# IGNF/MAESTRO

Measured on AMD Instinct MI355X. Metric: MAE-pretrain tiles/sec, higher is better.
Workload: dtype bf16

## Files before the change

### __graft_entry__.py

```python

from __future__ import annotations

import os
import subprocess
import sys
from pathlib import Path

ROOT = Path(__file__).resolve().parent
if str(ROOT) not in sys.path:
    sys.path.insert(0, str(ROOT))


def build() -> None:
    from maestro_amd.csrc.build import build as build_lib
    from maestro_amd.csrc.build import build_example

    lib = build_lib(verbose=bool(os.environ.get("MAESTRO_BUILD_VERBOSE")))
    build_example()
    import ctypes

    import maestro_amd
    from maestro_amd import hip

    handle = ctypes.CDLL(str(lib))
    import re

    for name in ("maestro_hip.h", "maestro_hip_metrics.h", "maestro_hip_det.h"):
        header = (ROOT / "include" / name).read_text()
        missing = [n for n in re.findall(r"\b(mh_[a-z0-9_]+)\s*\(", header) if not hasattr(handle, n)]
        if missing:
            raise RuntimeError(f"libmaestro_hip.so lacks symbols declared in include/{name}: {sorted(set(missing))}")
    assert hip.lib().mh_version() >= 1


def smoke() -> None:
    import torch

    import maestro_amd.conf as conf
    from maestro_amd.ssl import mae as pmae
    from maestro_amd.train.optim import FusedAdamW
    from oracle import mae as om
    from oracle.gen_golden import build_datasets, case_table, init_weights, make_batch

    if not torch.cuda.is_available():
        raise RuntimeError("smoke() needs cuda:0")
    dev = torch.device("cuda:0")
    case = case_table()["c3_aerial_s2"]
    ds = build_datasets(case, conf)
    kw = dict(interpolate="nearest", model="mae", num_levels=1, fusion_mode=case["fusion"], inter_depth=case["inter_depth"],
              **case["model_kw"])
    oracle = om.build_oracle(ds, conf.MaskConfig(), model_size=case["size"], **kw)
    init_weights(oracle, case["seed"])
    model = getattr(pmae, f"mae_{case['size']}")(datasets=ds, mask=conf.MaskConfig(), **kw)
    model.load_state_dict(oracle.state_dict(), strict=True)
    batch = make_batch(ds.dataset, case["B"], case["seed"], stress=case.get("stress", False))
    eng = model.engine(case["B"], dev, loss="l2_norm")
    torch.manual_seed(7)
    noise, struct = eng.draw_masks()
    loss = eng.forward({k: v.to(dev) for k, v in batch.items()}, noise=noise, struct=struct)
    eng.zero_grad()
    eng.backward()
    pixels, masks = eng.reconstructions()
    ob, orec, omsk, _ = oracle({k: v.clone() for k, v in batch.items()}, "pretrain", noise=noise,
                               struct_masks={g: s[:, :, None] for g, s in struct.items()})
    want = om.compute_loss_rec(ob, orec, omsk, oracle.out_grid_size, om.norm_bands_of(ds.dataset), "l2_norm")
    got = float(loss.item())
    assert abs(got - want.item()) < 3e-3 * abs(want.item()), (got, want.item())
    for m in orec:
        assert torch.equal(masks[m].cpu(), omsk[m]), f"{m}: mask indices differ from the oracle"
        rel = ((pixels[m].cpu() - orec[m]).norm() / orec[m].norm()).item()
        assert rel < 1.3e-2, (m, rel)
    FusedAdamW(eng, 1e-3).step()
    loss2 = float(eng.forward({k: v.to(dev) for k, v in batch.items()}, noise=noise, struct=struct).item())
    assert loss2 < got, (loss2, got)
    print(f"smoke ok: loss hip={got:.6f} oracle={want.item():.6f}; after one AdamW step {loss2:.6f}")


if __name__ == "__main__":
    build()
    if "--smoke" in sys.argv:
# ... 2 lines not shown
```

### maestro_amd/csrc/build.py

```python

from __future__ import annotations

import hashlib
import os
import shutil
import subprocess
import sys
from concurrent.futures import ThreadPoolExecutor
from pathlib import Path

CSRC = Path(__file__).resolve().parent
ROOT = CSRC.parent.parent
LIB_DIR = CSRC.parent / "lib"
LIB = LIB_DIR / "libmaestro_hip.so"
OBJ_DIR = CSRC / "build"
ARCH = "gfx950"
FLAGS = ["-O3", "-std=c++17", "-fPIC", f"--offload-arch={ARCH}", "-Wno-unused-result"] + os.environ.get("MH_BUILD_FLAGS", "").split()
FILE_FLAGS = {"attn.hip": ["-mllvm", "-amdgpu-mfma-vgpr-form", "-fno-slp-vectorize"] + os.environ.get("MH_ATTN_FLAGS", "").split(),
              "gemm_sk.hip": ["-mllvm", "-amdgpu-mfma-vgpr-form"]}
NO_PK_F32 = ["-Xclang", "-target-feature", "-Xclang", "-packed-fp32-ops"]
for _f in ("gemm.hip", "gemm_pp.hip", "gemm_dma.hip"):
    FILE_FLAGS[_f] = FILE_FLAGS.get(_f, []) + NO_PK_F32


def _hipcc() -> str:
    for cand in (shutil.which("hipcc"), "/opt/rocm/bin/hipcc"):
        if cand and Path(cand).exists():
            return cand
    raise RuntimeError("hipcc not found; the MI355X kernels cannot be built")


def _digest(src: Path) -> str:
    h = hashlib.sha256()
    for f in [src, *sorted(CSRC.glob("*.hpp")), ROOT / "include" / "maestro_hip.h",
              ROOT / "include" / "maestro_hip_metrics.h", ROOT / "include" / "maestro_hip_det.h"]:
        h.update(f.read_bytes())
    h.update(" ".join(FLAGS + FILE_FLAGS.get(src.name, [])).encode())
    return h.hexdigest()[:16]


def build(force: bool = False, verbose: bool = False) -> Path:
    hipcc = _hipcc()
    OBJ_DIR.mkdir(exist_ok=True)
    LIB_DIR.mkdir(exist_ok=True)
    sources = sorted(CSRC.glob("*.hip"))
    jobs, objs = [], []
    for src in sources:
        obj = OBJ_DIR / f"{src.stem}.{_digest(src)}.o"
        objs.append(obj)
        if force or not obj.exists():
            for old in OBJ_DIR.glob(f"{src.stem}.*.o"):
                old.unlink()
            jobs.append((src, obj))

    def compile_one(job):
        src, obj = job
        cmd = [hipcc, *FLAGS, *FILE_FLAGS.get(src.name, []), "-c", str(src), "-o", str(obj)]
        if verbose:
            print(" ".join(cmd), flush=True)
        r = subprocess.run(cmd, capture_output=True, text=True)
        if r.returncode != 0:
            raise RuntimeError(f"hipcc failed for {src.name}:\n{r.stdout}\n{r.stderr}")
        return "\n".join(ln for ln in r.stderr.splitlines() if "'-packed-fp32-ops' is not a recognized feature" not in ln)

    if jobs:
        with ThreadPoolExecutor(max_workers=min(4, os.cpu_count() or 1)) as ex:
            for warn in ex.map(compile_one, jobs):
                if verbose and warn:
                    print(warn, file=sys.stderr)
    if jobs or not LIB.exists():
        cmd = [hipcc, "-shared", "-fPIC", f"--offload-arch={ARCH}", *map(str, objs), "-o", str(LIB)]
        r = subprocess.run(cmd, capture_output=True, text=True)
        if r.returncode != 0:
            raise RuntimeError(f"link failed:\n{r.stdout}\n{r.stderr}")
    return LIB


EXAMPLE_SRC = ROOT / "examples" / "abi_smoke.cpp"
EXAMPLE_BIN = ROOT / "examples" / "abi_smoke"


def build_example(force: bool = False) -> Path:
    if not force and EXAMPLE_BIN.exists() and EXAMPLE_BIN.stat().st_mtime >= max(EXAMPLE_SRC.stat().st_mtime, LIB.stat().st_mtime):
        return EXAMPLE_BIN
    cmd = [_hipcc(), "-O2", "-std=c++17", f"--offload-arch={ARCH}", str(EXAMPLE_SRC), f"-I{ROOT / 'include'}", f"-L{LIB_DIR}",
           "-lmaestro_hip", "-Wl,-rpath,$ORIGIN/../maestro_amd/lib", "-o", str(EXAMPLE_BIN)]
    r = subprocess.run(cmd, capture_output=True, text=True)
    if r.returncode != 0:
# ... 8 lines not shown
```

### maestro_amd/csrc/embed.hip

```cpp
#include "common.hpp"
#include "reduce_det.hpp"
#include "../../include/maestro_hip.h"

namespace {

__device__ __forceinline__ float block_sum_any(float v, float* red) {
    v = wave_sum(v);
    const int nw = blockDim.x >> 6;
    if (nw == 1) return v;
    const int w = threadIdx.x >> 6, l = threadIdx.x & 63;
    __syncthreads();
    if (l == 0) red[w] = v;
    __syncthreads();
    float t = 0.f;
    for (int i = 0; i < nw; ++i) t += red[i];
    return t;
}

__global__ void patchify_kernel(const float* __restrict__ img, bf16_t* __restrict__ cols, float* __restrict__ target,
                                int Csrc, int c0, int Ctot, int S, int P, int Kpad, const int* __restrict__ norm_bands,
                                int n_groups, int normalise, int rescale_elev) {
    extern __shared__ __attribute__((aligned(16))) float patch[];
    const int g = S / P;
    const int tok = blockIdx.x;
    const int bd = tok / (g * g), pp = tok - bd * g * g, ph = pp / g, pw = pp - ph * g;
    const int PP = P * P, K = Ctot * PP;
    float* red = patch + K;
    const float* base0 = img + ((size_t)bd * Csrc) * S * S + (size_t)(ph * P) * S + pw * P;
    const float* base = base0 + (size_t)c0 * S * S;
    if ((P & 3) == 0 && (Kpad & 3) == 0) {
        for (int k = threadIdx.x * 4; k < Kpad; k += blockDim.x * 4) {
            f32x4 v = {0.f, 0.f, 0.f, 0.f};
            if (k < K) {
                const int c = k / PP, r = k - c * PP, p1 = r / P, p2 = r - p1 * P;
                v = *reinterpret_cast<const f32x4*>(base + (size_t)c * S * S + p1 * S + p2);
                if (rescale_elev && c0 + c >= 1) v = 30.f * (*reinterpret_cast<const f32x4*>(base0 + p1 * S + p2) - v);
#pragma unroll
                for (int e = 0; e < 4; ++e) patch[(r + e) * Ctot + c] = v[e];
            }
            if (cols) {
                u32x2 pk = {pack_bf2(v[0], v[1]), pack_bf2(v[2], v[3])};
                *reinterpret_cast<u32x2*>(cols + (size_t)tok * Kpad + k) = pk;
            }
        }
    } else {
        for (int k = threadIdx.x; k < Kpad; k += blockDim.x) {
            float v = 0.f;
            if (k < K) {
                const int c = k / PP, r = k - c * PP, p1 = r / P, p2 = r - p1 * P;
                v = base[(size_t)c * S * S + p1 * S + p2];
                if (rescale_elev && c0 + c >= 1) v = 30.f * (base0[p1 * S + p2] - v);
                patch[r * Ctot + c] = v;
            }
            if (cols) cols[(size_t)tok * Kpad + k] = f2bf(v);
        }
// ... 130 lines not shown
    }
}

__global__ __launch_bounds__(64) void gn_finalize_kernel(const float* __restrict__ partial, float* __restrict__ stats,
                                                         long per_image, int nchunk, float eps) {
    const int bd = blockIdx.x;
    double s = 0.0;
    for (int i = threadIdx.x; i < nchunk; i += 64) s += partial[((size_t)bd * nchunk + i) * 2];
    for (int o = 32; o > 0; o >>= 1) s += __shfl_xor(s, o, 64);
    const double mu = s / per_image;
    double q = 0.0;
    for (int i = threadIdx.x; i < nchunk; i += 64) {
        const float sc = partial[((size_t)bd * nchunk + i) * 2];
        const float nc = (float)min((long)GN_CHUNK, per_image - (long)i * GN_CHUNK);
        const float mc = sc / nc;
        const double dm = (double)mc - mu;
        q += partial[((size_t)bd * nchunk + i) * 2 + 1] + dm * (2.0 * ((double)sc - (double)nc * mc) + (double)nc * dm);
    }
    for (int o = 32; o > 0; o >>= 1) q += __shfl_xor(q, o, 64);
    if (threadIdx.x == 0) {
        const double var = fmax(q / per_image, 0.0);
        stats[bd * 2] = (float)mu;
        stats[bd * 2 + 1] = (float)(1.0 / sqrt(var + (double)eps));
    }
}

__global__ __launch_bounds__(256) void embed_finish_kernel(const float* __restrict__ y, const float* __restrict__ stats,
                                                           const float* __restrict__ gamma, const float* __restrict__ beta,
                                                           const float* __restrict__ pos, const float* __restrict__ date,
                                                           float* __restrict__ xg, int B, int D, int L, int E, int tok_off,
                                                           int Lgroup, int date_rows, int date_off) {
    const int row = blockIdx.x * 4 + (threadIdx.x >> 6), lane = threadIdx.x & 63;
    if (row >= B * D * L) return;
    const int bd = row / L, l = row - bd * L, b = bd / D, d = bd - b * D;
    const float mu = stats[bd * 2], rs = stats[bd * 2 + 1];
    const float* yr = y + (size_t)row * E;
    float* o = xg + ((size_t)b * Lgroup + tok_off + d * L + l) * E;
    const float* pr = pos + (size_t)l * E;
    const float* dr = date ? date + ((size_t)b * date_rows + date_off + d) * 8 : nullptr;
    for (int c = lane * 4; c < E; c += 256) {
        const f32x4 v = *reinterpret_cast<const f32x4*>(yr + c);
        const f32x4 g = *reinterpret_cast<const f32x4*>(gamma + c);
        const f32x4 bt = *reinterpret_cast<const f32x4*>(beta + c);
        const f32x4 ps = *reinterpret_cast<const f32x4*>(pr + c);
        f32x4 r;
#pragma unroll
        for (int e = 0; e < 4; ++e) r[e] = (v[e] - mu) * rs * g[e] + bt[e] + ps[e];
        if (dr && c >= E - 8) r += *reinterpret_cast<const f32x4*>(dr + (c - (E - 8)));
        *reinterpret_cast<f32x4*>(o + c) = r;
    }
}

constexpr int EB_ROWS = 8;
template <int NV, bool DET>
__global__ __launch_bounds__(256) void embed_bwd_stats_kernel(const float* __restrict__ dxg, const float* __restrict__ y,
                                                              const float* __restrict__ stats, const float* __restrict__ gamma,
                                                              float* __restrict__ sums, float* __restrict__ dgamma,
                                                              float* __restrict__ dbeta, int B, int D, int L, int E,
                                                              int tok_off, int Lgroup) {
    extern __shared__ __attribute__((aligned(16))) float red[];
    const int w = threadIdx.x >> 6, lane = threadIdx.x & 63;
    const int bd = blockIdx.y, b = bd / D, d = bd - b * D;
    const float mu = stats[bd * 2], rs = stats[bd * 2 + 1];
    float* rg = red + (size_t)w * 2 * E;
    float s1 = 0.f, s2 = 0.f;
    const int l0 = (blockIdx.x * 4 + w) * EB_ROWS;
    if constexpr (NV > 0) {
        f32x4 gz[NV], gd[NV], gm[NV];
#pragma unroll
        for (int j = 0; j < NV; ++j) {
            const int c = lane * 4 + 256 * j;
            gz[j] = (f32x4){0, 0, 0, 0}; gd[j] = (f32x4){0, 0, 0, 0};
            gm[j] = c < E ? *reinterpret_cast<const f32x4*>(gamma + c) : (f32x4){0, 0, 0, 0};
        }
#pragma unroll 2
        for (int rr = 0; rr < EB_ROWS; ++rr) {
            const int l = l0 + rr;
            if (l >= L) break;
            const float* yr = y + ((size_t)bd * L + l) * E;
            const float* gr = dxg + ((size_t)b * Lgroup + tok_off + d * L + l) * E;
#pragma unroll
            for (int j = 0; j < NV; ++j) {
                const int c = lane * 4 + 256 * j;
                if (c < E) {
                    const f32x4 v = *reinterpret_cast<const f32x4*>(yr + c);
                    const f32x4 dd = *reinterpret_cast<const f32x4*>(gr + c);
#pragma unroll
                    for (int e = 0; e < 4; ++e) {
                        const float z = (v[e] - mu) * rs, dz = dd[e] * gm[j][e];
                        s1 += dz; s2 += dz * z;
                        gz[j][e] += dd[e] * z;
                        gd[j][e] += dd[e];
                    }
                }
            }
        }
#pragma unroll
        for (int j = 0; j < NV; ++j) {
            const int c = lane * 4 + 256 * j;
            if (c < E) {
                *reinterpret_cast<f32x4*>(rg + c) = gz[j];
                *reinterpret_cast<f32x4*>(rg + E + c) = gd[j];
            }
        }
    } else {
        for (int c = lane; c < 2 * E; c += 64) rg[c] = 0.f;
        for (int rr = 0; rr < EB_ROWS; ++rr) {
            const int l = l0 + rr;
            if (l >= L) break;
            const float* yr = y + ((size_t)bd * L + l) * E;
            const float* gr = dxg + ((size_t)b * Lgroup + tok_off + d * L + l) * E;
            for (int c = lane * 4; c < E; c += 256) {
                const f32x4 v = *reinterpret_cast<const f32x4*>(yr + c);
                const f32x4 dd = *reinterpret_cast<const f32x4*>(gr + c);
                const f32x4 gm = *reinterpret_cast<const f32x4*>(gamma + c);
#pragma unroll
                for (int e = 0; e < 4; ++e) {
                    const float z = (v[e] - mu) * rs, dz = dd[e] * gm[e];
                    s1 += dz; s2 += dz * z;
                    rg[c + e] += dd[e] * z;
                    rg[E + c + e] += dd[e];
                }
            }
        }
    }
    s1 = wave_sum(s1); s2 = wave_sum(s2);
    if constexpr (DET) {
        if (lane == 0) { red[8 * E + 2 * w] = s1; red[8 * E + 2 * w + 1] = s2; }
    } else {
    if (lane == 0) { atomicAdd(sums + bd * 2, s1); atomicAdd(sums + bd * 2 + 1, s2); }
    }
    __syncthreads();
    for (int c = threadIdx.x; c < 2 * E; c += 256) {
        const float t = red[c] + red[2 * E + c] + red[4 * E + c] + red[6 * E + c];
        if constexpr (DET) {
            dgamma[((size_t)bd * gridDim.x + blockIdx.x) * 2 * E + c] = t;
        } else {
        if (c < E) atomicAdd(dgamma + c, t); else atomicAdd(dbeta + (c - E), t);
        }
    }
    if constexpr (DET) {
        if (threadIdx.x < 2) {
            const float* ws = red + 8 * E + threadIdx.x;
            sums[((size_t)bd * gridDim.x + blockIdx.x) * 2 + threadIdx.x] = ((ws[0] + ws[2]) + ws[4]) + ws[6];
        }
    }
}

__global__ __launch_bounds__(64) void embed_bwd_sums_det_kernel(const float* __restrict__ blk_sums, float* __restrict__ sums, int nblk) {
    if (threadIdx.x < 2)
        sums[blockIdx.x * 2 + threadIdx.x] = 0.f + ordered_job_total(blk_sums + (size_t)blockIdx.x * nblk * 2 + threadIdx.x, nblk, 2);
}

__global__ __launch_bounds__(256) void zero_f32_kernel(float* __restrict__ p, int n) {
    const int i = blockIdx.x * 256 + threadIdx.x;
    if (i < n) p[i] = 0.f;
}

__global__ __launch_bounds__(256) void embed_bwd_apply_kernel(const float* __restrict__ dxg, const float* __restrict__ y,
                                                              const float* __restrict__ stats, const float* __restrict__ gamma,
                                                              const float* __restrict__ sums, bf16_t* __restrict__ dyc,
                                                              int B, int D, int L, int E, int tok_off, int Lgroup) {
    const int row = blockIdx.x * 4 + (threadIdx.x >> 6), lane = threadIdx.x & 63;
    if (row >= B * D * L) return;
    const int bd = row / L, l = row - bd * L, b = bd / D, d = bd - b * D;
    const float mu = stats[bd * 2], rs = stats[bd * 2 + 1];
    const float n = (float)L * (float)E;
    const float c1 = sums[bd * 2] / n, c2 = sums[bd * 2 + 1] / n;
    const float* yr = y + (size_t)row * E;
    const float* gr = dxg + ((size_t)b * Lgroup + tok_off + d * L + l) * E;
    bf16_t* o = dyc + (size_t)row * E;
    for (int c = lane * 4; c < E; c += 256) {
        const f32x4 v = *reinterpret_cast<const f32x4*>(yr + c);
        const f32x4 dd = *reinterpret_cast<const f32x4*>(gr + c);
        const f32x4 gm = *reinterpret_cast<const f32x4*>(gamma + c);
        float r[4];
#pragma unroll
        for (int e = 0; e < 4; ++e) {
            const float z = (v[e] - mu) * rs;
            r[e] = rs * (dd[e] * gm[e] - c1 - z * c2);
        }
        u32x2 pk = {pack_bf2(r[0], r[1]), pack_bf2(r[2], r[3])};
        *reinterpret_cast<u32x2*>(o + c) = pk;
    }
}

__global__ __launch_bounds__(256) void depatchify_kernel(const float* __restrict__ patches, float* __restrict__ img,
                                                         int C, int S, int P, long total) {
    const long i = (long)blockIdx.x * 256 + threadIdx.x;
    if (i >= total) return;
    const int x = i % S; long r = i / S;
    const int yy = r % S; r /= S;
    const int c = r % C; const long bd = r / C;
    const int g = S / P, ph = yy / P, p1 = yy - ph * P, pw = x / P, p2 = x - pw * P;
    img[i] = patches[((bd * g + ph) * g + pw) * (long)(P * P * C) + (p1 * P + p2) * C + c];
}

__global__ __launch_bounds__(256) void date_features_kernel(const int16_t* __restrict__ dates, const int16_t* __restrict__ ref,
                                                            float* __restrict__ out, int B, int D, int rows, int row_off, float fac) {
    const int i = blockIdx.x * 256 + threadIdx.x;
    if (i >= B * D) return;
    const int b = i / D, d = i - b * D;
    const int16_t* dt = dates + (size_t)i * 3;
    const float year = (float)dt[0], doy = (float)dt[1] / 365.25f, hour = (float)dt[2] / 24.0f;
    const float year_ref = (float)ref[b * 3], doy_ref = (float)ref[b * 3 + 1] / 365.25f;
    const float diff = (year + doy) - (year_ref + doy_ref);
    const float a = 6.283185307179586f * doy, h = 6.283185307179586f * hour;
    float* o = out + ((size_t)b * rows + row_off + d) * 8;
    o[0] = o[1] = o[2] = o[3] = diff * fac;
    o[4] = sinf(a) * fac; o[5] = cosf(a) * fac; o[6] = sinf(h) * fac; o[7] = cosf(h) * fac;
}

__global__ __launch_bounds__(256) void rescale_elev_kernel(const float* __restrict__ img, float* __restrict__ out, int C, long plane, long total) {
    const long i = (long)blockIdx.x * 256 + threadIdx.x;
    if (i >= total) return;
    const long px = i % plane; const long r = i / plane; const int c = r % C; const long bd = r / C;
    const float v = img[i];
    out[i] = c == 0 ? v : 30.f * (img[(bd * C) * plane + px] - v);
}

__device__ __forceinline__ void cubic_weights(float t, float (&w)[4]) {
    const float A = -0.75f;
    const float x0 = t + 1.f, x3 = 2.f - t, x2 = 1.f - t;
    w[0] = ((A * x0 - 5.f * A) * x0 + 8.f * A) * x0 - 4.f * A;
    w[1] = ((A + 2.f) * t - (A + 3.f)) * t * t + 1.f;
    w[2] = ((A + 2.f) * x2 - (A + 3.f)) * x2 * x2 + 1.f;
    w[3] = ((A * x3 - 5.f * A) * x3 + 8.f * A) * x3 - 4.f * A;
}
__global__ __launch_bounds__(256) void resize_kernel(const float* __restrict__ in, float* __restrict__ out, int Hin, int Win,
                                                     int Hout, int Wout, int mode, long total) {
    const long i = (long)blockIdx.x * 256 + threadIdx.x;
    if (i >= total) return;
    const int x = i % Wout; const long r = i / Wout; const int y = r % Hout; const long plane = r / Hout;
    const float* src = in + plane * (long)Hin * Win;
    const float sy = (float)Hin / (float)Hout, sx = (float)Win / (float)Wout;
    if (mode == 0) {
        const int yy = min((int)floorf(y * sy), Hin - 1), xx = min((int)floorf(x * sx), Win - 1);
// ... 135 lines not shown
    MH_LAUNCH_CHECK();
    return 0;
}

extern "C" int mh_groupnorm_stats(const float* y, float* partial, float* stats, int BD, int L, int E, float eps,
                                  void* stream) {
    MH_CHECK_ARG(y && partial && stats && E % 4 == 0, "mh_groupnorm_stats: bad arguments");
    const long per_image = (long)L * E;
    const int nchunk = ceil_div(per_image, GN_CHUNK);
    hipLaunchKernelGGL(gn_partial_kernel, dim3(nchunk, BD), dim3(256), 0, (hipStream_t)stream, y, partial, per_image, nchunk);
    hipLaunchKernelGGL(gn_finalize_kernel, dim3(BD), dim3(64), 0, (hipStream_t)stream, partial, stats, per_image, nchunk, eps);
    MH_LAUNCH_CHECK();
    return 0;
}

extern "C" int mh_groupnorm_partial_size(int BD, int L, int E) { return BD * ceil_div((long)L * E, GN_CHUNK) * 2; }

extern "C" int mh_embed_finish(const float* y, const float* stats, const float* gamma, const float* beta,
                               const float* pos, const float* date, int date_rows, int date_off, float* xg, int B, int D,
                               int L, int E, int tok_off, int Lgroup, void* stream) {
    MH_CHECK_ARG(y && stats && gamma && beta && pos && xg && E % 4 == 0 && E >= 8, "mh_embed_finish: bad arguments");
    MH_CHECK_ARG(tok_off + D * L <= Lgroup, "mh_embed_finish: modality does not fit its group sequence");
    hipLaunchKernelGGL(embed_finish_kernel, dim3(ceil_div((long)B * D * L, 4)), dim3(256), 0, (hipStream_t)stream, y, stats,
                       gamma, beta, pos, date, xg, B, D, L, E, tok_off, Lgroup, date_rows, date_off);
    MH_LAUNCH_CHECK();
    return 0;
}

extern "C" int mh_embed_finish_bwd(const float* dxg, const float* y, const float* stats, const float* gamma, void* dyc,
                                   float* dgamma, float* dbeta, float* sums, int B, int D, int L, int E, int tok_off,
                                   int Lgroup, void* stream) {
    MH_CHECK_ARG(dxg && y && stats && gamma && dyc && dgamma && dbeta && sums && E % 4 == 0, "mh_embed_finish_bwd: bad arguments");
    hipStream_t s = (hipStream_t)stream;
    hipLaunchKernelGGL(zero_f32_kernel, dim3(ceil_div((long)B * D * 2, 256)), dim3(256), 0, s, sums, B * D * 2);
    {
        const dim3 grid(ceil_div(L, 4 * EB_ROWS), B * D), block(256);
        const size_t lds = (size_t)8 * E * sizeof(float);
#define MH_EB_LAUNCH(NV) hipLaunchKernelGGL((embed_bwd_stats_kernel<NV, false>), grid, block, lds, s, dxg, y, stats, gamma, sums, dgamma, dbeta, B, D, L, E, tok_off, Lgroup)
        switch ((E + 255) / 256) {
            case 1: MH_EB_LAUNCH(1); break;
            case 2: MH_EB_LAUNCH(2); break;
            case 3: MH_EB_LAUNCH(3); break;
            case 4: MH_EB_LAUNCH(4); break;
            default: MH_EB_LAUNCH(0); break;
        }
#undef MH_EB_LAUNCH
    }
    hipLaunchKernelGGL(embed_bwd_apply_kernel, dim3(ceil_div((long)B * D * L, 4)), dim3(256), 0, s, dxg, y, stats, gamma, sums,
                       (bf16_t*)dyc, B, D, L, E, tok_off, Lgroup);
    MH_LAUNCH_CHECK();
    return 0;
}

extern "C" int mh_embed_bwd_partial_rows(int BD, int L) { return BD > 0 && L > 0 ? BD * ceil_div(L, 4 * EB_ROWS) : 0; }

extern "C" int mh_embed_finish_bwd_det(const float* dxg, const float* y, const float* stats, const float* gamma, void* dyc,
                                       float* param_partial, float* blk_sums, float* sums, int B, int D, int L, int E, int tok_off,
                                       int Lgroup, void* stream) {
    MH_CHECK_ARG(dxg && y && stats && gamma && dyc && param_partial && blk_sums && sums, "mh_embed_finish_bwd_det: null pointer");
    MH_CHECK_ARG(B > 0 && D > 0 && L > 0 && E > 0 && E % 4 == 0 && tok_off >= 0 && tok_off + D * L <= Lgroup,
                 "mh_embed_finish_bwd_det: bad sizes B=%d D=%d L=%d E=%d tok_off=%d Lgroup=%d", B, D, L, E, tok_off, Lgroup);
    hipStream_t s = (hipStream_t)stream;
    const int nblk = ceil_div(L, 4 * EB_ROWS);
    {
        const dim3 grid(nblk, B * D), block(256);
        const size_t lds = (size_t)(8 * E + 8) * sizeof(float);
#define MH_EB_LAUNCH(NV) hipLaunchKernelGGL((embed_bwd_stats_kernel<NV, true>), grid, block, lds, s, dxg, y, stats, gamma, blk_sums, param_partial, (float*)nullptr, B, D, L, E, tok_off, Lgroup)
        switch ((E + 255) / 256) {
            case 1: MH_EB_LAUNCH(1); break;
            case 2: MH_EB_LAUNCH(2); break;
            case 3: MH_EB_LAUNCH(3); break;
            case 4: MH_EB_LAUNCH(4); break;
            default: MH_EB_LAUNCH(0); break;
        }
#undef MH_EB_LAUNCH
    }
    hipLaunchKernelGGL(embed_bwd_sums_det_kernel, dim3(B * D), dim3(64), 0, s, blk_sums, sums, nblk);
    hipLaunchKernelGGL(embed_bwd_apply_kernel, dim3(ceil_div((long)B * D * L, 4)), dim3(256), 0, s, dxg, y, stats, gamma, sums,
                       (bf16_t*)dyc, B, D, L, E, tok_off, Lgroup);
    MH_LAUNCH_CHECK();
    return 0;
}

extern "C" int mh_depatchify(const float* patches, float* img, int BD, int C, int S, int P, void* stream) {
    MH_CHECK_ARG(patches && img && S % P == 0, "mh_depatchify: bad arguments");
    const long total = (long)BD * C * S * S;
    hipLaunchKernelGGL(depatchify_kernel, dim3(ceil_div(total, 256)), dim3(256), 0, (hipStream_t)stream, patches, img, C, S, P, total);
    MH_LAUNCH_CHECK();
    return 0;
}
```

### maestro_amd/csrc/loss.hip

```cpp
#include "gemm_common.hpp"
#include "../../include/maestro_hip_det.h"

namespace {

template <bool DET>
__global__ __launch_bounds__(256) void masked_loss_kernel(const float* __restrict__ rec, const float* __restrict__ target,
                                                          const uint8_t* __restrict__ mask_group, const int* __restrict__ n_masked,
                                                          float weight, float* __restrict__ acc, bf16_t* __restrict__ drec,
                                                          int B, int Lm, int Lgroup, int tok_off, int PPC, int p, int tgt_C,
                                                          int tgt_c0, int n_g, int denom_is_elems, int rows_per_wave) {
    __shared__ float red[4];
    const int w = threadIdx.x >> 6, lane = threadIdx.x & 63;
    const float coef = weight / (denom_is_elems ? (float)(*n_masked) : (float)(*n_masked) * (float)PPC);
    const bool window = n_g != tgt_C;
    const int tgt_ld = window ? PPC / n_g * tgt_C : PPC;
    float s = 0.f;
    for (int rr = 0; rr < rows_per_wave; ++rr) {
        const int row = (blockIdx.x * 4 + w) * rows_per_wave + rr;
        if (row >= B * Lm) break;
        const int b = row / Lm, t = row - b * Lm;
        const bool masked = mask_group[(size_t)b * Lgroup + tok_off + t] != 0;
        const float* r = rec + (size_t)row * PPC;
        const float* g = target + (size_t)row * tgt_ld;
        bf16_t* d = drec ? drec + (size_t)row * PPC : nullptr;
        for (int c = lane * 4; c < PPC; c += 256) {
            float dd[4] = {0.f, 0.f, 0.f, 0.f};
            if (masked) {
                const f32x4 rv = *reinterpret_cast<const f32x4*>(r + c);
                f32x4 tv;
                if (!window) {
                    tv = *reinterpret_cast<const f32x4*>(g + c);
                } else {
#pragma unroll
                    for (int e = 0; e < 4; ++e) { const int pix = (c + e) / n_g; tv[e] = g[pix * tgt_C + tgt_c0 + (c + e) - pix * n_g]; }
                }
#pragma unroll
                for (int e = 0; e < 4; ++e) {
                    const float diff = rv[e] - tv[e];
                    if (p == 2) { s += diff * diff; dd[e] = 2.f * diff * coef; }
                    else { s += fabsf(diff); dd[e] = (diff > 0.f ? coef : (diff < 0.f ? -coef : 0.f)); }
                }
            }
            if (d) {
                u32x2 pk = {pack_bf2(dd[0], dd[1]), pack_bf2(dd[2], dd[3])};
                *reinterpret_cast<u32x2*>(d + c) = pk;
            }
        }
    }
    s = wave_sum(s);
    if (lane == 0) red[w] = s;
    __syncthreads();
    if (threadIdx.x == 0) {
        const float t = (red[0] + red[1]) + (red[2] + red[3]);
        if constexpr (DET) {
            acc[blockIdx.x] = (blockIdx.x == 0 && *n_masked == 0) ? __builtin_nanf("") : t * coef;
        } else {
        if (t != 0.f) atomicAdd(acc, t * coef);
        if (blockIdx.x == 0 && *n_masked == 0) atomicAdd(acc, __builtin_nanf(""));
        }
    }
}

template <bool DET>
__global__ __launch_bounds__(1024) void colsum_kernel(const void* __restrict__ x, int is_f32, float* __restrict__ out, int M,
                                                      int N, int ld, int rows_per_block) {
    __shared__ f32x4 red[16][64];
    const int w = threadIdx.x >> 6, lane = threadIdx.x & 63, nw = blockDim.x >> 6;
    const int c = (blockIdx.x * 64 + lane) * 4;
    const int r0 = blockIdx.y * rows_per_block, r1 = min(M, r0 + rows_per_block);
    f32x4 acc = {0, 0, 0, 0};
    if (c < N) {
        if (is_f32) {
#pragma unroll 8
            for (int r = r0 + w; r < r1; r += nw)
                acc += *reinterpret_cast<const f32x4*>(reinterpret_cast<const float*>(x) + (size_t)r * ld + c);
        } else {
#pragma unroll 8
            for (int r = r0 + w; r < r1; r += nw) {
                const u32x2 pk = *reinterpret_cast<const u32x2*>(reinterpret_cast<const bf16_t*>(x) + (size_t)r * ld + c);
                acc += (f32x4){__uint_as_float(pk[0] << 16), __uint_as_float(pk[0] & 0xffff0000u),
                               __uint_as_float(pk[1] << 16), __uint_as_float(pk[1] & 0xffff0000u)};
            }
        }
    }
    red[w][lane] = acc;
    __syncthreads();
    if (w == 0 && c < N) {
        f32x4 t = red[0][lane];
        for (int i = 1; i < nw; ++i) t += red[i][lane];
        if constexpr (DET) {
            *reinterpret_cast<f32x4*>(out + (size_t)blockIdx.y * N + c) = t;
        } else {
#pragma unroll
        for (int e = 0; e < 4; ++e) atomicAdd(out + c + e, t[e]);
        }
    }
}

__global__ __launch_bounds__(256) void zero_spans_kernel(float* __restrict__ base, const long* __restrict__ spans) {
    const long off = spans[2 * blockIdx.y], len = spans[2 * blockIdx.y + 1];
// ... 140 lines not shown
    MH_CHECK_ARG((p == 1 || p == 2) && PPC % 4 == 0 && tok_off + Lm <= Lgroup, "mh_masked_loss: bad arguments");
    const int rpw = loss_rows_per_wave((long)B * Lm);
    hipLaunchKernelGGL(masked_loss_kernel<false>, dim3(ceil_div((long)B * Lm, 4 * rpw)), dim3(256), 0, (hipStream_t)stream, rec, target, mask_group, n_masked,
                       weight, acc, (bf16_t*)drec, B, Lm, Lgroup, tok_off, PPC, p, 1, 0, 1, 0, rpw);
    MH_LAUNCH_CHECK();
    return 0;
}

extern "C" int mh_masked_loss_bands(const float* rec, const float* target, const uint8_t* mask_group, const int* n_elems,
                                    float weight, float* acc, void* drec, int B, int Lm, int Lgroup, int tok_off, int PPC, int p,
                                    int tgt_C, int tgt_c0, int n_g, void* stream) {
    MH_CHECK_ARG(rec && target && mask_group && n_elems && acc, "mh_masked_loss_bands: null pointer");
    MH_CHECK_ARG((p == 1 || p == 2) && PPC % 4 == 0 && tok_off + Lm <= Lgroup, "mh_masked_loss_bands: bad arguments");
    MH_CHECK_ARG(n_g > 0 && PPC % n_g == 0 && tgt_c0 >= 0 && tgt_c0 + n_g <= tgt_C, "mh_masked_loss_bands: band window [%d, %d) of %d",
                 tgt_c0, tgt_c0 + n_g, tgt_C);
    const int rpw = loss_rows_per_wave((long)B * Lm);
    hipLaunchKernelGGL(masked_loss_kernel<false>, dim3(ceil_div((long)B * Lm, 4 * rpw)), dim3(256), 0, (hipStream_t)stream, rec, target, mask_group, n_elems,
                       weight, acc, (bf16_t*)drec, B, Lm, Lgroup, tok_off, PPC, p, tgt_C, tgt_c0, n_g, 1, rpw);
    MH_LAUNCH_CHECK();
    return 0;
}

extern "C" int mh_masked_loss_partial_size(int B, int Lm) {
    const long rows = (long)B * Lm;
    return rows > 0 ? ceil_div(rows, 4 * loss_rows_per_wave(rows)) : 0;
}

extern "C" int mh_masked_loss_det(const float* rec, const float* target, const uint8_t* mask_group, const int* n_masked,
                                  float weight, float* loss_partial, void* drec, int B, int Lm, int Lgroup, int tok_off, int PPC,
                                  int p, void* stream) {
    MH_CHECK_ARG(rec && target && mask_group && n_masked && loss_partial, "mh_masked_loss_det: null pointer");
    MH_CHECK_ARG(B > 0 && Lm > 0 && (p == 1 || p == 2) && PPC % 4 == 0 && tok_off + Lm <= Lgroup, "mh_masked_loss_det: bad arguments");
    const int rpw = loss_rows_per_wave((long)B * Lm);
    hipLaunchKernelGGL(masked_loss_kernel<true>, dim3(ceil_div((long)B * Lm, 4 * rpw)), dim3(256), 0, (hipStream_t)stream, rec, target,
                       mask_group, n_masked, weight, loss_partial, (bf16_t*)drec, B, Lm, Lgroup, tok_off, PPC, p, 1, 0, 1, 0, rpw);
    MH_LAUNCH_CHECK();
    return 0;
}

extern "C" int mh_masked_loss_bands_det(const float* rec, const float* target, const uint8_t* mask_group, const int* n_elems,
                                        float weight, float* loss_partial, void* drec, int B, int Lm, int Lgroup, int tok_off,
                                        int PPC, int p, int tgt_C, int tgt_c0, int n_g, void* stream) {
    MH_CHECK_ARG(rec && target && mask_group && n_elems && loss_partial, "mh_masked_loss_bands_det: null pointer");
    MH_CHECK_ARG(B > 0 && Lm > 0 && (p == 1 || p == 2) && PPC % 4 == 0 && tok_off + Lm <= Lgroup, "mh_masked_loss_bands_det: bad arguments");
    MH_CHECK_ARG(n_g > 0 && PPC % n_g == 0 && tgt_c0 >= 0 && tgt_c0 + n_g <= tgt_C, "mh_masked_loss_bands_det: band window [%d, %d) of %d",
                 tgt_c0, tgt_c0 + n_g, tgt_C);
    const int rpw = loss_rows_per_wave((long)B * Lm);
    hipLaunchKernelGGL(masked_loss_kernel<true>, dim3(ceil_div((long)B * Lm, 4 * rpw)), dim3(256), 0, (hipStream_t)stream, rec, target,
                       mask_group, n_elems, weight, loss_partial, (bf16_t*)drec, B, Lm, Lgroup, tok_off, PPC, p, tgt_C, tgt_c0, n_g, 1, rpw);
    MH_LAUNCH_CHECK();
    return 0;
}

extern "C" int mh_colsum_partial_rows(int M) { return M > 0 ? ceil_div(M, MH_COLSUM_PARTIAL_ROWS) : 0; }

extern "C" int mh_colsum_partial(const void* x, int x_is_f32, float* partial, int M, int N, int ld, void* stream) {
    MH_CHECK_ARG(x && partial && ((uintptr_t)partial % 16) == 0, "mh_colsum_partial: null pointer / partial not 16-byte aligned");
    MH_CHECK_ARG(M > 0 && N > 0 && N % 4 == 0 && ld % 4 == 0 && N <= ld, "mh_colsum_partial: bad sizes M=%d N=%d ld=%d", M, N, ld);
    hipLaunchKernelGGL(colsum_kernel<true>, dim3(ceil_div(N, 256), ceil_div(M, MH_COLSUM_PARTIAL_ROWS)), dim3(1024), 0,
                       (hipStream_t)stream, x, x_is_f32, partial, M, N, ld, MH_COLSUM_PARTIAL_ROWS);
    MH_LAUNCH_CHECK();
    return 0;
}

extern "C" int mh_colsum(const void* x, int x_is_f32, float* out, int M, int N, int ld, void* stream) {
    MH_CHECK_ARG(x && out && N % 4 == 0 && ld % 4 == 0, "mh_colsum: bad arguments");
    const int col_blocks = ceil_div(N, 256);
    int rows_per_block = 1024;
    while (rows_per_block > 128 && (long)col_blocks * ceil_div(M, rows_per_block) < 128) rows_per_block >>= 1;
    hipLaunchKernelGGL(colsum_kernel<false>, dim3(col_blocks, ceil_div(M, rows_per_block)), dim3(1024), 0, (hipStream_t)stream, x,
                       x_is_f32, out, M, N, ld, rows_per_block);
    MH_LAUNCH_CHECK();
    return 0;
}

extern "C" int mh_zero_spans(float* base, const long* spans_device, int n_spans, long max_len, void* stream) {
    MH_CHECK_ARG(base && spans_device && n_spans > 0 && max_len > 0, "mh_zero_spans: bad arguments");
    dim3 grid((unsigned)min(64L, (max_len + 1023) / 1024), n_spans);
    hipLaunchKernelGGL(zero_spans_kernel, grid, dim3(256), 0, (hipStream_t)stream, base, spans_device);
    MH_LAUNCH_CHECK();
    return 0;
}

extern "C" int mh_cast_bf16(const float* src, void* dst, long n, void* stream) {
    MH_CHECK_ARG(src && dst && n > 0, "mh_cast_bf16: bad arguments");
    hipLaunchKernelGGL(cast_bf16_kernel, dim3(ceil_div(n, 1024)), dim3(256), 0, (hipStream_t)stream, src, (bf16_t*)dst, n);
    MH_LAUNCH_CHECK();
    return 0;
}

extern "C" int mh_pack_rows_bf16(const float* w, void* dst, int E, int K, int Kpad, void* stream) {
    MH_CHECK_ARG(w && dst && Kpad >= K, "mh_pack_rows_bf16: bad arguments");
    hipLaunchKernelGGL(pack_rows_kernel, dim3(ceil_div((long)E * Kpad, 256)), dim3(256), 0, (hipStream_t)stream, w, (bf16_t*)dst, E, K, Kpad);
    MH_LAUNCH_CHECK();
    return 0;
}

extern "C" int mh_unpack_rows_add(const float* src, float* dst, int E, int K, int Kpad, void* stream) {
    MH_CHECK_ARG(src && dst && Kpad >= K, "mh_unpack_rows_add: bad arguments");
    hipLaunchKernelGGL(unpack_rows_add_kernel, dim3(ceil_div((long)E * K, 256)), dim3(256), 0, (hipStream_t)stream, src, dst, E, K, Kpad);
    MH_LAUNCH_CHECK();
    return 0;
}

extern "C" int mh_adamw(float* p, const float* g, float* m, float* v, void* p_bf16, long n, float lr, float b1, float b2,
                        float eps, float wd, int step, float grad_scale, void* stream) {
// ... 31 lines not shown
```

### maestro_amd/csrc/mask.hip

```cpp
#include "common.hpp"
#include "../../include/maestro_hip.h"

namespace {

__global__ __launch_bounds__(1024) void mask_select_kernel(const float* __restrict__ noise, const uint8_t* __restrict__ smask,
                                                          int* __restrict__ visible_idx, int* __restrict__ masked_idx,
                                                          int* __restrict__ inv, uint8_t* __restrict__ mask, int L, int k) {
    extern __shared__ __attribute__((aligned(16))) float sm[];
    const int L4 = (L + 3) & ~3;
    int* wtot = reinterpret_cast<int*>(sm + L4);
    const int b = blockIdx.x, lane = threadIdx.x & 63, w = threadIdx.x >> 6;
    for (int i = threadIdx.x; i < L4; i += 1024) {
        float v = INFINITY;
        if (i < L) {
            v = noise[(size_t)b * L + i];
            if (smask && smask[(size_t)b * L + i]) v = 0.f;
        }
        sm[i] = v;
    }
    __syncthreads();
    int base = 0;
    for (int i0 = 0; i0 < L; i0 += 1024) {
        const int i = i0 + threadIdx.x;
        int f = 0;
        if (i < L) {
            const float v = sm[i];
            int r = 0;
            for (int j = 0; j < L4; j += 4) {
                const f32x4 u = *reinterpret_cast<const f32x4*>(sm + j);
                r += (int)((u[0] < v) | ((u[0] == v) & (j < i)));
                r += (int)((u[1] < v) | ((u[1] == v) & (j + 1 < i)));
                r += (int)((u[2] < v) | ((u[2] == v) & (j + 2 < i)));
                r += (int)((u[3] < v) | ((u[3] == v) & (j + 3 < i)));
            }
            f = r < k;
        }
        const unsigned long long bal = __ballot(f);
        const int before = __popcll(bal & ((1ull << lane) - 1ull));
        __syncthreads();
        if (lane == 0) wtot[w] = __popcll(bal);
        __syncthreads();
        int nm = base + before, tot = 0;
#pragma unroll
        for (int x = 0; x < 16; ++x) {
            const int c = wtot[x];
            nm += x < w ? c : 0;
            tot += c;
        }
        base += tot;
        if (i < L) {
            mask[(size_t)b * L + i] = (uint8_t)f;
            if (f) {
                masked_idx[(size_t)b * k + nm] = i;
                inv[(size_t)b * L + i] = -1;
            } else {
                visible_idx[(size_t)b * (L - k) + (i - nm)] = i;
                inv[(size_t)b * L + i] = i - nm;
            }
        }
    }
}

__global__ __launch_bounds__(256) void gather_rows_kernel(const float* __restrict__ src, const int* __restrict__ idx,
                                                          float* __restrict__ dst, int B, int src_L, int n_idx, int dim,
                                                          int dst_L, int dst_off) {
    const int row = blockIdx.x * 4 + (threadIdx.x >> 6), lane = threadIdx.x & 63;
    if (row >= B * n_idx) return;
    const int b = row / n_idx, j = row - b * n_idx;
    const float* s = src + ((size_t)b * src_L + idx[row]) * dim;
    float* d = dst + ((size_t)b * dst_L + dst_off + j) * dim;
    for (int c = lane * 4; c < dim; c += 256) *reinterpret_cast<f32x4*>(d + c) = *reinterpret_cast<const f32x4*>(s + c);
}

__global__ __launch_bounds__(256) void scatter_rows_kernel(const float* __restrict__ ddst, const int* __restrict__ idx,
                                                           float* __restrict__ dsrc, int B, int src_L, int n_idx, int dim,
                                                           int dst_L, int dst_off) {
    const int row = blockIdx.x * 4 + (threadIdx.x >> 6), lane = threadIdx.x & 63;
    if (row >= B * n_idx) return;
    const int b = row / n_idx, j = row - b * n_idx;
    float* s = dsrc + ((size_t)b * src_L + idx[row]) * dim;
    const float* d = ddst + ((size_t)b * dst_L + dst_off + j) * dim;
    for (int c = lane * 4; c < dim; c += 256) *reinterpret_cast<f32x4*>(s + c) = *reinterpret_cast<const f32x4*>(d + c);
}

__global__ __launch_bounds__(256) void expand_rows_kernel(const float* __restrict__ src, const int* __restrict__ inv,
                                                          float* __restrict__ dst, int B, int L, int n, int dim) {
    const int row = blockIdx.x * 4 + (threadIdx.x >> 6), lane = threadIdx.x & 63;
    if (row >= B * L) return;
    const int b = row / L, iv = inv[row];
    float* o = dst + (size_t)row * dim;
    const float* s = src + ((size_t)b * n + (iv < 0 ? 0 : iv)) * dim;
    for (int c = lane * 4; c < dim; c += 256) {
        f32x4 v = {0.f, 0.f, 0.f, 0.f};
        if (iv >= 0) v = *reinterpret_cast<const f32x4*>(s + c);
        *reinterpret_cast<f32x4*>(o + c) = v;
    }
}

__global__ __launch_bounds__(256) void unmask_kernel(const float* __restrict__ y, const int* __restrict__ inv,
                                                     const float* __restrict__ mask_token, const int* __restrict__ tok_slot,
                                                     const float* __restrict__ pos, const float* __restrict__ date,
                                                     const int* __restrict__ date_row, int n_date_rows,
                                                     float* __restrict__ xdec, int B, int L, int n_vis, int Dd, int slot_stride) {
    const int row = blockIdx.x * 4 + (threadIdx.x >> 6), lane = threadIdx.x & 63;
    if (row >= B * L) return;
    const int b = row / L, t = row - b * L;
    const int iv = inv[row];
    const float* s = iv < 0 ? mask_token + (size_t)tok_slot[(size_t)b * slot_stride + t] * Dd : y + ((size_t)b * n_vis + iv) * Dd;
    const float* pr = pos + (size_t)t * Dd;
    const float* dr = date ? date + ((size_t)b * n_date_rows + date_row[t]) * 8 : nullptr;
    float* o = xdec + (size_t)row * Dd;
    for (int c = lane * 4; c < Dd; c += 256) {
        f32x4 v = *reinterpret_cast<const f32x4*>(s + c) + *reinterpret_cast<const f32x4*>(pr + c);
        if (dr && c >= Dd - 8) v += *reinterpret_cast<const f32x4*>(dr + (c - (Dd - 8)));
        *reinterpret_cast<f32x4*>(o + c) = v;
    }
}

constexpr int UM_ROWS = 512, UM_NT = 1024;
template <bool DET>
__global__ __launch_bounds__(UM_NT) void unmask_bwd_token_kernel(const float* __restrict__ dxdec, const uint8_t* __restrict__ mask,
                                                                 const int* __restrict__ tok_slot, float* __restrict__ dmask_token,
                                                                 int B, int L, int Dd, int slot, int t_lo, int t_hi, int slot_stride) {
    __shared__ __attribute__((aligned(16))) float red[UM_NT * 4];
// ... 24 lines not shown
                const int off = ri < UM_ROWS ? row_off[ri] : -1;
                if (off >= 0) v[u] = *reinterpret_cast<const f32x4*>(dxdec + (size_t)off * Dd + 4 * col);
            }
            acc += (v[0] + v[1]) + (v[2] + v[3]);
        }
    }
    *reinterpret_cast<f32x4*>(red + 4 * threadIdx.x) = acc;
    __syncthreads();
    if (sub == 0) {
        for (int s = 1; s < lanes; ++s) acc += *reinterpret_cast<const f32x4*>(red + 4 * (s * cols + col));
        if constexpr (DET) {
            *reinterpret_cast<f32x4*>(dmask_token + (size_t)blockIdx.x * Dd + 4 * col) = acc;
        } else {
#pragma unroll
        for (int e = 0; e < 4; ++e) if (acc[e] != 0.f) atomicAdd(dmask_token + 4 * col + e, acc[e]);
        }
    }
}

__global__ __launch_bounds__(1024) void count_masked_kernel(const uint8_t* __restrict__ mask, int B, int L, int t_lo, int t_hi,
                                                            int* __restrict__ out, int mult, int accumulate) {
    __shared__ float red[16];
    const int span = t_hi - t_lo, w = threadIdx.x >> 6, lane = threadIdx.x & 63;
    float c = 0.f;
    for (int b = w; b < B; b += 16) {
        const uint8_t* row = mask + (size_t)b * L + t_lo;
        for (int t = lane; t < span; t += 64) c += row[t] ? 1.f : 0.f;
    }
    c = block_sum<16>(c, red);
    if (threadIdx.x == 0) *out = (accumulate ? *out : 0) + (int)(c + 0.5f) * mult;
}

}

extern "C" int mh_mask_select(const float* noise, const uint8_t* struct_mask, int* visible_idx, int* masked_idx, int* inv,
                              uint8_t* mask, int B, int L, int k, void* stream) {
    MH_CHECK_ARG(noise && visible_idx && masked_idx && inv && mask, "mh_mask_select: null pointer");
    MH_CHECK_ARG(B > 0 && L > 0 && k >= 0 && k <= L && L <= 8192, "mh_mask_select: bad sizes B=%d L=%d k=%d", B, L, k);
    hipLaunchKernelGGL(mask_select_kernel, dim3(B), dim3(1024), (size_t)((L + 3) & ~3) * 4 + 64, (hipStream_t)stream, noise, struct_mask,
                       visible_idx, masked_idx, inv, mask, L, k);
    MH_LAUNCH_CHECK();
    return 0;
}

extern "C" int mh_gather_rows(const float* src, const int* idx, float* dst, int B, int src_L, int n_idx, int dim, int dst_L,
                              int dst_off, void* stream) {
    MH_CHECK_ARG(src && idx && dst && dim % 4 == 0 && dst_off + n_idx <= dst_L, "mh_gather_rows: bad arguments");
    hipLaunchKernelGGL(gather_rows_kernel, dim3(ceil_div((long)B * n_idx, 4)), dim3(256), 0, (hipStream_t)stream, src, idx, dst, B,
                       src_L, n_idx, dim, dst_L, dst_off);
    MH_LAUNCH_CHECK();
    return 0;
}

extern "C" int mh_scatter_rows(const float* ddst, const int* idx, float* dsrc, int B, int src_L, int n_idx, int dim,
                               int dst_L, int dst_off, void* stream) {
    MH_CHECK_ARG(ddst && idx && dsrc && dim % 4 == 0 && dst_off + n_idx <= dst_L, "mh_scatter_rows: bad arguments");
    hipLaunchKernelGGL(scatter_rows_kernel, dim3(ceil_div((long)B * n_idx, 4)), dim3(256), 0, (hipStream_t)stream, ddst, idx, dsrc,
                       B, src_L, n_idx, dim, dst_L, dst_off);
    MH_LAUNCH_CHECK();
    return 0;
}

extern "C" int mh_expand_rows(const float* src, const int* inv, float* dst, int B, int L, int n, int dim, void* stream) {
    MH_CHECK_ARG(src && inv && dst && B > 0 && L > 0 && n > 0 && dim % 4 == 0, "mh_expand_rows: bad arguments");
    hipLaunchKernelGGL(expand_rows_kernel, dim3(ceil_div((long)B * L, 4)), dim3(256), 0, (hipStream_t)stream, src, inv, dst, B, L,
                       n, dim);
    MH_LAUNCH_CHECK();
    return 0;
}

extern "C" int mh_unmask_assemble(const float* y, const int* inv, const float* mask_token, const int* tok_slot,
                                  const float* pos, const float* date, const int* date_row, int n_date_rows, float* xdec,
                                  int B, int L, int n_vis, int Dd, void* stream) {
    MH_CHECK_ARG(y && inv && mask_token && tok_slot && pos && xdec && Dd % 4 == 0 && Dd >= 8, "mh_unmask_assemble: bad arguments");
    MH_CHECK_ARG(!date || date_row, "mh_unmask_assemble: date without date_row");
    hipLaunchKernelGGL(unmask_kernel, dim3(ceil_div((long)B * L, 4)), dim3(256), 0, (hipStream_t)stream, y, inv, mask_token,
                       tok_slot, pos, date, date_row, n_date_rows, xdec, B, L, n_vis, Dd, 0);
    MH_LAUNCH_CHECK();
    return 0;
}

extern "C" int mh_unmask_assemble_per_sample(const float* y, const int* inv, const float* mask_token, const int* tok_slot_bl,
                                             const float* pos, const float* date, const int* date_row, int n_date_rows,
                                             float* xdec, int B, int L, int n_vis, int Dd, void* stream) {
    MH_CHECK_ARG(y && inv && mask_token && tok_slot_bl && pos && xdec && Dd % 4 == 0 && Dd >= 8, "mh_unmask_assemble_per_sample: bad arguments");
    MH_CHECK_ARG(!date || date_row, "mh_unmask_assemble_per_sample: date without date_row");
    hipLaunchKernelGGL(unmask_kernel, dim3(ceil_div((long)B * L, 4)), dim3(256), 0, (hipStream_t)stream, y, inv, mask_token,
                       tok_slot_bl, pos, date, date_row, n_date_rows, xdec, B, L, n_vis, Dd, L);
    MH_LAUNCH_CHECK();
    return 0;
}

extern "C" int mh_unmask_token_grad(const float* dxdec, const uint8_t* mask, const int* tok_slot, float* dmask_token, int B,
                                    int L, int Dd, int slot, int t_lo, int t_hi, void* stream) {
    MH_CHECK_ARG(dxdec && mask && tok_slot && dmask_token && Dd % 4 == 0 && Dd <= 1024, "mh_unmask_token_grad: bad arguments");
    MH_CHECK_ARG(0 <= t_lo && t_lo < t_hi && t_hi <= L, "mh_unmask_token_grad: bad token range");
    hipLaunchKernelGGL(unmask_bwd_token_kernel<false>, dim3(ceil_div((long)B * (t_hi - t_lo), UM_ROWS)), dim3(UM_NT), 0,
                       (hipStream_t)stream, dxdec, mask, tok_slot, dmask_token, B, L, Dd, slot, t_lo, t_hi, 0);
    MH_LAUNCH_CHECK();
    return 0;
}

extern "C" int mh_unmask_token_grad_per_sample(const float* dxdec, const uint8_t* mask, const int* tok_slot_bl, float* dmask_token,
                                               int B, int L, int Dd, int slot, void* stream) {
    MH_CHECK_ARG(dxdec && mask && tok_slot_bl && dmask_token && Dd % 4 == 0 && Dd <= 1024 && B > 0 && L > 0,
                 "mh_unmask_token_grad_per_sample: bad arguments");
// ... 45 lines not shown
```

### maestro_amd/csrc/norm.hip

```cpp
#include "gemm_common.hpp"

namespace {

struct RowMap { int L, off; };
__device__ __forceinline__ size_t map_row(RowMap m, int b, int j) { return (size_t)b * m.L + m.off + j; }

template <int NV>
__global__ __launch_bounds__(256) void ln_fwd_kernel(const float* __restrict__ x, RowMap xm, const float* __restrict__ gamma,
                                                     const float* __restrict__ beta, void* __restrict__ y, RowMap ym,
                                                     int y_is_f32, float* __restrict__ mean, float* __restrict__ rstd,
                                                     int B, int n, int dim, float eps, uint8_t* __restrict__ y8,
                                                     const float* __restrict__ y8_scale, float* __restrict__ y8_amax,
                                                     uint8_t* __restrict__ y8s, int ld_y8s) {
    const int row = blockIdx.x * 4 + (threadIdx.x >> 6);
    const int lane = threadIdx.x & 63;
    if (row >= B * n) return;
    const int b = row / n, j = row - b * n;
    const float* xr = x + map_row(xm, b, j) * dim;
    const int nv = dim >> 2;
    f32x4 v[NV];
    float s = 0.f;
#pragma unroll
    for (int i = 0; i < NV; ++i) {
        const int c = lane + 64 * i;
        v[i] = (f32x4){0, 0, 0, 0};
        if (c < nv) v[i] = *reinterpret_cast<const f32x4*>(xr + 4 * c);
        s += (v[i][0] + v[i][1]) + (v[i][2] + v[i][3]);
    }
    const float mu = wave_sum(s) / dim;
    float q = 0.f;
#pragma unroll
    for (int i = 0; i < NV; ++i) {
        if (lane + 64 * i < nv) {
#pragma unroll
            for (int e = 0; e < 4; ++e) { const float d = v[i][e] - mu; q += d * d; }
        }
    }
    const float rs = rsqrtf(wave_sum(q) / dim + eps);
    if (lane == 0) { mean[row] = mu; rstd[row] = rs; }
    const size_t yrow = map_row(ym, b, j) * dim;
    const bool t8 = y8 && !y8s;
    const float s8 = t8 ? *y8_scale : 0.f;
    float amax8 = 0.f;
#pragma unroll
    for (int i = 0; i < NV; ++i) {
        const int c = lane + 64 * i;
        u32x2 pk16 = {0u, 0u};
        if (c < nv) {
            const f32x4 g = *reinterpret_cast<const f32x4*>(gamma + 4 * c);
            const f32x4 bt = *reinterpret_cast<const f32x4*>(beta + 4 * c);
            f32x4 o;
#pragma unroll
            for (int e = 0; e < 4; ++e) o[e] = (v[i][e] - mu) * rs * g[e] + bt[e];
// ... 269 lines not shown
        gm[i] = *reinterpret_cast<const f32x4*>(gamma + 4 * (lane + 64 * i));
    }
    const int row0 = (blockIdx.x * 4 + w) * ROWS_PER_WAVE;
    if (row0 < B * n) {
        f32x4 xq[ROWS_PER_WAVE][NV], rq[ROWS_PER_WAVE][NV];
        u32x2 dq[ROWS_PER_WAVE][NV];
        float muq[ROWS_PER_WAVE], rsq[ROWS_PER_WAVE];
        size_t xrowq[ROWS_PER_WAVE];
        auto fetch = [&](int p) {
            const int row = row0 + p, b = row / n, j = row - b * n;
            xrowq[p] = map_row(xm, b, j) * dim;
            const size_t dyrow = map_row(dym, b, j) * dim;
            muq[p] = mean[row]; rsq[p] = rstd[row];
#pragma unroll
            for (int i = 0; i < NV; ++i) {
                const int c4 = 4 * (lane + 64 * i);
                xq[p][i] = *reinterpret_cast<const f32x4*>(x + xrowq[p] + c4);
                dq[p][i] = *reinterpret_cast<const u32x2*>(dy + dyrow + c4);
                rq[p][i] = *reinterpret_cast<const f32x4*>(dres + xrowq[p] + c4);
            }
        };
#pragma unroll
        for (int p = 0; p < DEPTH; ++p) fetch(p);
#pragma unroll
        for (int rr = 0; rr < ROWS_PER_WAVE; ++rr) {
            if (rr + DEPTH < ROWS_PER_WAVE) fetch(rr + DEPTH);
            __builtin_amdgcn_sched_barrier(0);
            const float mu = muq[rr], rs = rsq[rr];
            f32x4 xh[NV], dz[NV];
            float s1 = 0.f, s2 = 0.f;
#pragma unroll
            for (int i = 0; i < NV; ++i) {
                const u32x2 pk = dq[rr][i];
                const f32x4 d = {__uint_as_float(pk[0] << 16), __uint_as_float(pk[0] & 0xffff0000u),
                                 __uint_as_float(pk[1] << 16), __uint_as_float(pk[1] & 0xffff0000u)};
#pragma unroll
                for (int e = 0; e < 4; ++e) {
                    xh[i][e] = (xq[rr][i][e] - mu) * rs;
                    dz[i][e] = d[e] * gm[i][e];
                    s1 += dz[i][e];
                    s2 += dz[i][e] * xh[i][e];
                    gsum[i][e] += d[e] * xh[i][e];
                    bsum[i][e] += d[e];
                }
            }
            const float c1 = ln_wave_sum(s1) / dim, c2 = ln_wave_sum(s2) / dim;
#pragma unroll
            for (int i = 0; i < NV; ++i) {
                const int c4 = 4 * (lane + 64 * i);
                f32x4 o;
#pragma unroll
                for (int e = 0; e < 4; ++e) o[e] = rs * (dz[i][e] - c1 - xh[i][e] * c2);
                o += rq[rr][i];
                csum[i] += o;
                *reinterpret_cast<f32x4*>(dx + xrowq[rr] + c4) = o;
                const u32x2 pk = {pack_bf2(o[0], o[1]), pack_bf2(o[2], o[3])};
                *reinterpret_cast<u32x2*>(dx_bf16 + xrowq[rr] + c4) = pk;
            }
            __builtin_amdgcn_sched_barrier(0);
        }
    }
    if (!partial) return;
    float* rg = red + (size_t)w * 3 * dim;
#pragma unroll
    for (int i = 0; i < NV; ++i) {
        const int c4 = 4 * (lane + 64 * i);
        *reinterpret_cast<f32x4*>(rg + c4) = gsum[i];
        *reinterpret_cast<f32x4*>(rg + dim + c4) = bsum[i];
        *reinterpret_cast<f32x4*>(rg + 2 * dim + c4) = csum[i];
    }
    __syncthreads();
    float* prow = partial + (size_t)blockIdx.x * 3 * dim;
    for (int c = threadIdx.x; c < 3 * dim; c += 256)
        prow[c] = red[c] + red[3 * dim + c] + red[6 * dim + c] + red[9 * dim + c];
}

#ifndef LN_BWD_DEPTH
#define LN_BWD_DEPTH 4
#endif
constexpr int RED_ROWS = 8;
__global__ __launch_bounds__(256) void ln_bwd_reduce_kernel(const float* __restrict__ partial, int nblk, int dim,
                                                            float* __restrict__ dgamma, float* __restrict__ dbeta,
                                                            float* __restrict__ dcol) {
    const int c = blockIdx.x * 256 + threadIdx.x;
    if (c >= 3 * dim) return;
    const int r0 = blockIdx.y * RED_ROWS, r1 = min(nblk, r0 + RED_ROWS);
    float s = 0.f;
    for (int r = r0; r < r1; ++r) s += partial[(size_t)r * 3 * dim + c];
    if (c < dim) atomicAdd(dgamma + c, s);
    else if (c < 2 * dim) atomicAdd(dbeta + (c - dim), s);
    else if (dcol) atomicAdd(dcol + (c - 2 * dim), s);
}

__global__ __launch_bounds__(256) void colsum_batched_kernel(const MhColsumJob* __restrict__ jobs, int n_jobs,
                                                             const uint64_t* __restrict__ blocks) {
    const uint64_t e = blocks[blockIdx.x];
    const int ji = (int)(e >> 48);
    if (ji >= n_jobs) return;
    const MhColsumJob j = jobs[ji];
    const int c = (int)((e >> 32) & 0xFFFF) * 256 + threadIdx.x;
    const int r0 = (int)(e & 0xFFFFFFFFu) * MH_COLSUM_ROWS;
    if (c >= j.cols || r0 >= j.rows) return;
    const int r1 = min(j.rows, r0 + MH_COLSUM_ROWS);
    const float* src = j.src + (size_t)r0 * j.ld + c;
    float v[MH_COLSUM_ROWS];
#pragma unroll
// ... 39 lines not shown

static int layernorm_fwd_impl(const float* x, int x_L, int x_off, const float* gamma, const float* beta, void* y, int y_L,
                              int y_off, int y_is_f32, float* mean, float* rstd, int B, int n, int dim, float eps, void* y8,
                              const float* y8_scale, float* y8_amax, void* stream, void* y8s, int ld_y8s) {
    MH_CHECK_ARG(x && gamma && beta && y && mean && rstd, "mh_layernorm_fwd: null pointer");
    MH_CHECK_ARG(dim % 4 == 0 && dim >= 4 && dim <= 2048, "mh_layernorm_fwd: dim %d unsupported", dim);
    MH_CHECK_ARG(B > 0 && n > 0 && x_off + n <= x_L && y_off + n <= y_L, "mh_layernorm_fwd: bad row map");
    const int rows = B * n;
    dim3 grid(ceil_div(rows, 4)), block(256);
    hipStream_t s = (hipStream_t)stream;
#define LN_FWD(NV) hipLaunchKernelGGL(ln_fwd_kernel<NV>, grid, block, 0, s, x, RowMap{x_L, x_off}, gamma, beta, y, \
                                      RowMap{y_L, y_off}, y_is_f32, mean, rstd, B, n, dim, eps, (uint8_t*)y8, y8_scale, y8_amax, \
                                      (uint8_t*)y8s, ld_y8s)
#define LN_FWD_FAST_(NV, FP8) hipLaunchKernelGGL((ln_fwd_fast_kernel<NV, FP8>), grid, block, 0, s, x, RowMap{x_L, x_off}, gamma, beta, \
                                                 (bf16_t*)y, RowMap{y_L, y_off}, mean, rstd, B, n, eps, (uint8_t*)y8, y8_scale, y8_amax)
#define LN_FWD_FAST_MX(NV) hipLaunchKernelGGL((ln_fwd_fast_mx_kernel<NV>), grid, block, 0, s, x, RowMap{x_L, x_off}, gamma, beta, \
                                              (bf16_t*)y, RowMap{y_L, y_off}, mean, rstd, B, n, eps, (uint8_t*)y8, (uint8_t*)y8s, ld_y8s)
#define LN_FWD_FAST(NV) do { if (y8s) LN_FWD_FAST_MX(NV); else if (y8) LN_FWD_FAST_(NV, true); else LN_FWD_FAST_(NV, false); } while (0)
    const int nvs = ln_nv(dim);
    MH_CHECK_ARG(!y8s || (dim % 32 == 0 && !y_is_f32), "mh_layernorm_fwd_mx: dim %% 32 == 0 required, got %d", dim);
    if (MH_LN_FAST && nvs <= 4 && dim == 256 * nvs && !y_is_f32) {
        switch (nvs) { case 1: LN_FWD_FAST(1); break; case 2: LN_FWD_FAST(2); break; case 3: LN_FWD_FAST(3); break;
                       default: LN_FWD_FAST(4); }
    } else {
        switch (nvs) { case 1: LN_FWD(1); break; case 2: LN_FWD(2); break; case 3: LN_FWD(3); break;
                       case 4: LN_FWD(4); break; default: LN_FWD(8); }
    }
#undef LN_FWD_FAST
#undef LN_FWD_FAST_MX
#undef LN_FWD_FAST_
#undef LN_FWD
    MH_LAUNCH_CHECK();
    return 0;
}

extern "C" long mh_layernorm_bwd_workspace(int rows, int dim) {
    return (long)ceil_div(rows, 4 * ROWS_PER_WAVE) * 3 * dim;
}

static int layernorm_bwd_impl(const void* dy, int dy_L, int dy_off, int dy_is_f32, const float* x, int x_L, int x_off,
                              const float* gamma, const float* mean, const float* rstd, const float* dres, float* dx,
                              void* dx_bf16, float* dgamma, float* dbeta, float* dcol, float* workspace, bool partial_only,
                              int B, int n, int dim, void* stream) {
    const int rows = B * n, nblk = ceil_div(rows, 4 * ROWS_PER_WAVE);
    const size_t lds = (size_t)4 * 3 * dim * sizeof(float);
    dim3 grid(nblk), block(256);
    hipStream_t s = (hipStream_t)stream;
    float* part = (dgamma || partial_only) ? workspace : nullptr;
#define LN_BWD(NV) hipLaunchKernelGGL(ln_bwd_kernel<NV>, grid, block, lds, s, dy, RowMap{dy_L, dy_off}, dy_is_f32, x, \
                                      RowMap{x_L, x_off}, gamma, mean, rstd, dres, dx, (bf16_t*)dx_bf16, part, B, n, dim)
#define LN_BWD_FAST(NV, DEPTH) hipLaunchKernelGGL((ln_bwd_fast_kernel<NV, DEPTH>), grid, block, lds, s, (const bf16_t*)dy, \
                                                  RowMap{dy_L, dy_off}, x, RowMap{x_L, x_off}, gamma, mean, rstd, dres, dx, \
                                                  (bf16_t*)dx_bf16, part, B, n)
    const int nvs = ln_nv(dim);
    if (MH_LN_FAST && nvs <= 4 && dim == 256 * nvs && !dy_is_f32 && dres && dx_bf16 && rows % ROWS_PER_WAVE == 0) {
        constexpr int DEPTH = LN_BWD_DEPTH < ROWS_PER_WAVE ? LN_BWD_DEPTH : ROWS_PER_WAVE, DEPTH4 = 2 < ROWS_PER_WAVE ? 2 : ROWS_PER_WAVE;
        switch (nvs) { case 1: LN_BWD_FAST(1, DEPTH); break; case 2: LN_BWD_FAST(2, DEPTH); break;
                       case 3: LN_BWD_FAST(3, DEPTH); break; default: LN_BWD_FAST(4, DEPTH4); }
    } else {
        switch (nvs) { case 1: LN_BWD(1); break; case 2: LN_BWD(2); break; case 3: LN_BWD(3); break;
                       case 4: LN_BWD(4); break; default: LN_BWD(8); }
    }
#undef LN_BWD_FAST
#undef LN_BWD
    if (dgamma && !partial_only)
        hipLaunchKernelGGL(ln_bwd_reduce_kernel, dim3(ceil_div(3 * dim, 256), ceil_div(nblk, RED_ROWS)), dim3(256), 0, s,
                           workspace, nblk, dim, dgamma, dbeta, dcol);
    MH_LAUNCH_CHECK();
    return 0;
}

extern "C" int mh_layernorm_bwd(const void* dy, int dy_L, int dy_off, int dy_is_f32, const float* x, int x_L, int x_off,
                                const float* gamma, const float* mean, const float* rstd, const float* dres, float* dx,
                                void* dx_bf16, float* dgamma, float* dbeta, float* dcol, float* workspace, int B, int n,
                                int dim, void* stream) {
    MH_CHECK_ARG(dy && x && gamma && mean && rstd && dx, "mh_layernorm_bwd: null pointer");
    MH_CHECK_ARG((dgamma == nullptr) == (dbeta == nullptr), "mh_layernorm_bwd: dgamma/dbeta must come together");
    MH_CHECK_ARG(!dgamma || workspace, "mh_layernorm_bwd: parameter gradients need the workspace");
    MH_CHECK_ARG(!dcol || dgamma, "mh_layernorm_bwd: dcol needs dgamma/dbeta");
    MH_CHECK_ARG(dim % 4 == 0 && dim >= 4 && dim <= 2048, "mh_layernorm_bwd: dim %d unsupported", dim);
    MH_CHECK_ARG(B > 0 && n > 0 && x_off + n <= x_L && dy_off + n <= dy_L, "mh_layernorm_bwd: bad row map");
    return layernorm_bwd_impl(dy, dy_L, dy_off, dy_is_f32, x, x_L, x_off, gamma, mean, rstd, dres, dx, dx_bf16, dgamma, dbeta, dcol,
                              workspace, false, B, n, dim, stream);
}

extern "C" int mh_layernorm_bwd_partial(const void* dy, int dy_L, int dy_off, int dy_is_f32, const float* x, int x_L, int x_off,
                                        const float* gamma, const float* mean, const float* rstd, const float* dres, float* dx,
                                        void* dx_bf16, float* workspace, int B, int n, int dim, void* stream) {
    MH_CHECK_ARG(dy && x && gamma && mean && rstd && dx && workspace, "mh_layernorm_bwd_partial: null pointer");
    MH_CHECK_ARG(dim % 4 == 0 && dim >= 4 && dim <= 2048, "mh_layernorm_bwd_partial: dim %d unsupported", dim);
    MH_CHECK_ARG(B > 0 && n > 0 && x_off + n <= x_L && dy_off + n <= dy_L, "mh_layernorm_bwd_partial: bad row map");
    return layernorm_bwd_impl(dy, dy_L, dy_off, dy_is_f32, x, x_L, x_off, gamma, mean, rstd, dres, dx, dx_bf16, nullptr, nullptr,
                              nullptr, workspace, true, B, n, dim, stream);
}

extern "C" int mh_colsum_batched(const MhColsumJob* jobs_device, int n_jobs, const uint64_t* blocks_device, int n_blocks,
                                 void* stream) {
    MH_CHECK_ARG(jobs_device && blocks_device && n_jobs > 0 && n_jobs < 65536 && n_blocks > 0, "mh_colsum_batched: bad arguments");
    hipLaunchKernelGGL(colsum_batched_kernel, dim3(n_blocks), dim3(256), 0, (hipStream_t)stream, jobs_device, n_jobs, blocks_device);
    MH_LAUNCH_CHECK();
    return 0;
}
```

### maestro_amd/engine.py

```python

from __future__ import annotations

import contextlib
import gc
import os
import weakref
import time

import torch
from torch import nn

from maestro_amd import hip
from maestro_amd.fp8 import mx_scale_cols, resolve_scaling
from maestro_amd.layers.utils import draw_struct_masks

F32, BF16, I32, U8 = torch.float32, torch.bfloat16, torch.int32, torch.uint8
_NEVER = object()
_ROCTX = os.environ.get("MAESTRO_ROCTX", "0") == "1"
RING = 4
ALIGN = 64


class ParamStore:

# ... 309 lines not shown
            else:
                hip.layernorm_bwd(self.dh2, M, 0, x_in, M, 0, attn.norm.weight, s["mean1"], s["rstd1"], mid, nxt, nxt16,
                                  ps.g(attn.norm.weight), ps.g(attn.norm.bias), prev_fc2_bias, self.ln_ws, 1, M, dim)
            cur, cur16 = nxt, nxt16
            if ready:
                eng._grads_ready(self.t.layers[l])
        return cur, cur16


class PatchEmbedEnd:

    def __init__(self, eng: "EngineBase", s) -> None:
        self.eng, self.s = eng, s
        m, dev, E = eng.model, eng.device, eng.E
        e = lambda *sh, dt=F32: torch.empty(*sh, dtype=dt, device=dev)
        z = lambda *sh, dt=F32: torch.zeros(*sh, dtype=dt, device=dev)
        T, BD = s.Beff * s.n_tok, s.Beff * s.D
        self.buf = dict(
            cols=e(T, s.Kpad, dt=BF16), yconv=e(T, E), gn_partial=e(hip.groupnorm_partial_size(BD, s.L, E)), gn_stats=e(BD, 2),
            gn_sums=e(BD, 2), pos_enc=m.pos_enc_rows[s.name].to(dev), norm_bands=torch.tensor(s.norm_bands, dtype=I32, device=dev),
            w_conv16=z(E, s.Kpad, dt=BF16), dw_conv=z(E, s.Kpad), dyc=e(T, E, dt=BF16),
            pe=m.patch_embed[s.embed].patchify_bands[s.gi])

    def pack(self) -> None:
        b, s = self.buf, self.s
        hip.pack_rows_bf16(b["pe"].conv.weight, b["w_conv16"], self.eng.E, s.K, s.Kpad)

    def forward(self, batch: dict, gbuf: dict, xg: torch.Tensor, Lgroup: int, target=None, normalise: bool = False) -> None:
        eng, s, b = self.eng, self.s, self.buf
        m, B, E = eng.model, eng.B, eng.E
        BD, T = s.Beff * s.D, s.Beff * s.n_tok
        if s.G == 1 and target is not None:
            hip.patchify(batch[s.src], b["cols"], target, BD, s.C, s.S, s.P, s.Kpad, b["norm_bands"], len(s.norm_bands),
                         normalise, s.rescale_elev)
        else:
            hip.patchify_bands(batch[s.src], b["cols"], None, BD, s.C_src, s.c0, s.C, s.S, s.P, s.Kpad, None, 0, False,
                               s.rescale_elev)
            if target is not None and s.gi == 0:
                k_src = s.C_src * s.P * s.P
                hip.patchify_bands(batch[s.src], None, target, BD, s.C_src, 0, s.C_src, s.S, s.P, (k_src + 7) // 8 * 8,
                                   b["norm_bands"], len(s.norm_bands), normalise, s.rescale_elev)
        dates, ref_date = batch[f"{s.src}_dates"], batch["ref_date"]
        if s.D != s.Dates:
            hip.date_features(dates, ref_date, gbuf["dates"].view(B, s.Dates, 8), B, s.Dates, s.Dates, 0, m.fac_date_enc)
        else:
            hip.date_features(dates, ref_date, gbuf["dates"], B, s.D, gbuf["n_dates"], s.date_off, m.fac_date_enc)
        pe = b["pe"]
        hip.gemm(hip.GEMM_NT, T, E, s.Kpad, b["cols"], s.Kpad, b["w_conv16"], s.Kpad, b["yconv"], E, hip.OUT_F32 | hip.BIAS,
                 bias=pe.conv.bias)
        hip.groupnorm_stats(b["yconv"], b["gn_partial"], b["gn_stats"], BD, s.L, E)
        hip.embed_finish(b["yconv"], b["gn_stats"], pe.norm.weight, pe.norm.bias, b["pos_enc"], gbuf["dates"], gbuf["n_dates"],
                         s.date_off, xg, s.Beff, s.D, s.L, E, s.tok_off, Lgroup)

    def backward(self, dxg: torch.Tensor, Lgroup: int, clear_dw: bool) -> None:
        eng, s, b = self.eng, self.s, self.buf
        ps, E, pe, T = eng.store, eng.E, b["pe"], s.Beff * s.n_tok
        if getattr(eng, "deterministic", False):
            return self._backward_det(dxg, Lgroup)
        hip.embed_finish_bwd(dxg, b["yconv"], b["gn_stats"], pe.norm.weight, b["dyc"], ps.g(pe.norm.weight), ps.g(pe.norm.bias),
                             b["gn_sums"], s.Beff, s.D, s.L, E, s.tok_off, Lgroup)
        if clear_dw:
            b["dw_conv"].zero_()
        hip.gemm(hip.GEMM_TN, E, s.Kpad, T, b["dyc"], E, b["cols"], s.Kpad, b["dw_conv"], s.Kpad, hip.OUT_F32 | hip.ATOMIC)
        hip.unpack_rows_add(b["dw_conv"], ps.g(pe.conv.weight), E, s.K, s.Kpad)
        hip.colsum(b["dyc"], ps.g(pe.conv.bias), T, E, E)

    def _backward_det(self, dxg: torch.Tensor, Lgroup: int) -> None:
        eng, s, b = self.eng, self.s, self.buf
        ps, E, pe, T = eng.store, eng.E, b["pe"], s.Beff * s.n_tok

        def make():
            e = lambda *sh: torch.empty(*sh, dtype=F32, device=eng.device)
            rows, S, cr = hip.embed_bwd_partial_rows(s.Beff * s.D, s.L), hip.det_slices(T), hip.colsum_partial_rows(T)
            w = dict(gn=e(rows, 2 * E), blk=e(rows, 2), slabs=e(S, E, s.Kpad), cs=e(cr, E))
            flat = w["gn"].view(-1)
            return w, [(flat, ps.g(pe.norm.weight), rows, E, 2 * E), (flat[E:], ps.g(pe.norm.bias), rows, E, 2 * E),
                       (w["slabs"].view(-1), b["dw_conv"].view(-1), S, E * s.Kpad, E * s.Kpad),
                       (w["cs"].view(-1), ps.g(pe.conv.bias), cr, E, E)]
        w = eng._det_site("bwd", ("embed", s.name), make)
        hip.embed_finish_bwd_det(dxg, b["yconv"], b["gn_stats"], pe.norm.weight, b["dyc"], w["gn"], w["blk"], b["gn_sums"], s.Beff,
                                 s.D, s.L, E, s.tok_off, Lgroup)
        hip.gemm_tn_slabs(E, s.Kpad, T, b["dyc"], E, b["cols"], s.Kpad, w["slabs"])
        hip.colsum_partial(b["dyc"], w["cs"], T, E, E)


_RETIRED_GRAPHS: list = []


def resolve_deterministic(flag: bool | None = None) -> bool:
    if flag is None:
        return os.environ.get("MAESTRO_DETERMINISTIC", "0") == "1"
    return bool(flag)


def training_warm_passes() -> int:
    return 0 if _PROCESS_WARMED else max(0, int(os.environ.get("MAESTRO_WARM_PASSES", "6")))


def _retire_graphs(graphs: dict) -> None:
    if graphs:
        _RETIRED_GRAPHS.append(dict(graphs))
        graphs.clear()


def drain_retired_graphs() -> None:
    if _RETIRED_GRAPHS:
        torch.cuda.synchronize()
        _RETIRED_GRAPHS.clear()


_PROCESS_WARMED = False


class EngineBase:

    def _init_runtime(self, device, n_side_streams: int) -> None:
        self.device = device
        self.grad_hook = None
# ... 103 lines not shown
            side.wait_stream(main)
        fns[0]()
        for side, fn in zip(sides, fns[1:]):
            with torch.cuda.stream(side):
                fn()
        for side in sides:
            main.wait_stream(side)

    def _instep_tune(self, one_pass) -> None:
        self.instep_tune = False
        if (getattr(self, "fp8", None) is not None or getattr(self, "_opt", None) is not None or hip.kernel_timer_active()
                or torch.cuda.is_current_stream_capturing()):
            return
        saved = (self.use_graphs, self.multi_stream, self.grad_hook)
        self.use_graphs, self.multi_stream, self.grad_hook = False, False, None
        tuner = hip.InStepTuner()
        hip.set_instep_tuner(tuner)
        try:
            one_pass()
            for cand in tuner.CANDIDATES:
                tuner.begin(cand)
                one_pass()
            tuner.begin(None)
            self.tile_report = tuner.finish()
        finally:
            hip.set_instep_tuner(None)
            self.use_graphs, self.multi_stream, self.grad_hook = saved

    def _warm_up(self, one_pass) -> None:
        global _PROCESS_WARMED
        n, self.warm_passes = self.warm_passes, 0
        self.warm_passes_run = 0
        if (n <= 0 or _PROCESS_WARMED or getattr(self, "fp8", None) is not None or getattr(self, "_opt", None) is not None
                or hip.kernel_timer_active() or torch.cuda.is_current_stream_capturing() or not torch.is_grad_enabled()):
            return
        _PROCESS_WARMED = True
        hook, graphs = self.grad_hook, self.use_graphs
        self.use_graphs = False
        if hook is not None:
            self.grad_hook = lambda lo, hi: None
        try:
            for _ in range(n):
                one_pass()
                self.warm_passes_run += 1
        finally:
            self.grad_hook, self.use_graphs = hook, graphs

    def _first_step_passes(self, one_pass) -> None:
        if self.instep_tune:
            self._instep_tune(one_pass)
        if self.warm_passes > 0:
            self._warm_up(one_pass)

    def _launch_wgrads(self, items) -> None:
        items = [(st, lo, hi) for st, lo, hi in items if hi > lo]
        if not items:
            return
        key = tuple((st.tag, lo, hi) for st, lo, hi in items)
        table = self._wgrad_tables.get(key)
        if table is None:
            probs = [p for st, lo, hi in items for p in st.wgrad_problems(lo, hi)]
            jobs = [j for st, lo, hi in items for j in st.reduce_jobs(lo, hi)]
            table = self._wgrad_tables[key] = (hip.GroupedTN(probs, self.device), hip.ColsumBatch(jobs, self.device))
        table[1].launch()
        table[0].launch()

    @contextlib.contextmanager
    def _tuning_pass(self, what: str):
        if not self.tune_gemm or what in self._tuned or hip.kernel_timer_active():
            yield
            return
        saved = self.multi_stream
        self.multi_stream = False
        hip.set_gemm_tuning(True)
        try:
            yield
        finally:
            hip.set_gemm_tuning(False)
            self.multi_stream = saved
            self._tuned.add(what)

    def _segment(self, name: str, key, fn) -> None:
        if _ROCTX:
            torch.cuda.nvtx.range_push(f"maestro:{name.split(':')[0]}")
            try:
                return self._segment_run(name, key, fn)
            finally:
                torch.cuda.nvtx.range_pop()
        return self._segment_run(name, key, fn)

    def _segment_run(self, name: str, key, fn) -> None:
        if not self.use_graphs or hip.kernel_timer_active():
            self._ready_spans = []
            fn()
            self._flush_ready(self._ready_spans)
            return
        entry = self._graphs.get(name)
        if entry is not None and entry["key"] == key:
            entry["graph"].replay()
            self._flush_ready(entry["spans"])
            return
        seen = self._seen.get(name, _NEVER)
        self._ready_spans = []
        if seen == key:
            graph = torch.cuda.CUDAGraph()
            gc_was_on, failure = gc.isenabled(), None
            gc.disable()
            try:
                with torch.cuda.graph(graph, capture_error_mode="thread_local"):
                    fn()
            except Exception as exc:
                failure = exc
            finally:
                if gc_was_on:
                    gc.enable()
            if failure is not None:
                import warnings
                warnings.warn(f"hipGraph capture of segment {name!r} failed ({failure}); continuing with eager launches")
                self.use_graphs = False
                torch.cuda.synchronize()
                self._ready_spans = []
                fn()
                self._flush_ready(self._ready_spans)
                return
            self._graphs[name] = {"key": key, "graph": graph, "spans": list(self._ready_spans)}
            graph.replay()
        else:
            self._seen[name] = key
            fn()
        self._flush_ready(self._ready_spans)

    def _flush_ready(self, spans) -> None:
        if self.grad_hook is not None:
            for lo, hi in spans:
                self.grad_hook(lo, hi)



class MAEEngine(EngineBase):
    def __init__(self, model, batch_size: int, device, loss: str = "l2_norm", dtype: str = "bf16",
                 fp8_scaling: str | None = None, deterministic: bool = False) -> None:
        self.deterministic = bool(deterministic)
        if self.deterministic and dtype == "fp8":
            raise ValueError("deterministic=True is not available with dtype='fp8' (the amax / scale bookkeeping is not covered)")
        if loss not in ("l1", "l2", "l1_norm", "l2_norm"):
            raise ValueError(f"Invalid loss {loss}.")
        if dtype not in ("bf16", "fp8"):
            raise ValueError(f"Invalid compute dtype {dtype!r} (bf16, fp8)")
        scaling = resolve_scaling(fp8_scaling)
        self.fp8_scaling = scaling if dtype == "fp8" else None
        device = torch.device(device)
        if device.type != "cuda":
            raise hip.HipExtensionError("MAEEngine needs a GPU device; the MAE hot path has no CPU fallback")
        hip.lib()
        self.model, self.B, self.device, self.loss, self.dtype = model, batch_size, device, loss, dtype
        self.fp8, self._fp8_weights = None, {}
        self.p_loss = 1 if loss.startswith("l1") else 2
        self.normalise = loss.endswith("_norm")
        m = model
        self.e2d_identity = m.embed_dim == m.decoder_dim
        self.E, self.Dd = m.embed_dim, m.decoder_dim
        self._init_runtime(device, len(model.group_specs) - 1)
        self.wgrad_mode = os.environ.get("MAESTRO_WGRAD", "auto")
        if self.wgrad_mode not in ("auto", "fused", "deferred"):
            raise ValueError(f"MAESTRO_WGRAD={self.wgrad_mode!r}: expected auto, fused or deferred")
        self._wgrad_plans, self._zero_lists = {}, {}
        self._det_sites, self._det_tables = {"fwd": {}, "bwd": {}}, {}
        self._h2d_done = [None] * RING
        self._opt = None
        self.host_wait_s = 0.0
        self._step = 0
        self._enc_state = {}
        B = batch_size
        fold = m.fusion_mode in ("shared", "monotemp")
        self.mods, self.groups = m.mod_specs, list(m.group_specs.values())
        for s in self.mods.values():
            s.Beff = B * s.Dates if fold else B
        for g in self.groups:
            g.Beff = g.mods[0].Beff
        ordered = []
        for name in m.patch_embed:
            ordered += [(f"patch_embed.{name}.{k}", p) for k, p in m.patch_embed[name].named_parameters()]
        for name in m.encoder:
            ordered += [(f"encoder.{name}.{k}", p) for k, p in m.encoder[name].named_parameters()]
        if m.encoder_inter is not None:
            ordered += [(f"encoder_inter.{k}", p) for k, p in m.encoder_inter.named_parameters()]
        for name in m.enc_to_dec:
            ordered += [(f"enc_to_dec.{name}.{k}", p) for k, p in m.enc_to_dec[name].named_parameters()]
        ordered += [(f"mask_token.{k}", p) for k, p in m.mask_token.items()]
        for name in m.decoder:
            ordered += [(f"decoder.{name}.{k}", p) for k, p in m.decoder[name].named_parameters()]
        for name in m.embed_to_rec:
            ordered += [(f"embed_to_rec.{name}.{k}", p) for k, p in m.embed_to_rec[name].named_parameters()]
        self.store = ParamStore(ordered, device)
        for bname in ("enc_pos_encoding", "dec_pos_encoding"):
            setattr(m, bname, getattr(m, bname).to(device))
        if dtype == "fp8":
            from maestro_amd.fp8 import Fp8Plan
            self.fp8 = Fp8Plan(device, self.store.total, scaling=self.fp8_scaling)
        self._alloc()
        self._alloc_mask_upload()
        if self.fp8 is not None:
            self.fp8.finalize()
        self.store.refresh_half(force=True)
        self._pack_conv_weights()

    @property
    def grad_hook(self):
        return self._grad_hook

    @grad_hook.setter
    def grad_hook(self, fn) -> None:
        if fn is not None and getattr(self, "deterministic", False):
            raise ValueError("deterministic=True excludes a gradient hook / exchange: the order of the cross-rank sum is the "
                             "collective library's, and the ready spans would have to move behind the ordered reduce")
        self._grad_hook = fn

    def _det_site(self, phase: str, key, make, variant=None):
        site = self._det_sites[phase].get(key)
# ... 29 lines not shown
            w = dict(slabs=e(S, M, N), cs=e(cr, M))
            return w, [(w["slabs"].view(-1), weight_grad.view(-1), S, M * N, M * N), (w["cs"].view(-1), bias_grad, cr, M, M)]
        w = self._det_site("bwd", key, make)
        hip.gemm_tn_slabs(M, N, K, dy16, M, x16, N, w["slabs"])
        hip.colsum_partial(dy16, w["cs"], K, M, M)

    def _det_finish_backward(self) -> None:
        wg = self._det_tables.get("wgrad")
        if wg is None:
            probs = [p for st in self._all_stacks() for p in st.wgrad_problems()]
            n_writers: dict = {}
            for p in probs:
                n_writers[p[2].data_ptr()] = n_writers.get(p[2].data_ptr(), 0) + 1
            slabs_of, seen, slab_jobs, out = {}, {}, [], []
            for p in probs:
                dst = p[2]
                n = n_writers[dst.data_ptr()]
                if n > 1:
                    if dst.data_ptr() not in slabs_of:
                        slabs = slabs_of[dst.data_ptr()] = torch.empty(n, dst.numel(), dtype=F32, device=self.device)
                        slab_jobs.append((slabs.view(-1), dst.view(-1), n, dst.numel(), dst.numel()))
                    i = seen[dst.data_ptr()] = seen.get(dst.data_ptr(), -1) + 1
                    p = p[:2] + (slabs_of[dst.data_ptr()][i].view(dst.shape),) + p[3:]
                out.append(p)
            grouped, single = [], []
            for i, p in enumerate(out):
                try:
                    hip.GroupedTN.check(i, p)
                    grouped.append(p)
                except hip.HipExtensionError:
                    single.append(p)
            stack_jobs = [j for st in self._all_stacks() for j in st.reduce_jobs()]
            wg = self._det_tables["wgrad"] = (hip.GroupedTN(grouped, self.device) if grouped else None, single, stack_jobs + slab_jobs)
        if wg[0] is not None:
            wg[0].launch()
        for (A, B, C, M, N, K, lda, ldb, ldc) in wg[1]:
            hip.gemm(hip.GEMM_TN, M, N, K, A, lda, B, ldb, C, ldc, hip.OUT_F32)
        self._det_reduce("bwd", wg[2])
        for end in self.embed.values():
            b, s = end.buf, end.s
            hip.unpack_rows_add(b["dw_conv"], self.store.g(b["pe"].conv.weight), self.E, s.K, s.Kpad)

    def _alloc(self) -> None:
        m, dev, E, Dd = self.model, self.device, self.E, self.Dd
        e = lambda *s, dt=F32: torch.empty(*s, dtype=dt, device=dev)
        z = lambda *s, dt=F32: torch.zeros(*s, dtype=dt, device=dev)
        self._alloc_embed()
        for name, s in self.mods.items():
            T = s.Beff * s.n_tok
            first = self.mb[m.src_specs[s.src][0].name] if s.gi else None
            self.mb[name].update(
                target=first["target"] if first else e(T, s.C_src * s.P * s.P), hdec=e(T, Dd, dt=BF16), mean_f=e(T), rstd_f=e(T),
                rec=e(T, s.K), drec=e(T, s.K, dt=BF16), dh=e(T, Dd, dt=BF16), cnt=first["cnt"] if first else z(1, dt=I32))
        self.gb = {}
        self.enc, self.dec = {}, {}
        for g in self.groups:
            Bn, L, N = g.Beff, g.L, g.N
            n_dates = sum(s.D for s in g.mods)
            tok_slot = torch.cat([torch.full((s.n_tok,), s.slot, dtype=I32) for s in g.mods])
            date_row = torch.cat([(s.date_off + torch.arange(s.n_tok) // s.L).to(I32) for s in g.mods])
            pos_dec = torch.cat([m.pos_dec_rows[s.name].repeat(s.D, 1) for s in g.mods], dim=0)
            self.gb[g.name] = dict(
                xg=e(Bn, L, E), dxg=z(Bn, L, E),
                vis=e(Bn, N, dt=I32), msk=e(Bn, g.k, dt=I32), inv=e(Bn, L, dt=I32), mask=e(Bn, L, dt=U8),
                dates=z(Bn, n_dates, 8), n_dates=n_dates, tok_slot=tok_slot.to(dev), date_row=date_row.to(dev),
                pos_dec=pos_dec.to(dev).contiguous(), tok_table=e(len(g.mods), Dd),
                henc=e(Bn * N, E, dt=BF16), mean_e=e(Bn * N), rstd_e=e(Bn * N), y_e2d=e(Bn * N, Dd),
                dy_e2d=e(Bn * N, Dd), dy_e2d16=e(Bn * N, Dd, dt=BF16), dhenc=e(Bn * N, E, dt=BF16),
                mean_j=e(Bn * N), rstd_j=e(Bn * N))
            holder = m.encoder[g.model]
            self.enc[g.name] = Stack(self, holder, Bn, N, f"enc.{g.name}")
            self.dec[g.name] = Stack(self, m.decoder[g.model], Bn, L, f"dec.{g.name}")
        if m.encoder_inter is not None:
            self.joint = Stack(self, m.encoder_inter, self.B, m.joint_N, "joint")
        else:
            self.joint = None
        for g in self.groups:
            self.gb[g.name]["ln_ws"] = e(max(hip.layernorm_bwd_workspace(g.Beff * g.L, Dd),
                                             hip.layernorm_bwd_workspace(g.Beff * g.N, E)))
        self.loss_acc = z(1)
        srcs = {s.src: s for s in self.mods.values()}
        tot_w = sum(s.Dates * s.L for s in srcs.values())
        self.loss_w = {n: (s.Dates * s.L) / tot_w for n, s in srcs.items()}

    def _alloc_mask_upload(self) -> None:
        segs, off = [], 0
        for g in self.groups:
            for key, dt, esz in (("noise", F32, 4), ("struct", U8, 1)):
                n = g.Beff * g.L * esz
                segs.append((g.name, key, dt, off, n, (g.Beff, g.L)))
                off += (n + 255) // 256 * 256
        self._mask_dev = torch.zeros(off, dtype=U8, device=self.device)
        self._mask_stage = [torch.zeros(off, dtype=U8, device=self.device) for _ in range(RING)]
        self._mask_host = [torch.zeros(off, dtype=U8).pin_memory() for _ in range(RING)]
        self._upload_stream = torch.cuda.Stream(device=self.device)
        for name, key, dt, o, n, shape in segs:
            self.gb[name][key] = self._mask_dev[o: o + n].view(dt).view(shape)
            self.gb[name][key + "_h"] = [h[o: o + n].view(dt).view(shape) for h in self._mask_host]

    def _pack_conv_weights(self, fp8_done: bool = False) -> None:
        super()._pack_conv_weights()
        if self.fp8 is not None:
            if fp8_done:
                self.fp8.refresh_transposed()
            else:
                self.fp8.refresh_weights()

    def draw_masks(self, generator=None):
        struct = draw_struct_masks(self.groups, self.mods, generator)
        noise = {}
        for g in self.groups:
            if g.draw not in noise:
                noise[g.draw] = torch.rand((g.Beff * g.draw_G, g.L), generator=generator)
        return noise, struct

    @staticmethod
    def _rows_of(draws: dict, g) -> torch.Tensor:
        if g.name in draws:
            return draws[g.name]
        t = draws[g.draw]
        if g.draw_G == 1:
# ... 28 lines not shown
    def forward(self, batch: dict, noise: dict | None = None, struct: dict | None = None) -> torch.Tensor:
        if self.deterministic:
            self.tune_gemm = self.instep_tune = False
            with hip.shape_only_tiles():
                return self._forward(batch, noise, struct)
        return self._forward(batch, noise, struct)

    def _forward(self, batch: dict, noise: dict | None, struct: dict | None) -> torch.Tensor:
        if self.store.refresh_half():
            if self.fp8 is not None:
                self.fp8._w_ready = False
            self._pack_conv_weights()
        if noise is None or struct is None:
            n2, s2 = self.draw_masks()
            noise = noise if noise is not None else n2
            struct = struct if struct is not None else s2

        def one_pass():
            self.forward(batch, noise=noise, struct=struct)
            self.zero_grad()
            self.backward()
        self._first_step_passes(one_pass)
        slot = self._step % RING
        self._step += 1
        if self._h2d_done[slot] is not None:
            t0 = time.perf_counter()
            self._h2d_done[slot].synchronize()
            self.host_wait_s += time.perf_counter() - t0
        for g in self.groups:
            gbuf = self.gb[g.name]
            nh, sh = gbuf["noise_h"][slot], gbuf["struct_h"][slot]
            n_g, s_g = self._rows_of(noise, g), self._rows_of(struct, g).reshape(g.Beff, g.L)
            if self.tie_order == "torch":
                n_g, s_g = self._reference_tie_order(g, gbuf, n_g, s_g, slot)
            nh.copy_(n_g)
            sh.copy_(s_g)
        main = torch.cuda.current_stream()
        with torch.cuda.stream(self._upload_stream):
            self._mask_stage[slot].copy_(self._mask_host[slot], non_blocking=True)
            up = torch.cuda.Event()
            up.record(self._upload_stream)
        main.wait_event(up)
        self._mask_dev.copy_(self._mask_stage[slot], non_blocking=True)
        if self._opt is not None:
            hh = self._opt_hyper_h[slot]
            hh.copy_(torch.tensor(self._opt_pending if self._opt_pending is not None else [0.0] * 5, dtype=F32))
            self._opt_hyper.copy_(hh, non_blocking=True)
            self._opt_pending = None
        ev = torch.cuda.Event()
        ev.record()
        self._h2d_done[slot] = ev
        batch = self._stage_inputs(batch)
        with self._tuning_pass("forward"):
            self._segment("forward" if self._opt is None else "forward:opt", self._cur_key, lambda: self._forward_launches(batch))
        if self._opt is not None:
            self.store.mark_synced()
        return self.loss_acc

    def attach_optimizer(self, opt) -> None:
        if self.deterministic:
            raise ValueError("deterministic=True excludes overlap_optimizer (the update inside the next forward is not covered)")
        self._attach_optimizer(opt)

    def _attach_optimizer(self, opt) -> None:
        m, ps = self.model, self.store
        if (opt.lo, opt.hi) != (0, ps.total):
            raise ValueError("the overlapped optimizer expects an optimizer over the whole flat buffer")
        stages: dict = {}
        seen_spans = set()

        def add(key, params):
            params = list(params)
            if params:
                sp = ps.span(params)
                if sp not in seen_spans:
                    seen_spans.add(sp)
                    stages.setdefault(key, []).append(sp)

        for name in m.patch_embed:
            add(("embed", 0), m.patch_embed[name].parameters())
        for kind, holders in (("enc", [m.encoder[n] for n in m.encoder]),
                              ("joint", [m.encoder_inter] if m.encoder_inter is not None else []),
                              ("dec", [m.decoder[n] for n in m.decoder])):
            for t in holders:
                depth = len(t.layers)
                for l, layer in enumerate(t.layers):
                    add((kind, l), layer.parameters())
                add((kind, max(depth - 1, 0)), t.norm.parameters())
        add(("e2d", 0), [p for n in m.enc_to_dec for p in m.enc_to_dec[n].parameters()] + list(m.mask_token.values()))
        for name in m.embed_to_rec:
            add(("rec", 0), m.embed_to_rec[name].parameters())
        order = {"embed": 0, "enc": 1, "joint": 2, "e2d": 3, "dec": 4, "rec": 5}
        self._opt_stage_keys = sorted(stages, key=lambda k: (order[k[0]], k[1]))
        covered = sorted(sp for k in stages for sp in stages[k])
        assert covered[0][0] == 0 and all(a[1] <= b[0] for a, b in zip(covered, covered[1:])), "optimizer stages overlap"
        n_cov = sum(hi - lo for lo, hi in covered)
        n_par = sum((p.numel() + ALIGN - 1) // ALIGN * ALIGN for p in ps.params)
        assert n_cov >= n_par - ALIGN * len(ps.params) and covered[-1][1] <= ps.total, "optimizer stages miss parameters"
        self._opt_stages = stages
        self._opt = opt
        self._opt_hyper = torch.zeros(5, dtype=F32, device=self.device)
        self._opt_hyper_h = [torch.zeros(5, dtype=F32).pin_memory() for _ in range(RING)]
        self._opt_pending = None
        self._opt_events = {}
        self._opt_stream = torch.cuda.Stream(device=self.device)

    def defer_step(self, lr: float, grad_scale: float = 1.0) -> None:
# ... 69 lines not shown

        def tail(g):
            def run():
                gbuf, st = self.gb[g.name], self.dec[g.name]
                self._opt_wait("e2d")
                if self.joint is not None:
                    nrm = self.joint.t.norm
                    hip.layernorm_fwd(self.joint.x_last, m.joint_N, g.joint_off, nrm.weight, nrm.bias,
                                      gbuf["y_e2d" if self.e2d_identity else "henc"], g.N, 0, gbuf["mean_j"], gbuf["rstd_j"],
                                      g.Beff, g.N, E)
                lin = m.enc_to_dec[g.model]
                M = g.Beff * g.N
                if not self.e2d_identity:
                    hip.gemm(hip.GEMM_NT, M, Dd, E, gbuf["henc"], E, self.store.h(lin.weight), E, gbuf["y_e2d"], Dd,
                             hip.OUT_F32 | hip.BIAS, bias=lin.bias)
                for s in g.mods:
                    gbuf["tok_table"][s.slot].copy_(m.mask_token[s.src].view(s.G, Dd)[s.gi])
                if self.tie_order == "torch":
                    hip.unmask_assemble_per_sample(gbuf["y_e2d"], gbuf["inv"], gbuf["tok_table"], gbuf["tok_slot_ps"], gbuf["pos_dec"],
                                                   gbuf["dates"], gbuf["date_row"], gbuf["n_dates"], st.x0, g.Beff, g.L, g.N, Dd)
                else:
                    hip.unmask_assemble(gbuf["y_e2d"], gbuf["inv"], gbuf["tok_table"], gbuf["tok_slot"], gbuf["pos_dec"],
                                        gbuf["dates"], gbuf["date_row"], gbuf["n_dates"], st.x0, g.Beff, g.L, g.N, Dd)
                st.forward(lambda l: self._opt_wait("dec", l))
                tail_post(g, gbuf, st)
            return run

        def tail_post(g, gbuf, st):
            nrm = st.t.norm
            self._opt_wait("rec")
            for s in g.mods:
                b = self.mb[s.name]
                T = s.Beff * s.n_tok
                conv = m.embed_to_rec[s.embed].pixelify_bands[s.gi].conv
                hip.layernorm_fwd(st.x_last, g.L, s.tok_off, nrm.weight, nrm.bias, b["hdec"], s.n_tok, 0, b["mean_f"],
                                  b["rstd_f"], s.Beff, s.n_tok, Dd)
                hip.gemm(hip.GEMM_NT, T, s.K, Dd, b["hdec"], Dd, self.store.h(conv.weight).view(s.K, Dd), Dd, b["rec"],
                         s.K, hip.OUT_F32 | hip.BIAS, bias=conv.bias)
                if s.G == 1:
                    hip.count_masked(gbuf["mask"], g.Beff, g.L, s.tok_off, s.tok_off + s.n_tok, b["cnt"])
            for s in g.mods:
                b = self.mb[s.name]
                if self.deterministic:
                    def make(s=s):
                        part = torch.empty(hip.masked_loss_partial_size(s.Beff, s.n_tok), dtype=F32, device=self.device)
                        return part, [(part, self.loss_acc, part.numel(), 1, 1)]
                    part = self._det_site("fwd", ("loss", s.name), make)
                    if s.G == 1:
                        hip.masked_loss_det(b["rec"], b["target"], gbuf["mask"], b["cnt"], self.loss_w[s.src], part,
                                            b["drec"], s.Beff, s.n_tok, g.L, s.tok_off, s.K, self.p_loss)
                    else:
                        hip.masked_loss_bands_det(b["rec"], b["target"], gbuf["mask"], b["cnt"], self.loss_w[s.src], part,
                                                  b["drec"], s.Beff, s.n_tok, g.L, s.tok_off, s.K, self.p_loss, s.C_src, s.c0, s.C)
                elif s.G == 1:
                    hip.masked_loss(b["rec"], b["target"], gbuf["mask"], b["cnt"], self.loss_w[s.src], self.loss_acc,
                                    b["drec"], s.Beff, s.n_tok, g.L, s.tok_off, s.K, self.p_loss)
                else:
                    hip.masked_loss_bands(b["rec"], b["target"], gbuf["mask"], b["cnt"], self.loss_w[s.src], self.loss_acc,
                                          b["drec"], s.Beff, s.n_tok, g.L, s.tok_off, s.K, self.p_loss, s.C_src, s.c0, s.C)

        self._run_parallel([head(g) for g in self.groups])
        if self.joint is not None:
            self.joint.forward(lambda l: self._opt_wait("joint", l))
        for parts in m.src_specs.values():
            if len(parts) > 1:
                for s in parts:
                    g = m.group_specs[s.group]
                    hip.count_masked_elems(self.gb[g.name]["mask"], g.Beff, g.L, s.tok_off, s.tok_off + s.n_tok,
                                           self.mb[s.name]["cnt"], s.K, s.gi > 0)
        self._run_parallel([tail(g) for g in self.groups])
        if self.deterministic:
            self._det_reduce("fwd")
        if self._opt is not None and self._opt_events:
            torch.cuda.current_stream().wait_stream(self._opt_stream)
        if self.fp8 is not None:
            self.fp8.end_of_forward()

    def zero_grad(self) -> None:
        plan = self._wgrad_plan()
        if plan == "fused":
            self.store.grad.zero_()
            for b in self.mb.values():
                if b.get("dw_conv") is not None:
                    b["dw_conv"].zero_()
            self._dw_conv_clear = True
            return
        z = self._zero_lists.get(plan)
        if z is None:
            writers = {}
            for st in self._all_stacks():
                for prob in st.wgrad_problems():
                    c = prob[2]
                    writers.setdefault(c.data_ptr(), [0, c.numel()])[0] += 1
            base = self.store.grad.data_ptr()
            stored = sorted(((ptr - base) // 4, n) for ptr, (cnt, n) in writers.items() if cnt == 1)
            spans, cur = [], 0
            for off, n in stored:
                if off > cur:
                    spans.append((cur, off - cur))
                cur = off + n
            if cur < self.store.total:
                spans.append((cur, self.store.total - cur))
            for b in self.mb.values():
                if b.get("dw_conv") is not None:
                    spans.append(((b["dw_conv"].data_ptr() - base) // 4, b["dw_conv"].numel()))
            dev = torch.tensor([v for sp in spans for v in sp], dtype=torch.int64, device=self.device)
            z = self._zero_lists[plan] = (dev, len(spans), max(n for _, n in spans))
        hip.zero_spans(self.store.grad, z[0], z[1], z[2])
        self._dw_conv_clear = True

    WGRAD_MIN_TILES = 256

    def _wgrad_plan(self) -> str:
        if self.deterministic:
            return "all"
        if self.wgrad_mode == "fused":
            return "fused"
        hooked = self.grad_hook is not None
        plan = self._wgrad_plans.get((self.wgrad_mode, hooked))
        if plan is not None:
            return plan
        try:
            every = {st.tag: hip.GroupedTN.count_tiles(st.wgrad_problems()) for st in self._all_stacks()}
            tiles = [every[st.tag] for st in self.enc.values()] if hooked else list(every.values())
            ok = True
        except hip.HipExtensionError:
            tiles, ok = [], False
        if not ok:
            if self.wgrad_mode == "deferred":
                raise hip.HipExtensionError("MAESTRO_WGRAD=deferred: a weight-gradient problem is not eligible for the grouped GEMM")
            plan = "fused"
        elif hooked:
            n_seg = len(self._enc_cuts()) - 1
            plan = "enc" if self.wgrad_mode == "deferred" or sum(tiles) // n_seg >= self.WGRAD_MIN_TILES else "fused"
        else:
            plan = "all" if self.wgrad_mode == "deferred" or sum(tiles) >= self.WGRAD_MIN_TILES else "fused"
            if plan == "all" and os.environ.get("MAESTRO_WGRAD_OVERLAP", "0") == "1":
                plan = "ovl"
        self._wgrad_plans[(self.wgrad_mode, hooked)] = plan
        return plan

    def _all_stacks(self) -> list:
        return list(self.dec.values()) + ([self.joint] if self.joint is not None else []) + list(self.enc.values())

    def _with_overlapped_wgrads(self, fn, previous, own):
        def run():
            if previous and self.multi_stream:
                main = torch.cuda.current_stream()
                side = self._wgrad_stream
                side.wait_stream(main)
                with torch.cuda.stream(side):
                    self._launch_wgrads(previous)
                fn()
                main.wait_stream(side)
            else:
                if previous:
                    self._launch_wgrads(previous)
                fn()
            if own:
                self._launch_wgrads(own)
        return run

    def _enc_cuts(self) -> list:
        depth = max(st.depth for st in self.enc.values())
        n = max(1, min(4, int(os.environ.get("MAESTRO_ENC_CUTS", "3"))))
        cut = self.grad_hook is not None or getattr(self, "_plan", None) == "ovl"
        if not cut or depth < 3 or n == 1:
            return [depth, 0]
        return [depth] + [depth - (i * depth) // n for i in range(1, n)] + [0]

    def backward(self, grad_scale: float = 1.0) -> None:
        if grad_scale != 1.0:
            raise NotImplementedError("loss scaling is not needed for bf16 (SURVEY §8(f) AMP row)")
        if self.deterministic:
            with hip.shape_only_tiles():
                return self._backward()
        return self._backward()

    def _backward(self) -> None:
        key = getattr(self, "_cur_key", None)
        plan = self._plan = self._wgrad_plan()
        sfx = f":{plan}:{'h' if self.grad_hook is not None else 'n'}"
        if not self._dw_conv_clear:
            sfx += ":nz"
        if self.fp8 is not None and self.fp8.dgrad:
            sfx += ":f8" if self.fp8.grad_ready else ":cal"
        cuts = self._enc_cuts()
        segs = [("bwd_dec", self._bwd_decoder_side, [(st, 0, st.depth) for st in self.dec.values()])]
        if self.joint is not None:
            segs.append(("bwd_joint", self._bwd_joint, [(self.joint, 0, self.joint.depth)]))
        for i in range(len(cuts) - 1):
            segs.append((f"bwd_enc{i}", lambda hi=cuts[i], lo=cuts[i + 1], first=(i == 0), last=(i == len(cuts) - 2):
                         self._bwd_encoder_side(hi, lo, first, last),
                         [(st, min(cuts[i + 1], st.depth), min(cuts[i], st.depth)) for st in self.enc.values()]))
        with self._tuning_pass("backward"):
            for i, (name, fn, items) in enumerate(segs):
                if plan == "ovl":
                    fn = self._with_overlapped_wgrads(fn, segs[i - 1][2] if i else None, items if i == len(segs) - 1 else None)
                self._segment(name + sfx, key, fn)
        self._dw_conv_clear = False
        if self.fp8 is not None:
            self.fp8.end_of_backward()

    def _bwd_decoder_side(self) -> None:
        m, E, Dd, ps = self.model, self.E, self.Dd, self.store
        AT = hip.OUT_F32 | hip.ATOMIC

        def side(g):
            def run():
                gbuf, st = self.gb[g.name], self.dec[g.name]
                nrm = st.t.norm
                dx, dx16 = st.dxa, st.top16
                for s in g.mods:
                    b = self.mb[s.name]
                    T = s.Beff * s.n_tok
                    conv = m.embed_to_rec[s.embed].pixelify_bands[s.gi].conv
                    w16 = ps.h(conv.weight).view(s.K, Dd)
                    hip.gemm(hip.GEMM_NN, T, Dd, s.K, b["drec"], s.K, w16, Dd, b["dh"], Dd)
                    if self.deterministic:
                        self._det_linear_grads(("rec", s.name), b["drec"], b["hdec"], s.K, Dd, T, ps.g(conv.weight), ps.g(conv.bias))
                        self._det_layernorm_bwd(("ln_dec", s.name), b["dh"], s.n_tok, 0, st.x_last, g.L, s.tok_off, nrm, b["mean_f"],
                                                b["rstd_f"], dx, dx16, st.top_bias_grad(), s.Beff, s.n_tok, Dd)
                        self._grads_ready(m.embed_to_rec[s.embed])
                        continue
                    hip.gemm(hip.GEMM_TN, s.K, Dd, T, b["drec"], s.K, b["hdec"], Dd, ps.g(conv.weight).view(s.K, Dd), Dd, AT)
                    hip.colsum(b["drec"], ps.g(conv.bias), T, s.K, s.K)
                    hip.layernorm_bwd(b["dh"], s.n_tok, 0, st.x_last, g.L, s.tok_off, nrm.weight, b["mean_f"], b["rstd_f"],
                                      None, dx, dx16, ps.g(nrm.weight), ps.g(nrm.bias), st.top_bias_grad(), gbuf["ln_ws"],
                                      s.Beff, s.n_tok, Dd)
                    self._grads_ready(m.embed_to_rec[s.embed])
                dx0, _ = st.backward(dx, defer=self._plan in ("all", "enc", "ovl"))
                side_post(g, gbuf, st, dx0)
            return run

        def side_post(g, gbuf, st, dx0):
            self._grads_ready(st.t.norm)
            hip.gather_rows(dx0, gbuf["vis"], gbuf["dy_e2d"], g.Beff, g.L, g.N, Dd, g.N, 0)
            for s in g.mods:
                if self.deterministic:
                    per_sample = self.tie_order == "torch"
                    n_rows = g.Beff * (g.L if per_sample else s.n_tok)

                    def make(s=s, n_rows=n_rows):
                        rows = hip.unmask_token_grad_partial_rows(n_rows)
                        part = torch.empty(rows, Dd, dtype=F32, device=self.device)
                        return part, [(part.view(-1), ps.g(m.mask_token[s.src]).view(s.G, Dd)[s.gi], rows, Dd, Dd)]
                    part = self._det_site("bwd", ("tok", s.name), make, variant=per_sample)
                    if per_sample:
                        hip.unmask_token_grad_per_sample_det(dx0, gbuf["mask"], gbuf["tok_slot_ps"], part, g.Beff, g.L, Dd, s.slot)
                    else:
                        hip.unmask_token_grad_det(dx0, gbuf["mask"], gbuf["tok_slot"], part, g.Beff, g.L, Dd, s.slot, s.tok_off,
                                                  s.tok_off + s.n_tok)
                elif self.tie_order == "torch":
                    hip.unmask_token_grad_per_sample(dx0, gbuf["mask"], gbuf["tok_slot_ps"],
                                                     ps.g(m.mask_token[s.src]).view(s.G, Dd)[s.gi], g.Beff, g.L, Dd, s.slot)
                else:
                    hip.unmask_token_grad(dx0, gbuf["mask"], gbuf["tok_slot"], ps.g(m.mask_token[s.src]).view(s.G, Dd)[s.gi], g.Beff,
                                          g.L, Dd, s.slot, s.tok_off, s.tok_off + s.n_tok)
                self._ready_spans.append(ps.span([m.mask_token[s.src]]))
            M = g.Beff * g.N
            lin = m.enc_to_dec[g.model]
            if not self.e2d_identity:
                hip.cast_bf16(gbuf["dy_e2d"], gbuf["dy_e2d16"], M * Dd)
                hip.gemm(hip.GEMM_NN, M, E, Dd, gbuf["dy_e2d16"], Dd, ps.h(lin.weight), E, gbuf["dhenc"], E)
                if self.deterministic:
                    self._det_linear_grads(("e2d", g.name), gbuf["dy_e2d16"], gbuf["henc"], Dd, E, M, ps.g(lin.weight), ps.g(lin.bias))
                else:
                    hip.gemm(hip.GEMM_TN, Dd, E, M, gbuf["dy_e2d16"], Dd, gbuf["henc"], E, ps.g(lin.weight), E, AT)
                    hip.colsum(gbuf["dy_e2d16"], ps.g(lin.bias), M, Dd, Dd)
                self._grads_ready(lin)
            if self.joint is not None:
                jt = self.joint
                jn = jt.t.norm
                dy = gbuf["dy_e2d" if self.e2d_identity else "dhenc"]
                if self.deterministic:
                    self._det_layernorm_bwd(("ln_joint", g.name), dy, g.N, 0, jt.x_last, m.joint_N, g.joint_off, jn, gbuf["mean_j"],
                                            gbuf["rstd_j"], jt.dxa, jt.top16, jt.top_bias_grad(), g.Beff, g.N, E)
                else:
                    hip.layernorm_bwd(dy, g.N, 0, jt.x_last, m.joint_N, g.joint_off, jn.weight, gbuf["mean_j"],
                                      gbuf["rstd_j"], None, jt.dxa, jt.top16, ps.g(jn.weight), ps.g(jn.bias),
                                      jt.top_bias_grad(), gbuf["ln_ws"], g.Beff, g.N, E)

        self._run_parallel([side(g) for g in self.groups])
        if self._plan == "enc":
            self._launch_wgrads([(st, 0, st.depth) for st in self.dec.values()])

    def _bwd_joint(self) -> None:
        jt = self.joint
        self._djoint, _ = jt.backward(jt.dxa, defer=self._plan in ("all", "enc", "ovl"))
        self._grads_ready(jt.t.norm)
        if self._plan == "enc":
            self._launch_wgrads([(jt, 0, jt.depth)])

    def _bwd_encoder_side(self, hi: int, lo: int, first: bool, last: bool) -> None:
        m, E, ps = self.model, self.E, self.store

        def side(g):
            def run():
                gbuf, st = self.gb[g.name], self.enc[g.name]
                nrm = st.t.norm
                s_hi, s_lo = min(hi, st.depth), min(lo, st.depth)
                if first and self.deterministic:
                    dy, dy_L, dy_off = ((self._djoint, m.joint_N, g.joint_off) if self.joint is not None else
                                        (gbuf["dy_e2d" if self.e2d_identity else "dhenc"], g.N, 0))
                    self._det_layernorm_bwd(("ln_enc", g.name), dy, dy_L, dy_off, st.x_last, g.N, 0, nrm, gbuf["mean_e"], gbuf["rstd_e"],
                                            st.dxa, st.top16, st.top_bias_grad(), g.Beff, g.N, E)
                    self._grads_ready(nrm)
                    self._enc_state[g.name] = (st.dxa, st.top16)
                elif first:
                    if self.joint is not None:
                        hip.layernorm_bwd(self._djoint, m.joint_N, g.joint_off, st.x_last, g.N, 0, nrm.weight, gbuf["mean_e"],
                                          gbuf["rstd_e"], None, st.dxa, st.top16, ps.g(nrm.weight), ps.g(nrm.bias),
                                          st.top_bias_grad(), gbuf["ln_ws"], g.Beff, g.N, E)
                    else:
                        hip.layernorm_bwd(gbuf["dy_e2d" if self.e2d_identity else "dhenc"], g.N, 0, st.x_last, g.N, 0, nrm.weight,
                                          gbuf["mean_e"],
                                          gbuf["rstd_e"], None, st.dxa, st.top16, ps.g(nrm.weight), ps.g(nrm.bias),
                                          st.top_bias_grad(), gbuf["ln_ws"], g.Beff, g.N, E)
                    self._grads_ready(nrm)
                    self._enc_state[g.name] = (st.dxa, st.top16)
                cur, _ = self._enc_state[g.name]
                self._enc_state[g.name] = st.backward(cur, s_hi, s_lo, defer=self._plan != "fused")
                if last:
                    side_post(g, gbuf, st)
            return run

        def side_post(g, gbuf, st):
            dx0 = self._enc_state[g.name][0]
            hip.expand_rows(dx0, gbuf["inv"], gbuf["dxg"], g.Beff, g.L, g.N, E)
            for s in g.mods:
                self.embed[s.name].backward(gbuf["dxg"], g.L, not self._dw_conv_clear)

        self._run_parallel([side(g) for g in self.groups])
        if self._plan == "enc":
            self._launch_wgrads([(st, min(lo, st.depth), min(hi, st.depth)) for st in self.enc.values()])
        elif self.deterministic and last:
            self._det_finish_backward()
        elif self._plan == "all" and last:
            self._launch_wgrads([(st, 0, st.depth) for st in self._all_stacks()])
        if last:
            for name in m.patch_embed:
                self._grads_ready(m.patch_embed[name])

    def reconstructions(self):
        pixels, masks = {}, {}
        for g in self.groups:
            mask = self.gb[g.name]["mask"]
            for s in g.mods:
                b = self.mb[s.name]
                BD = s.Beff * s.D
                img = torch.empty(BD, s.C, s.S, s.S, dtype=F32, device=self.device)
                hip.depatchify(b["rec"], img, BD, s.C, s.S, s.P)
                pixels[s.name] = img.view(self.B, s.Dates, s.C, s.S, s.S)
                tok = mask[:, s.tok_off: s.tok_off + s.n_tok].bool().reshape(self.B, s.Dates, 1, s.g, 1, s.g, 1)
                masks[s.name] = tok.expand(self.B, s.Dates, s.C, s.g, s.P, s.g, s.P).reshape(self.B, s.Dates, s.C, s.S, s.S)
        for src, parts in self.model.src_specs.items():
            if len(parts) > 1:
                pixels[src] = torch.cat([pixels.pop(s.name) for s in parts], dim=2)
                masks[src] = torch.cat([masks.pop(s.name) for s in parts], dim=2)
        return pixels, masks

    def logged_sample(self, name_mod: str):
        parts = self.model.src_specs[name_mod]
        s0 = parts[0]
        recs, msks = [], []
        for s in parts:
            g = next(g for g in self.groups if s in g.mods)
            rec = torch.empty(1, s.C, s.S, s.S, dtype=F32, device=self.device)
            hip.depatchify(self.mb[s.name]["rec"][: s.L], rec, 1, s.C, s.S, s.P)
            tok = self.gb[g.name]["mask"][0, s.tok_off: s.tok_off + s.L].bool().reshape(1, s.g, 1, s.g, 1)
            recs.append(rec[0])
            msks.append(tok.expand(s.C, s.g, s.P, s.g, s.P).reshape(s.C, s.S, s.S))
        tgt = self._staged[name_mod][0, 0]
        if s0.rescale_elev:
            res = torch.empty(1, s0.C_src, s0.S, s0.S, dtype=F32, device=self.device)
            hip.rescale_elev(tgt.contiguous(), res, 1, s0.C_src, s0.S)
            tgt = res[0]
        return tgt, (recs[0] if len(parts) == 1 else torch.cat(recs)), (msks[0] if len(parts) == 1 else torch.cat(msks))

    def token_masks(self) -> dict:
        return {g.name: self.gb[g.name]["mask"].bool() for g in self.groups}
```

### maestro_amd/hip.py

```python

from __future__ import annotations

import contextlib
import ctypes
import os
from pathlib import Path

import torch

_LIB_PATH = Path(__file__).resolve().parent / "lib" / "libmaestro_hip.so"
_lib = None

GEMM_NT, GEMM_NN, GEMM_TN = 0, 1, 2
OUT_F32, BIAS, GELU, RESIDUAL, DGELU, ATOMIC, COLSUM, AUX_DGELU, MULAUX, C8_E5M2, AUX_U8 = 1, 2, 4, 8, 16, 32, 64, 128, 256, 512, 1024


class HipExtensionError(RuntimeError):
    pass


def lib() -> ctypes.CDLL:
    global _lib
    if _lib is None:
        if not _LIB_PATH.exists():
            raise HipExtensionError(
                f"{_LIB_PATH} not found: build it with `python -m maestro_amd.csrc.build` "
                "(or __graft_entry__.build()).  The MAE hot path has no fallback implementation.")
        retired = [v for v in ("MAESTRO_GROUPED", "MH_GEMM_SPLITK", "MH_ATTN_BWD", "MAESTRO_CU_MASK") if os.environ.get(v)]
        if retired:
            raise HipExtensionError(f"{', '.join(retired)}: retired experiment switch(es) -- the variant no longer exists, this run "
                                    "would measure the default path (INTEGRATION.md, profiles/r05_experiments.md, r06_experiments.md)")
        _lib = ctypes.CDLL(str(_LIB_PATH))
        _lib.mh_last_error.restype = ctypes.c_char_p
        vp, ci = ctypes.c_void_p, ctypes.c_int
        _lib.mh_confusion_ce.argtypes = [vp, vp, ci, ctypes.c_long, vp, ci, ci, ci, ci, ci, vp]
        _lib.mh_confusion_bce.argtypes = [vp, vp, ctypes.c_float, ctypes.c_float, vp, ci, ci, vp]
        _lib.mh_confusion_ce.restype = _lib.mh_confusion_bce.restype = ci
        _lib.mh_reduce_ordered.argtypes = [vp, vp, ci, vp, ci, vp]
        _lib.mh_colsum_partial_rows.argtypes = [ci]
        _lib.mh_masked_loss_partial_size.argtypes = _lib.mh_embed_bwd_partial_rows.argtypes = [ci, ci]
        _lib.mh_unmask_token_grad_partial_rows.argtypes = [ctypes.c_long]
    return _lib


def _check(rc: int, what: str) -> None:
    if rc != 0:
        msg = lib().mh_last_error().decode(errors="replace")
        raise HipExtensionError(f"{what} failed (rc={rc}): {msg}")


def ptr(t: torch.Tensor | None):
    if t is None:
        return ctypes.c_void_p(0)
    if not t.is_cuda:
        raise HipExtensionError("maestro_amd kernels need GPU tensors (no CPU fallback)")
    return ctypes.c_void_p(t.data_ptr())


def stream():
    return ctypes.c_void_p(torch.cuda.current_stream().cuda_stream)


_I, _F, _L = ctypes.c_int, ctypes.c_float, ctypes.c_long


TILE_AUTO, TILE_REG_128, TILE_DMA_256, TILE_DMA_256x128, TILE_DMA_128x256, TILE_DMA_128, TILE_DMA_128x4 = -1, 0, 1, 2, 3, 4, 5
TILE_DMA_256_LOCKSTEP = 6
TILE_REG_64, TILE_REG_192 = 13, 14
TILE_SK_192, TILE_SK_256, TILE_SK_DMA_256 = 15, 16, 17
SK_TILES = (TILE_SK_192, TILE_SK_256, TILE_SK_DMA_256)
TILE_PP_128 = 7
TILES = (TILE_REG_128, TILE_DMA_256, TILE_DMA_256x128, TILE_DMA_128x256, TILE_DMA_128, TILE_DMA_128x4)
_LAYOUT_NAME = {0: "NT", 1: "NN", 2: "TN"}
_TILE_NAME = {TILE_REG_128: "gemm_kernel<{}>", TILE_DMA_256: "gemm_dma_kernel<256x256,{}>",
              TILE_DMA_256x128: "gemm_dma_kernel<256x128,{}>", TILE_DMA_128x256: "gemm_dma_kernel<128x256,{}>",
              TILE_DMA_128: "gemm_dma_kernel<128x128,{}>", TILE_DMA_128x4: "gemm_dma_kernel<128x128q,{}>",
              TILE_DMA_256_LOCKSTEP: "gemm_dma_kernel<256x256,{}>", TILE_PP_128: "gemm_pp_kernel<{}>",
              TILE_REG_64: "gemm_kernel<{},64x128>", TILE_REG_192: "gemm_kernel<{},192x128>",
              TILE_SK_192: "gemm_sk_kernel<{},192x128>", TILE_SK_256: "gemm_sk_kernel<{},256x128>",
              TILE_SK_DMA_256: "gemm_sk_dma_kernel<256x256,{}>"}
_tile_choice: dict = {}
_tuning = False


def set_gemm_tuning(on: bool) -> None:
    global _tuning
    _tuning = bool(on)


def gemm_tile_choices() -> dict:
    return dict(_tile_choice)


class InStepTuner:
# ... 344 lines not shown

    def launch(self) -> None:
        ev = _timer.record_bytes("reduce_ordered", self.nbytes) if _timer is not None else None
        if ev is not None:
            ev[0].record()
        _check(lib().mh_reduce_ordered(ctypes.byref(self.host), ptr(self.table), _I(self.n), ptr(self.blocks), _I(self.n_blocks),
                                       stream()), "mh_reduce_ordered")
        if ev is not None:
            ev[1].record()


def colsum_partial_rows(M) -> int:
    return int(lib().mh_colsum_partial_rows(_I(M)))


def colsum_partial(x, partial, M, N, ld):
    call("mh_colsum_partial", x, _I(1 if x.dtype == torch.float32 else 0), partial, _I(M), _I(N), _I(ld))


def masked_loss_partial_size(B, Lm) -> int:
    return int(lib().mh_masked_loss_partial_size(_I(B), _I(Lm)))


def masked_loss_det(rec, target, mask_group, n_masked, weight, loss_partial, drec, B, Lm, Lgroup, tok_off, PPC, p):
    _hbm_call("masked_loss", float(B) * Lm * (PPC * (_esz(rec) + 4 + _esz(drec)) + 1), "mh_masked_loss_det", rec, target, mask_group,
              n_masked, _F(weight), loss_partial, drec, _I(B), _I(Lm), _I(Lgroup), _I(tok_off), _I(PPC), _I(p))


def masked_loss_bands_det(rec, target, mask_group, n_elems, weight, loss_partial, drec, B, Lm, Lgroup, tok_off, PPC, p, tgt_C,
                          tgt_c0, n_g):
    call("mh_masked_loss_bands_det", rec, target, mask_group, n_elems, _F(weight), loss_partial, drec, _I(B), _I(Lm), _I(Lgroup),
         _I(tok_off), _I(PPC), _I(p), _I(tgt_C), _I(tgt_c0), _I(n_g))


def unmask_token_grad_partial_rows(n_rows) -> int:
    return int(lib().mh_unmask_token_grad_partial_rows(_L(n_rows)))


def unmask_token_grad_det(dxdec, mask, tok_slot, partial, B, L, Dd, slot, t_lo, t_hi):
    call("mh_unmask_token_grad_det", dxdec, mask, tok_slot, partial, _I(B), _I(L), _I(Dd), _I(slot), _I(t_lo), _I(t_hi))


def unmask_token_grad_per_sample_det(dxdec, mask, tok_slot_bl, partial, B, L, Dd, slot):
    call("mh_unmask_token_grad_per_sample_det", dxdec, mask, tok_slot_bl, partial, _I(B), _I(L), _I(Dd), _I(slot))


def embed_bwd_partial_rows(BD, L) -> int:
    return int(lib().mh_embed_bwd_partial_rows(_I(BD), _I(L)))


def embed_finish_bwd_det(dxg, y, stats, gamma, dyc, param_partial, blk_sums, sums, B, D, L, E, tok_off, Lgroup):
    call("mh_embed_finish_bwd_det", dxg, y, stats, gamma, dyc, param_partial, blk_sums, sums, _I(B), _I(D), _I(L), _I(E),
         _I(tok_off), _I(Lgroup))


def det_slices(K: int) -> int:
    return max(1, min(8, K // 1024))


def gemm_tn_slabs(M, N, K, A, lda, B, ldb, slabs):
    S = slabs.shape[0]
    step = -(-(-(-K // S)) // 64) * 64
    for i in range(S):
        k0 = i * step
        kn = min(K, k0 + step) - k0
        if kn <= 0:
            raise HipExtensionError(f"gemm_tn_slabs: empty K-slice {i} of {S} (K = {K})")
        gemm(GEMM_TN, M, N, kn, A[k0:], lda, B[k0:], ldb, slabs[i], N, OUT_F32)


def attn_fwd(qkv, out, lse, B, N, H, D, scale):
    call("mh_attn_fwd", qkv, out, lse, _I(B), _I(N), _I(H), _I(D), _F(scale))


def attn_bwd(qkv, out, dout, lse, delta, dqkv, B, N, H, D, scale):
    call("mh_attn_bwd", qkv, out, dout, lse, delta, dqkv, _I(B), _I(N), _I(H), _I(D), _F(scale))


def patchify(img, cols, target, BD, Ctot, S, P, Kpad, norm_bands, n_groups, normalise, rescale_elev):
    nb = float(BD) * S * S * Ctot * 4 + float(BD) * (S // P) ** 2 * (Kpad * 2 * (cols is not None) + Ctot * P * P * 4 * (target is not None))
    _hbm_call("patchify", nb, "mh_patchify", img, cols, target, _I(BD), _I(Ctot), _I(S), _I(P), _I(Kpad), norm_bands, _I(n_groups),
              _I(int(normalise)), _I(int(rescale_elev)))


def patchify_bands(img, cols, target, BD, Csrc, c0, Ctot, S, P, Kpad, norm_bands, n_groups, normalise, rescale_elev):
    call("mh_patchify_bands", img, cols, target, _I(BD), _I(Csrc), _I(c0), _I(Ctot), _I(S), _I(P), _I(Kpad), norm_bands,
         _I(n_groups), _I(int(normalise)), _I(int(rescale_elev)))


def groupnorm_partial_size(BD, L, E) -> int:
    return int(lib().mh_groupnorm_partial_size(_I(BD), _I(L), _I(E)))


def groupnorm_stats(y, partial, stats, BD, L, E, eps=1e-5):
    call("mh_groupnorm_stats", y, partial, stats, _I(BD), _I(L), _I(E), _F(eps))


def embed_finish(y, stats, gamma, beta, pos, date, date_rows, date_off, xg, B, D, L, E, tok_off, Lgroup):
    call("mh_embed_finish", y, stats, gamma, beta, pos, date, _I(date_rows), _I(date_off), xg, _I(B), _I(D), _I(L), _I(E),
         _I(tok_off), _I(Lgroup))


def date_features(dates, ref_date, out, B, D, rows, row_off, fac):
    call("mh_date_features", dates, ref_date, out, _I(B), _I(D), _I(rows), _I(row_off), _F(fac))


# ... 534 lines not shown
```

Baseline: 1828.

## Fuse bias column sums into loss, gather and embed backward kernels

```diff
diff --git a/__graft_entry__.py b/__graft_entry__.py
--- a/__graft_entry__.py
+++ b/__graft_entry__.py
@@ -25,7 +25,7 @@
     handle = ctypes.CDLL(str(lib))
     import re
 
-    for name in ("maestro_hip.h", "maestro_hip_metrics.h", "maestro_hip_det.h"):
+    for name in ("maestro_hip.h", "maestro_hip_metrics.h", "maestro_hip_det.h", "maestro_hip_ends.h"):
         header = (ROOT / "include" / name).read_text()
         missing = [n for n in re.findall(r"\b(mh_[a-z0-9_]+)\s*\(", header) if not hasattr(handle, n)]
         if missing:
diff --git a/include/maestro_hip_ends.h b/include/maestro_hip_ends.h
--- /dev/null
+++ b/include/maestro_hip_ends.h
@@ -0,0 +1,28 @@
+#ifndef MAESTRO_HIP_ENDS_H
+#define MAESTRO_HIP_ENDS_H
+#include <stdint.h>
+#ifdef __cplusplus
+extern "C" {
+#endif
+
+int mh_masked_loss_cs_rows(int B, int Lm);
+int mh_masked_loss_cs(const float* rec, const float* target, const uint8_t* mask_group, const int* n_masked, float weight,
+                      float* acc, void* drec, float* cs_partial, int B, int Lm, int Lgroup, int tok_off, int PPC, int p,
+                      void* stream);
+int mh_masked_loss_bands_cs(const float* rec, const float* target, const uint8_t* mask_group, const int* n_elems, float weight,
+                            float* acc, void* drec, float* cs_partial, int B, int Lm, int Lgroup, int tok_off, int PPC, int p,
+                            int tgt_C, int tgt_c0, int n_g, void* stream);
+
+int mh_gather_rows_cs_rows(long rows);
+int mh_gather_rows_bf16_cs(const float* src, const int* idx, void* dst16, float* cs_partial, int B, int src_L, int n_idx, int dim,
+                           void* stream);
+
+int mh_embed_bwd_cs_rows(long rows);
+int mh_embed_finish_bwd_ends(const float* dx, const int* inv, int n_vis, const float* y, const float* stats, const float* gamma,
+                             void* dyc, float* dgamma, float* dbeta, float* sums, float* cs_partial, int B, int D, int L, int E,
+                             int tok_off, int Lgroup, void* stream);
+
+#ifdef __cplusplus
+}
+#endif
+#endif
diff --git a/maestro_amd/csrc/build.py b/maestro_amd/csrc/build.py
--- a/maestro_amd/csrc/build.py
+++ b/maestro_amd/csrc/build.py
@@ -33,7 +33,8 @@
 def _digest(src: Path) -> str:
     h = hashlib.sha256()
     for f in [src, *sorted(CSRC.glob("*.hpp")), ROOT / "include" / "maestro_hip.h",
-              ROOT / "include" / "maestro_hip_metrics.h", ROOT / "include" / "maestro_hip_det.h"]:
+              ROOT / "include" / "maestro_hip_metrics.h", ROOT / "include" / "maestro_hip_det.h",
+              ROOT / "include" / "maestro_hip_ends.h"]:
         h.update(f.read_bytes())
     h.update(" ".join(FLAGS + FILE_FLAGS.get(src.name, [])).encode())
     return h.hexdigest()[:16]
diff --git a/maestro_amd/csrc/embed.hip b/maestro_amd/csrc/embed.hip
--- a/maestro_amd/csrc/embed.hip
+++ b/maestro_amd/csrc/embed.hip
@@ -1,6 +1,7 @@
 #include "common.hpp"
 #include "reduce_det.hpp"
 #include "../../include/maestro_hip.h"
+#include "../../include/maestro_hip_ends.h"
 
 namespace {
 
@@ -237,12 +238,14 @@
 }
 
 constexpr int EB_ROWS = 8;
-template <int NV, bool DET>
+template <int NV, bool DET, bool MAP = false>
 __global__ __launch_bounds__(256) void embed_bwd_stats_kernel(const float* __restrict__ dxg, const float* __restrict__ y,
                                                               const float* __restrict__ stats, const float* __restrict__ gamma,
                                                               float* __restrict__ sums, float* __restrict__ dgamma,
                                                               float* __restrict__ dbeta, int B, int D, int L, int E,
-                                                              int tok_off, int Lgroup) {
+                                                              int tok_off, int Lgroup, const int* __restrict__ inv = nullptr,
+                                                              int n_vis = 0) {
+    static_assert(!MAP || NV > 0, "the position-map form keeps its sums in registers");
     extern __shared__ __attribute__((aligned(16))) float red[];
     const int w = threadIdx.x >> 6, lane = threadIdx.x & 63;
     const int bd = blockIdx.y, b = bd / D, d = bd - b * D;
@@ -264,6 +267,11 @@
             if (l >= L) break;
             const float* yr = y + ((size_t)bd * L + l) * E;
             const float* gr = dxg + ((size_t)b * Lgroup + tok_off + d * L + l) * E;
+            if constexpr (MAP) {
+                const int iv = inv[(size_t)b * Lgroup + tok_off + d * L + l];
+                if (iv < 0) continue;
+                gr = dxg + ((size_t)b * n_vis + iv) * E;
+            }
 #pragma unroll
             for (int j = 0; j < NV; ++j) {
                 const int c = lane * 4 + 256 * j;
@@ -368,6 +376,68 @@
         u32x2 pk = {pack_bf2(r[0], r[1]), pack_bf2(r[2], r[3])};
         *reinterpret_cast<u32x2*>(o + c) = pk;
     }
+}
+
+constexpr int EA_ROWS = 8;
+template <int NV, bool MAP>
+__global__ __launch_bounds__(256) void embed_bwd_apply_cs_kernel(const float* __restrict__ dxg, const int* __restrict__ inv, int n_vis,
+                                                                 const float* __restrict__ y, const float* __restrict__ stats,
+                                                                 const float* __restrict__ gamma, const float* __restrict__ sums,
+                                                                 bf16_t* __restrict__ dyc, float* __restrict__ cs_partial,
+                                                                 int B, int D, int L, int E, int tok_off, int Lgroup) {
+    __shared__ f32x4 red[4][64 * NV];
+    const int w = threadIdx.x >> 6, lane = threadIdx.x & 63;
+    const long rows = (long)B * D * L, row0 = ((long)blockIdx.x * 4 + w) * EA_ROWS;
+    const float n = (float)L * (float)E;
+    f32x4 gm[NV], cs[NV];
+#pragma unroll
+    for (int j = 0; j < NV; ++j) {
+        const int c = lane * 4 + 256 * j;
+        cs[j] = (f32x4){0, 0, 0, 0};
+        gm[j] = c < E ? *reinterpret_cast<const f32x4*>(gamma + c) : (f32x4){0, 0, 0, 0};
+    }
+#pragma unroll 2
+    for (int rr = 0; rr < EA_ROWS; ++rr) {
+        const long row = row0 + rr;
+        if (row >= rows) break;
+        const int bd = (int)(row / L), l = (int)(row - (long)bd * L), b = bd / D, d = bd - b * D;
+        const float mu = stats[bd * 2], rs = stats[bd * 2 + 1];
+        const float c1 = sums[bd * 2] / n, c2 = sums[bd * 2 + 1] / n;
+        const float* yr = y + (size_t)row * E;
+        const float* gr = dxg + ((size_t)b * Lgroup + tok_off + d * L + l) * E;
+        bool vis = true;
+        if constexpr (MAP) {
+            const int iv = inv[(size_t)b * Lgroup + tok_off + d * L + l];
+            vis = iv >= 0;
+            gr = dxg + ((size_t)b * n_vis + (vis ? iv : 0)) * E;
+        }
+        bf16_t* o = dyc + (size_t)row * E;
+#pragma unroll
+        for (int j = 0; j < NV; ++j) {
+            const int c = lane * 4 + 256 * j;
+            if (c < E) {
+                const f32x4 v = *reinterpret_cast<const f32x4*>(yr + c);
+                f32x4 dd = {0.f, 0.f, 0.f, 0.f};
+                if (vis) dd = *reinterpret_cast<const f32x4*>(gr + c);
+                float r[4];
+#pragma unroll
+                for (int e = 0; e < 4; ++e) {
+                    const float z = (v[e] - mu) * rs;
+                    r[e] = rs * (dd[e] * gm[j][e] - c1 - z * c2);
+                }
+                const u32x2 pk = {pack_bf2(r[0], r[1]), pack_bf2(r[2], r[3])};
+                *reinterpret_cast<u32x2*>(o + c) = pk;
+                cs[j] += (f32x4){__uint_as_float(pk[0] << 16), __uint_as_float(pk[0] & 0xffff0000u),
+                                 __uint_as_float(pk[1] << 16), __uint_as_float(pk[1] & 0xffff0000u)};
+            }
+        }
+    }
+#pragma unroll
+    for (int j = 0; j < NV; ++j) red[w][lane + 64 * j] = cs[j];
+    __syncthreads();
+    const float* cr = reinterpret_cast<const float*>(red);
+    for (int c = threadIdx.x; c < E; c += 256)
+        cs_partial[(size_t)blockIdx.x * E + c] = (cr[c] + cr[256 * NV + c]) + (cr[512 * NV + c] + cr[768 * NV + c]);
 }
 
 __global__ __launch_bounds__(256) void depatchify_kernel(const float* __restrict__ patches, float* __restrict__ img,
@@ -609,6 +679,38 @@
     return 0;
 }
 
+extern "C" int mh_embed_bwd_cs_rows(long rows) { return rows > 0 ? (int)ceil_div(rows, (long)(4 * EA_ROWS)) : 0; }
+
+extern "C" int mh_embed_finish_bwd_ends(const float* dx, const int* inv, int n_vis, const float* y, const float* stats,
+                                        const float* gamma, void* dyc, float* dgamma, float* dbeta, float* sums, float* cs_partial,
+                                        int B, int D, int L, int E, int tok_off, int Lgroup, void* stream) {
+    MH_CHECK_ARG(dx && y && stats && gamma && dyc && dgamma && dbeta && sums && cs_partial, "mh_embed_finish_bwd_ends: null pointer");
+    MH_CHECK_ARG(B > 0 && D > 0 && L > 0 && E > 0 && E % 4 == 0 && E <= 1024 && tok_off >= 0 && tok_off + D * L <= Lgroup &&
+                 (!inv || (n_vis > 0 && n_vis <= Lgroup)),
+                 "mh_embed_finish_bwd_ends: bad sizes B=%d D=%d L=%d E=%d (E %% 4 == 0, E <= 1024) tok_off=%d Lgroup=%d n_vis=%d", B, D, L, E,
+                 tok_off, Lgroup, n_vis);
+    hipStream_t s = (hipStream_t)stream;
+    hipLaunchKernelGGL(zero_f32_kernel, dim3(ceil_div((long)B * D * 2, 256)), dim3(256), 0, s, sums, B * D * 2);
+    const dim3 grid(ceil_div(L, 4 * EB_ROWS), B * D), block(256), grid2(mh_embed_bwd_cs_rows((long)B * D * L));
+    const size_t lds = (size_t)8 * E * sizeof(float);
+#define MH_EB_LAUNCH(NV, MAP) do { \
+        hipLaunchKernelGGL((embed_bwd_stats_kernel<NV, false, MAP>), grid, block, lds, s, dx, y, stats, gamma, sums, dgamma, dbeta, B, D, L, \
+                           E, tok_off, Lgroup, inv, n_vis); \
+        hipLaunchKernelGGL((embed_bwd_apply_cs_kernel<NV, MAP>), grid2, block, 0, s, dx, inv, n_vis, y, stats, gamma, sums, (bf16_t*)dyc, \
+                           cs_partial, B, D, L, E, tok_off, Lgroup); } while (0)
+#define MH_EB_FORMS(NV) do { if (inv) MH_EB_LAUNCH(NV, true); else MH_EB_LAUNCH(NV, false); } while (0)
+    switch ((E + 255) / 256) {
+        case 1: MH_EB_FORMS(1); break;
+        case 2: MH_EB_FORMS(2); break;
+        case 3: MH_EB_FORMS(3); break;
+        default: MH_EB_FORMS(4); break;
+    }
+#undef MH_EB_FORMS
+#undef MH_EB_LAUNCH
+    MH_LAUNCH_CHECK();
+    return 0;
+}
+
 extern "C" int mh_embed_bwd_partial_rows(int BD, int L) { return BD > 0 && L > 0 ? BD * ceil_div(L, 4 * EB_ROWS) : 0; }
 
 extern "C" int mh_embed_finish_bwd_det(const float* dxg, const float* y, const float* stats, const float* gamma, void* dyc,
diff --git a/maestro_amd/csrc/loss.hip b/maestro_amd/csrc/loss.hip
--- a/maestro_amd/csrc/loss.hip
+++ b/maestro_amd/csrc/loss.hip
@@ -1,20 +1,26 @@
 #include "gemm_common.hpp"
 #include "../../include/maestro_hip_det.h"
+#include "../../include/maestro_hip_ends.h"
 
 namespace {
 
-template <bool DET>
+constexpr int LOSS_CS_NV = 4;
+template <bool DET, bool CS = false>
 __global__ __launch_bounds__(256) void masked_loss_kernel(const float* __restrict__ rec, const float* __restrict__ target,
                                                           const uint8_t* __restrict__ mask_group, const int* __restrict__ n_masked,
                                                           float weight, float* __restrict__ acc, bf16_t* __restrict__ drec,
                                                           int B, int Lm, int Lgroup, int tok_off, int PPC, int p, int tgt_C,
-                                                          int tgt_c0, int n_g, int denom_is_elems, int rows_per_wave) {
+                                                          int tgt_c0, int n_g, int denom_is_elems, int rows_per_wave,
+                                                          float* __restrict__ cs_partial = nullptr) {
     __shared__ float red[4];
     const int w = threadIdx.x >> 6, lane = threadIdx.x & 63;
     const float coef = weight / (denom_is_elems ? (float)(*n_masked) : (float)(*n_masked) * (float)PPC);
     const bool window = n_g != tgt_C;
     const int tgt_ld = window ? PPC / n_g * tgt_C : PPC;
     float s = 0.f;
+    f32x4 cs[CS ? LOSS_CS_NV : 1];
+#pragma unroll
+    for (int j = 0; j < (CS ? LOSS_CS_NV : 1); ++j) cs[j] = (f32x4){0, 0, 0, 0};
     for (int rr = 0; rr < rows_per_wave; ++rr) {
         const int row = (blockIdx.x * 4 + w) * rows_per_wave + rr;
         if (row >= B * Lm) break;
@@ -23,7 +29,7 @@
         const float* r = rec + (size_t)row * PPC;
         const float* g = target + (size_t)row * tgt_ld;
         bf16_t* d = drec ? drec + (size_t)row * PPC : nullptr;
-        for (int c = lane * 4; c < PPC; c += 256) {
+        auto chunk = [&](int c, f32x4* colsum) {
             float dd[4] = {0.f, 0.f, 0.f, 0.f};
             if (masked) {
                 const f32x4 rv = *reinterpret_cast<const f32x4*>(r + c);
@@ -41,11 +47,28 @@
                     else { s += fabsf(diff); dd[e] = (diff > 0.f ? coef : (diff < 0.f ? -coef : 0.f)); }
                 }
             }
-            if (d) {
-                u32x2 pk = {pack_bf2(dd[0], dd[1]), pack_bf2(dd[2], dd[3])};
-                *reinterpret_cast<u32x2*>(d + c) = pk;
-            }
-        }
+            u32x2 pk = {pack_bf2(dd[0], dd[1]), pack_bf2(dd[2], dd[3])};
+            if (d) *reinterpret_cast<u32x2*>(d + c) = pk;
+            if (CS && masked)
+                *colsum += (f32x4){__uint_as_float(pk[0] << 16), __uint_as_float(pk[0] & 0xffff0000u),
+                                   __uint_as_float(pk[1] << 16), __uint_as_float(pk[1] & 0xffff0000u)};
+        };
+        if constexpr (CS) {
+#pragma unroll
+            for (int j = 0; j < LOSS_CS_NV; ++j)
+                if (lane * 4 + 256 * j < PPC) chunk(lane * 4 + 256 * j, &cs[j]);
+        } else {
+            for (int c = lane * 4; c < PPC; c += 256) chunk(c, nullptr);
+        }
+    }
+    if constexpr (CS) {
+        __shared__ f32x4 csred[4][64 * LOSS_CS_NV];
+#pragma unroll
+        for (int j = 0; j < LOSS_CS_NV; ++j) csred[w][lane + 64 * j] = cs[j];
+        __syncthreads();
+        const float* cr = reinterpret_cast<const float*>(csred);
+        for (int c = threadIdx.x; c < PPC; c += 256)
+            cs_partial[(size_t)blockIdx.x * PPC + c] = (cr[c] + cr[256 * LOSS_CS_NV + c]) + (cr[512 * LOSS_CS_NV + c] + cr[768 * LOSS_CS_NV + c]);
     }
     s = wave_sum(s);
     if (lane == 0) red[w] = s;
@@ -292,6 +315,37 @@
     return 0;
 }
 
+extern "C" int mh_masked_loss_cs_rows(int B, int Lm) { return mh_masked_loss_partial_size(B, Lm); }
+
+extern "C" int mh_masked_loss_cs(const float* rec, const float* target, const uint8_t* mask_group, const int* n_masked, float weight,
+                                 float* acc, void* drec, float* cs_partial, int B, int Lm, int Lgroup, int tok_off, int PPC, int p,
+                                 void* stream) {
+    MH_CHECK_ARG(rec && target && mask_group && n_masked && acc && drec && cs_partial, "mh_masked_loss_cs: null pointer");
+    MH_CHECK_ARG(B > 0 && Lm > 0 && (p == 1 || p == 2) && PPC > 0 && PPC % 4 == 0 && PPC <= 256 * LOSS_CS_NV && tok_off >= 0 &&
+                 tok_off + Lm <= Lgroup, "mh_masked_loss_cs: bad arguments (PPC %% 4 == 0, PPC <= %d)", 256 * LOSS_CS_NV);
+    const int rpw = loss_rows_per_wave((long)B * Lm);
+    hipLaunchKernelGGL((masked_loss_kernel<false, true>), dim3(ceil_div((long)B * Lm, 4 * rpw)), dim3(256), 0, (hipStream_t)stream, rec,
+                       target, mask_group, n_masked, weight, acc, (bf16_t*)drec, B, Lm, Lgroup, tok_off, PPC, p, 1, 0, 1, 0, rpw, cs_partial);
+    MH_LAUNCH_CHECK();
+    return 0;
+}
+
+extern "C" int mh_masked_loss_bands_cs(const float* rec, const float* target, const uint8_t* mask_group, const int* n_elems,
+                                       float weight, float* acc, void* drec, float* cs_partial, int B, int Lm, int Lgroup, int tok_off,
+                                       int PPC, int p, int tgt_C, int tgt_c0, int n_g, void* stream) {
+    MH_CHECK_ARG(rec && target && mask_group && n_elems && acc && drec && cs_partial, "mh_masked_loss_bands_cs: null pointer");
+    MH_CHECK_ARG(B > 0 && Lm > 0 && (p == 1 || p == 2) && PPC > 0 && PPC % 4 == 0 && PPC <= 256 * LOSS_CS_NV && tok_off >= 0 &&
+                 tok_off + Lm <= Lgroup, "mh_masked_loss_bands_cs: bad arguments (PPC %% 4 == 0, PPC <= %d)", 256 * LOSS_CS_NV);
+    MH_CHECK_ARG(n_g > 0 && PPC % n_g == 0 && tgt_c0 >= 0 && tgt_c0 + n_g <= tgt_C, "mh_masked_loss_bands_cs: band window [%d, %d) of %d",
+                 tgt_c0, tgt_c0 + n_g, tgt_C);
+    const int rpw = loss_rows_per_wave((long)B * Lm);
+    hipLaunchKernelGGL((masked_loss_kernel<false, true>), dim3(ceil_div((long)B * Lm, 4 * rpw)), dim3(256), 0, (hipStream_t)stream, rec,
+                       target, mask_group, n_elems, weight, acc, (bf16_t*)drec, B, Lm, Lgroup, tok_off, PPC, p, tgt_C, tgt_c0, n_g, 1, rpw,
+                       cs_partial);
+    MH_LAUNCH_CHECK();
+    return 0;
+}
+
 extern "C" int mh_colsum_partial_rows(int M) { return M > 0 ? ceil_div(M, MH_COLSUM_PARTIAL_ROWS) : 0; }
 
 extern "C" int mh_colsum_partial(const void* x, int x_is_f32, float* partial, int M, int N, int ld, void* stream) {
diff --git a/maestro_amd/csrc/mask.hip b/maestro_amd/csrc/mask.hip
--- a/maestro_amd/csrc/mask.hip
+++ b/maestro_amd/csrc/mask.hip
@@ -1,5 +1,6 @@
 #include "common.hpp"
 #include "../../include/maestro_hip.h"
+#include "../../include/maestro_hip_ends.h"
 
 namespace {
 
@@ -70,6 +71,50 @@
     const float* s = src + ((size_t)b * src_L + idx[row]) * dim;
     float* d = dst + ((size_t)b * dst_L + dst_off + j) * dim;
     for (int c = lane * 4; c < dim; c += 256) *reinterpret_cast<f32x4*>(d + c) = *reinterpret_cast<const f32x4*>(s + c);
+}
+
+constexpr int GC_ROWS = 8;
+template <int NV>
+__global__ __launch_bounds__(256) void gather_rows_bf16_cs_kernel(const float* __restrict__ src, const int* __restrict__ idx,
+                                                                  bf16_t* __restrict__ dst, float* __restrict__ cs_partial, int B,
+                                                                  int src_L, int n_idx, int dim) {
+    __shared__ f32x4 red[4][64 * NV];
+    const int w = threadIdx.x >> 6, lane = threadIdx.x & 63;
+    const long rows = (long)B * n_idx, row0 = ((long)blockIdx.x * 4 + w) * GC_ROWS;
+    f32x4 v[GC_ROWS][NV], cs[NV];
+#pragma unroll
+    for (int j = 0; j < NV; ++j) cs[j] = (f32x4){0, 0, 0, 0};
+#pragma unroll
+    for (int r = 0; r < GC_ROWS; ++r) {
+        const long row = min(row0 + r, rows - 1);
+        const float* s = src + ((size_t)(row / n_idx) * src_L + idx[row]) * dim;
+#pragma unroll
+        for (int j = 0; j < NV; ++j) {
+            const int c = lane * 4 + 256 * j;
+            v[r][j] = *reinterpret_cast<const f32x4*>(s + (c < dim ? c : 0));
+        }
+    }
+#pragma unroll
+    for (int r = 0; r < GC_ROWS; ++r) {
+        const long row = row0 + r;
+        if (row >= rows) break;
+#pragma unroll
+        for (int j = 0; j < NV; ++j) {
+            const int c = lane * 4 + 256 * j;
+            if (c < dim) {
+                const u32x2 pk = {pack_bf2(v[r][j][0], v[r][j][1]), pack_bf2(v[r][j][2], v[r][j][3])};
+                *reinterpret_cast<u32x2*>(dst + (size_t)row * dim + c) = pk;
+                cs[j] += (f32x4){__uint_as_float(pk[0] << 16), __uint_as_float(pk[0] & 0xffff0000u),
+                                 __uint_as_float(pk[1] << 16), __uint_as_float(pk[1] & 0xffff0000u)};
+            }
+        }
+    }
+#pragma unroll
+    for (int j = 0; j < NV; ++j) red[w][lane + 64 * j] = cs[j];
+    __syncthreads();
+    const float* cr = reinterpret_cast<const float*>(red);
+    for (int c = threadIdx.x; c < dim; c += 256)
+        cs_partial[(size_t)blockIdx.x * dim + c] = (cr[c] + cr[256 * NV + c]) + (cr[512 * NV + c] + cr[768 * NV + c]);
 }
 
 __global__ __launch_bounds__(256) void scatter_rows_kernel(const float* __restrict__ ddst, const int* __restrict__ idx,
@@ -200,6 +245,27 @@
     return 0;
 }
 
+extern "C" int mh_gather_rows_cs_rows(long rows) { return rows > 0 ? (int)ceil_div(rows, (long)(4 * GC_ROWS)) : 0; }
+
+extern "C" int mh_gather_rows_bf16_cs(const float* src, const int* idx, void* dst16, float* cs_partial, int B, int src_L, int n_idx,
+                                      int dim, void* stream) {
+    MH_CHECK_ARG(src && idx && dst16 && cs_partial, "mh_gather_rows_bf16_cs: null pointer");
+    MH_CHECK_ARG(B > 0 && src_L > 0 && n_idx > 0 && n_idx <= src_L && dim > 0 && dim % 4 == 0 && dim <= 1024,
+                 "mh_gather_rows_bf16_cs: bad sizes B=%d src_L=%d n_idx=%d dim=%d (dim %% 4 == 0, dim <= 1024)", B, src_L, n_idx, dim);
+    const dim3 grid(mh_gather_rows_cs_rows((long)B * n_idx)), block(256);
+#define MH_GC_LAUNCH(NV) hipLaunchKernelGGL((gather_rows_bf16_cs_kernel<NV>), grid, block, 0, (hipStream_t)stream, src, idx, \
+                                            (bf16_t*)dst16, cs_partial, B, src_L, n_idx, dim)
+    switch ((dim + 255) / 256) {
+        case 1: MH_GC_LAUNCH(1); break;
+        case 2: MH_GC_LAUNCH(2); break;
+        case 3: MH_GC_LAUNCH(3); break;
+        default: MH_GC_LAUNCH(4); break;
+    }
+#undef MH_GC_LAUNCH
+    MH_LAUNCH_CHECK();
+    return 0;
+}
+
 extern "C" int mh_scatter_rows(const float* ddst, const int* idx, float* dsrc, int B, int src_L, int n_idx, int dim,
                                int dst_L, int dst_off, void* stream) {
     MH_CHECK_ARG(ddst && idx && dsrc && dim % 4 == 0 && dst_off + n_idx <= dst_L, "mh_scatter_rows: bad arguments");
diff --git a/maestro_amd/csrc/norm.hip b/maestro_amd/csrc/norm.hip
--- a/maestro_amd/csrc/norm.hip
+++ b/maestro_amd/csrc/norm.hip
@@ -1,4 +1,5 @@
 #include "gemm_common.hpp"
+#include <type_traits>
 
 namespace {
 
@@ -374,6 +375,100 @@
 #pragma unroll
                 for (int e = 0; e < 4; ++e) o[e] = rs * (dz[i][e] - c1 - xh[i][e] * c2);
                 o += rq[rr][i];
+                csum[i] += o;
+                *reinterpret_cast<f32x4*>(dx + xrowq[rr] + c4) = o;
+                const u32x2 pk = {pack_bf2(o[0], o[1]), pack_bf2(o[2], o[3])};
+                *reinterpret_cast<u32x2*>(dx_bf16 + xrowq[rr] + c4) = pk;
+            }
+            __builtin_amdgcn_sched_barrier(0);
+        }
+    }
+    if (!partial) return;
+    float* rg = red + (size_t)w * 3 * dim;
+#pragma unroll
+    for (int i = 0; i < NV; ++i) {
+        const int c4 = 4 * (lane + 64 * i);
+        *reinterpret_cast<f32x4*>(rg + c4) = gsum[i];
+        *reinterpret_cast<f32x4*>(rg + dim + c4) = bsum[i];
+        *reinterpret_cast<f32x4*>(rg + 2 * dim + c4) = csum[i];
+    }
+    __syncthreads();
+    float* prow = partial + (size_t)blockIdx.x * 3 * dim;
+    for (int c = threadIdx.x; c < 3 * dim; c += 256)
+        prow[c] = red[c] + red[3 * dim + c] + red[6 * dim + c] + red[9 * dim + c];
+}
+
+template <int NV, int DEPTH, bool DY_F32>
+__global__ __launch_bounds__(256) void ln_bwd_final_kernel(const void* __restrict__ dy, RowMap dym, const float* __restrict__ x,
+                                                          RowMap xm, const float* __restrict__ gamma,
+                                                          const float* __restrict__ mean, const float* __restrict__ rstd,
+                                                          float* __restrict__ dx,
+                                                          bf16_t* __restrict__ dx_bf16, float* __restrict__ partial, int B, int n) {
+    constexpr int dim = 256 * NV;
+    static_assert(DEPTH >= 1 && DEPTH <= ROWS_PER_WAVE, "prefetch distance in rows");
+    extern __shared__ __attribute__((aligned(16))) float red[];
+    const int w = __builtin_amdgcn_readfirstlane(threadIdx.x >> 6), lane = threadIdx.x & 63;
+    f32x4 gsum[NV], bsum[NV], csum[NV], gm[NV];
+#pragma unroll
+    for (int i = 0; i < NV; ++i) {
+        gsum[i] = (f32x4){0, 0, 0, 0}; bsum[i] = (f32x4){0, 0, 0, 0}; csum[i] = (f32x4){0, 0, 0, 0};
+        gm[i] = *reinterpret_cast<const f32x4*>(gamma + 4 * (lane + 64 * i));
+    }
+    const int row0 = (blockIdx.x * 4 + w) * ROWS_PER_WAVE;
+    if (row0 < B * n) {
+        f32x4 xq[ROWS_PER_WAVE][NV];
+        std::conditional_t<DY_F32, f32x4, u32x2> dq[ROWS_PER_WAVE][NV];
+        float muq[ROWS_PER_WAVE], rsq[ROWS_PER_WAVE];
+        size_t xrowq[ROWS_PER_WAVE];
+        auto fetch = [&](int p) {
+            const int row = row0 + p, b = row / n, j = row - b * n;
+            xrowq[p] = map_row(xm, b, j) * dim;
+            const size_t dyrow = map_row(dym, b, j) * dim;
+            muq[p] = mean[row]; rsq[p] = rstd[row];
+#pragma unroll
+            for (int i = 0; i < NV; ++i) {
+                const int c4 = 4 * (lane + 64 * i);
+                xq[p][i] = *reinterpret_cast<const f32x4*>(x + xrowq[p] + c4);
+                if constexpr (DY_F32) dq[p][i] = *reinterpret_cast<const f32x4*>(reinterpret_cast<const float*>(dy) + dyrow + c4);
+                else dq[p][i] = *reinterpret_cast<const u32x2*>(reinterpret_cast<const bf16_t*>(dy) + dyrow + c4);
+            }
+        };
+#pragma unroll
+        for (int p = 0; p < DEPTH; ++p) fetch(p);
+#pragma unroll
+        for (int rr = 0; rr < ROWS_PER_WAVE; ++rr) {
+            if (rr + DEPTH < ROWS_PER_WAVE) fetch(rr + DEPTH);
+            __builtin_amdgcn_sched_barrier(0);
+            const float mu = muq[rr], rs = rsq[rr];
+            f32x4 xh[NV], dz[NV];
+            float s1 = 0.f, s2 = 0.f;
+#pragma unroll
+            for (int i = 0; i < NV; ++i) {
+                f32x4 d;
+                if constexpr (DY_F32) {
+                    d = dq[rr][i];
+                } else {
+                    const u32x2 pk = dq[rr][i];
+                    d = (f32x4){__uint_as_float(pk[0] << 16), __uint_as_float(pk[0] & 0xffff0000u),
+                                __uint_as_float(pk[1] << 16), __uint_as_float(pk[1] & 0xffff0000u)};
+                }
+#pragma unroll
+                for (int e = 0; e < 4; ++e) {
+                    xh[i][e] = (xq[rr][i][e] - mu) * rs;
+                    dz[i][e] = d[e] * gm[i][e];
+                    s1 += dz[i][e];
+                    s2 += dz[i][e] * xh[i][e];
+                    gsum[i][e] += d[e] * xh[i][e];
+                    bsum[i][e] += d[e];
+                }
+            }
+            const float c1 = ln_wave_sum(s1) / dim, c2 = ln_wave_sum(s2) / dim;
+#pragma unroll
+            for (int i = 0; i < NV; ++i) {
+                const int c4 = 4 * (lane + 64 * i);
+                f32x4 o;
+#pragma unroll
+                for (int e = 0; e < 4; ++e) o[e] = rs * (dz[i][e] - c1 - xh[i][e] * c2);
                 csum[i] += o;
                 *reinterpret_cast<f32x4*>(dx + xrowq[rr] + c4) = o;
                 const u32x2 pk = {pack_bf2(o[0], o[1]), pack_bf2(o[2], o[3])};
@@ -519,8 +614,18 @@
 #define LN_BWD_FAST(NV, DEPTH) hipLaunchKernelGGL((ln_bwd_fast_kernel<NV, DEPTH>), grid, block, lds, s, (const bf16_t*)dy, \
                                                   RowMap{dy_L, dy_off}, x, RowMap{x_L, x_off}, gamma, mean, rstd, dres, dx, \
                                                   (bf16_t*)dx_bf16, part, B, n)
+#define LN_BWD_FINAL(NV, DEPTH) do { \
+        if (dy_is_f32) hipLaunchKernelGGL((ln_bwd_final_kernel<NV, DEPTH, true>), grid, block, lds, s, dy, RowMap{dy_L, dy_off}, x, \
+                                          RowMap{x_L, x_off}, gamma, mean, rstd, dx, (bf16_t*)dx_bf16, part, B, n); \
+        else hipLaunchKernelGGL((ln_bwd_final_kernel<NV, DEPTH, false>), grid, block, lds, s, dy, RowMap{dy_L, dy_off}, x, \
+                                RowMap{x_L, x_off}, gamma, mean, rstd, dx, (bf16_t*)dx_bf16, part, B, n); } while (0)
     const int nvs = ln_nv(dim);
-    if (MH_LN_FAST && nvs <= 4 && dim == 256 * nvs && !dy_is_f32 && dres && dx_bf16 && rows % ROWS_PER_WAVE == 0) {
+    const bool fast = MH_LN_FAST && nvs <= 4 && dim == 256 * nvs && dx_bf16 && rows % ROWS_PER_WAVE == 0;
+    if (fast && !dres) {
+        constexpr int DEPTH = LN_BWD_DEPTH < ROWS_PER_WAVE ? LN_BWD_DEPTH : ROWS_PER_WAVE, DEPTH4 = 2 < ROWS_PER_WAVE ? 2 : ROWS_PER_WAVE;
+        switch (nvs) { case 1: LN_BWD_FINAL(1, DEPTH); break; case 2: LN_BWD_FINAL(2, DEPTH); break;
+                       case 3: LN_BWD_FINAL(3, DEPTH); break; default: LN_BWD_FINAL(4, DEPTH4); }
+    } else if (fast && !dy_is_f32) {
         constexpr int DEPTH = LN_BWD_DEPTH < ROWS_PER_WAVE ? LN_BWD_DEPTH : ROWS_PER_WAVE, DEPTH4 = 2 < ROWS_PER_WAVE ? 2 : ROWS_PER_WAVE;
         switch (nvs) { case 1: LN_BWD_FAST(1, DEPTH); break; case 2: LN_BWD_FAST(2, DEPTH); break;
                        case 3: LN_BWD_FAST(3, DEPTH); break; default: LN_BWD_FAST(4, DEPTH4); }
@@ -529,6 +634,7 @@
                        case 4: LN_BWD(4); break; default: LN_BWD(8); }
     }
 #undef LN_BWD_FAST
+#undef LN_BWD_FINAL
 #undef LN_BWD
     if (dgamma && !partial_only)
         hipLaunchKernelGGL(ln_bwd_reduce_kernel, dim3(ceil_div(3 * dim, 256), ceil_div(nblk, RED_ROWS)), dim3(256), 0, s,
diff --git a/maestro_amd/engine.py b/maestro_amd/engine.py
--- a/maestro_amd/engine.py
+++ b/maestro_amd/engine.py
@@ -385,18 +385,42 @@
         hip.embed_finish(b["yconv"], b["gn_stats"], pe.norm.weight, pe.norm.bias, b["pos_enc"], gbuf["dates"], gbuf["n_dates"],
                          s.date_off, xg, s.Beff, s.D, s.L, E, s.tok_off, Lgroup)
 
-    def backward(self, dxg: torch.Tensor, Lgroup: int, clear_dw: bool) -> None:
+    def backward(self, dxg: torch.Tensor, Lgroup: int, clear_dw: bool, defer_wgrad: bool = False) -> None:
         eng, s, b = self.eng, self.s, self.buf
         ps, E, pe, T = eng.store, eng.E, b["pe"], s.Beff * s.n_tok
         if getattr(eng, "deterministic", False):
             return self._backward_det(dxg, Lgroup)
         hip.embed_finish_bwd(dxg, b["yconv"], b["gn_stats"], pe.norm.weight, b["dyc"], ps.g(pe.norm.weight), ps.g(pe.norm.bias),
                              b["gn_sums"], s.Beff, s.D, s.L, E, s.tok_off, Lgroup)
+        if not defer_wgrad:
+            self._wgrad_in_line(clear_dw)
+        hip.colsum(b["dyc"], ps.g(pe.conv.bias), T, E, E)
+
+    def _wgrad_in_line(self, clear_dw: bool) -> None:
+        eng, s, b = self.eng, self.s, self.buf
+        E, T = eng.E, s.Beff * s.n_tok
         if clear_dw:
             b["dw_conv"].zero_()
         hip.gemm(hip.GEMM_TN, E, s.Kpad, T, b["dyc"], E, b["cols"], s.Kpad, b["dw_conv"], s.Kpad, hip.OUT_F32 | hip.ATOMIC)
-        hip.unpack_rows_add(b["dw_conv"], ps.g(pe.conv.weight), E, s.K, s.Kpad)
-        hip.colsum(b["dyc"], ps.g(pe.conv.bias), T, E, E)
+        hip.unpack_rows_add(b["dw_conv"], eng.store.g(b["pe"].conv.weight), E, s.K, s.Kpad)
+
+    def wgrad_problem(self) -> tuple:
+        b, s, E = self.buf, self.s, self.eng.E
+        return (b["dyc"], b["cols"], b["dw_conv"], E, s.Kpad, s.Beff * s.n_tok, E, s.Kpad, s.Kpad)
+
+    def cs_buffer(self) -> torch.Tensor:
+        b, s = self.buf, self.s
+        if b.get("dyc_cs") is None:
+            b["dyc_cs"] = torch.empty(hip.embed_bwd_cs_rows(s.Beff * s.n_tok), self.eng.E, dtype=F32, device=self.eng.device)
+        return b["dyc_cs"]
+
+    def backward_ends(self, dx: torch.Tensor, inv, n_vis: int, Lgroup: int, defer_wgrad: bool, clear_dw: bool) -> None:
+        eng, s, b = self.eng, self.s, self.buf
+        ps, E, pe = eng.store, eng.E, b["pe"]
+        hip.embed_finish_bwd_ends(dx, inv, n_vis, b["yconv"], b["gn_stats"], pe.norm.weight, b["dyc"], ps.g(pe.norm.weight),
+                                  ps.g(pe.norm.bias), b["gn_sums"], self.cs_buffer(), s.Beff, s.D, s.L, E, s.tok_off, Lgroup)
+        if not defer_wgrad:
+            self._wgrad_in_line(clear_dw)
 
     def _backward_det(self, dxg: torch.Tensor, Lgroup: int) -> None:
         eng, s, b = self.eng, self.s, self.buf
@@ -606,18 +630,31 @@
         if self.warm_passes > 0:
             self._warm_up(one_pass)
 
-    def _launch_wgrads(self, items) -> None:
+    def _launch_wgrads(self, items, ends=()) -> None:
         items = [(st, lo, hi) for st, lo, hi in items if hi > lo]
-        if not items:
+        if not items and not ends:
             return
-        key = tuple((st.tag, lo, hi) for st, lo, hi in items)
+        key = (tuple((st.tag, lo, hi) for st, lo, hi in items), tuple(ends))
         table = self._wgrad_tables.get(key)
         if table is None:
+            if torch.cuda.is_current_stream_capturing():
+                raise hip.HipExtensionError(f"weight-gradient table {key} first needed inside a hipGraph capture")
             probs = [p for st, lo, hi in items for p in st.wgrad_problems(lo, hi)]
             jobs = [j for st, lo, hi in items for j in st.reduce_jobs(lo, hi)]
-            table = self._wgrad_tables[key] = (hip.GroupedTN(probs, self.device), hip.ColsumBatch(jobs, self.device))
-        table[1].launch()
-        table[0].launch()
+            after, ready = [], []
+            for tag in ends:
+                e_probs, e_jobs, e_after, e_ready = self._ends_table(tag)
+                probs, jobs, after, ready = probs + e_probs, jobs + e_jobs, after + e_after, ready + e_ready
+            table = self._wgrad_tables[key] = (hip.GroupedTN(probs, self.device) if probs else None,
+                                               hip.ColsumBatch(jobs, self.device) if jobs else None, after, ready)
+        if table[1] is not None:
+            table[1].launch()
+        if table[0] is not None:
+            table[0].launch()
+        for fn in table[2]:
+            fn()
+        for module in table[3]:
+            self._grads_ready(module)
 
     @contextlib.contextmanager
     def _tuning_pass(self, what: str):
@@ -719,6 +756,11 @@
         if self.wgrad_mode not in ("auto", "fused", "deferred"):
             raise ValueError(f"MAESTRO_WGRAD={self.wgrad_mode!r}: expected auto, fused or deferred")
         self._wgrad_plans, self._zero_lists = {}, {}
+        self.ends_parts = frozenset(os.environ.get("MAESTRO_ENDS", "abc")) if not self.deterministic and dtype != "fp8" else frozenset()
+        if not self.ends_parts <= frozenset("abc") or ("c" in self.ends_parts and "b" not in self.ends_parts):
+            raise ValueError(f"MAESTRO_ENDS={os.environ.get('MAESTRO_ENDS')!r}: a subset of 'abc' expected, 'c' only with 'b'")
+        self._loss_cs = False
+        self._ends_ws = {}
         self._det_sites, self._det_tables = {"fwd": {}, "bwd": {}}, {}
         self._h2d_done = [None] * RING
         self._opt = None
@@ -854,6 +896,8 @@
             self.mb[name].update(
                 target=first["target"] if first else e(T, s.C_src * s.P * s.P), hdec=e(T, Dd, dt=BF16), mean_f=e(T), rstd_f=e(T),
                 rec=e(T, s.K), drec=e(T, s.K, dt=BF16), dh=e(T, Dd, dt=BF16), cnt=first["cnt"] if first else z(1, dt=I32))
+            if "b" in self.ends_parts and s.K <= 1024:
+                self.mb[name]["drec_cs"] = e(hip.masked_loss_cs_rows(s.Beff, s.n_tok), s.K)
         self.gb = {}
         self.enc, self.dec = {}, {}
         for g in self.groups:
@@ -863,12 +907,13 @@
             date_row = torch.cat([(s.date_off + torch.arange(s.n_tok) // s.L).to(I32) for s in g.mods])
             pos_dec = torch.cat([m.pos_dec_rows[s.name].repeat(s.D, 1) for s in g.mods], dim=0)
             self.gb[g.name] = dict(
-                xg=e(Bn, L, E), dxg=z(Bn, L, E),
+                xg=e(Bn, L, E),
                 vis=e(Bn, N, dt=I32), msk=e(Bn, g.k, dt=I32), inv=e(Bn, L, dt=I32), mask=e(Bn, L, dt=U8),
                 dates=z(Bn, n_dates, 8), n_dates=n_dates, tok_slot=tok_slot.to(dev), date_row=date_row.to(dev),
                 pos_dec=pos_dec.to(dev).contiguous(), tok_table=e(len(g.mods), Dd),
                 henc=e(Bn * N, E, dt=BF16), mean_e=e(Bn * N), rstd_e=e(Bn * N), y_e2d=e(Bn * N, Dd),
                 dy_e2d=e(Bn * N, Dd), dy_e2d16=e(Bn * N, Dd, dt=BF16), dhenc=e(Bn * N, E, dt=BF16),
+                e2d_cs=e(hip.gather_rows_cs_rows(Bn * N), Dd) if "b" in self.ends_parts and Dd <= 1024 else None,
                 mean_j=e(Bn * N), rstd_j=e(Bn * N))
             holder = m.encoder[g.model]
             self.enc[g.name] = Stack(self, holder, Bn, N, f"enc.{g.name}")
@@ -1003,7 +1048,9 @@
         self._h2d_done[slot] = ev
         batch = self._stage_inputs(batch)
         with self._tuning_pass("forward"):
-            self._segment("forward" if self._opt is None else "forward:opt", self._cur_key, lambda: self._forward_launches(batch))
+            self._loss_cs = "b" in self.ends_parts and self._wgrad_plan() != "fused"
+            self._segment("forward" if self._opt is None else "forward:opt", (self._cur_key, self._loss_cs),
+                          lambda: self._forward_launches(batch))
         if self._opt is not None:
             self.store.mark_synced()
         return self.loss_acc
@@ -1179,6 +1226,14 @@
                     else:
                         hip.masked_loss_bands_det(b["rec"], b["target"], gbuf["mask"], b["cnt"], self.loss_w[s.src], part,
                                                   b["drec"], s.Beff, s.n_tok, g.L, s.tok_off, s.K, self.p_loss, s.C_src, s.c0, s.C)
+                elif self._loss_cs and b.get("drec_cs") is not None:
+                    if s.G == 1:
+                        hip.masked_loss_cs(b["rec"], b["target"], gbuf["mask"], b["cnt"], self.loss_w[s.src], self.loss_acc,
+                                           b["drec"], b["drec_cs"], s.Beff, s.n_tok, g.L, s.tok_off, s.K, self.p_loss)
+                    else:
+                        hip.masked_loss_bands_cs(b["rec"], b["target"], gbuf["mask"], b["cnt"], self.loss_w[s.src], self.loss_acc,
+                                                 b["drec"], b["drec_cs"], s.Beff, s.n_tok, g.L, s.tok_off, s.K, self.p_loss,
+                                                 s.C_src, s.c0, s.C)
                 elif s.G == 1:
                     hip.masked_loss(b["rec"], b["target"], gbuf["mask"], b["cnt"], self.loss_w[s.src], self.loss_acc,
                                     b["drec"], s.Beff, s.n_tok, g.L, s.tok_off, s.K, self.p_loss)
@@ -1228,8 +1283,8 @@
                 cur = off + n
             if cur < self.store.total:
                 spans.append((cur, self.store.total - cur))
-            for b in self.mb.values():
-                if b.get("dw_conv") is not None:
+            for name, b in self.mb.items():
+                if b.get("dw_conv") is not None and not self._ends_deferred(self.embed[name].wgrad_problem(), plan):
                     spans.append(((b["dw_conv"].data_ptr() - base) // 4, b["dw_conv"].numel()))
             dev = torch.tensor([v for sp in spans for v in sp], dtype=torch.int64, device=self.device)
             z = self._zero_lists[plan] = (dev, len(spans), max(n for _, n in spans))
@@ -1277,15 +1332,15 @@
                 side = self._wgrad_stream
                 side.wait_stream(main)
                 with torch.cuda.stream(side):
-                    self._launch_wgrads(previous)
+                    self._launch_wgrads(*previous)
                 fn()
                 main.wait_stream(side)
             else:
                 if previous:
-                    self._launch_wgrads(previous)
+                    self._launch_wgrads(*previous)
                 fn()
             if own:
-                self._launch_wgrads(own)
+                self._launch_wgrads(*own)
         return run
 
     def _enc_cuts(self) -> list:
@@ -1312,26 +1367,131 @@
             sfx += ":nz"
         if self.fp8 is not None and self.fp8.dgrad:
             sfx += ":f8" if self.fp8.grad_ready else ":cal"
+        if self._ends("b") and not self._loss_cs:
+            sfx += ":nolcs"
         cuts = self._enc_cuts()
-        segs = [("bwd_dec", self._bwd_decoder_side, [(st, 0, st.depth) for st in self.dec.values()])]
+        segs = [("bwd_dec", self._bwd_decoder_side, [(st, 0, st.depth) for st in self.dec.values()], self._ends_tags("dec"))]
         if self.joint is not None:
-            segs.append(("bwd_joint", self._bwd_joint, [(self.joint, 0, self.joint.depth)]))
+            segs.append(("bwd_joint", self._bwd_joint, [(self.joint, 0, self.joint.depth)], ()))
         for i in range(len(cuts) - 1):
-            segs.append((f"bwd_enc{i}", lambda hi=cuts[i], lo=cuts[i + 1], first=(i == 0), last=(i == len(cuts) - 2):
+            first, last = i == 0, i == len(cuts) - 2
+            segs.append((f"bwd_enc{i}", lambda hi=cuts[i], lo=cuts[i + 1], first=first, last=last:
                          self._bwd_encoder_side(hi, lo, first, last),
-                         [(st, min(cuts[i + 1], st.depth), min(cuts[i], st.depth)) for st in self.enc.values()]))
+                         [(st, min(cuts[i + 1], st.depth), min(cuts[i], st.depth)) for st in self.enc.values()],
+                         self._ends_tags(*(["enc_first"] if first else []), *(["enc_last"] if last else []))))
         with self._tuning_pass("backward"):
-            for i, (name, fn, items) in enumerate(segs):
+            for i, (name, fn, items, ends) in enumerate(segs):
                 if plan == "ovl":
-                    fn = self._with_overlapped_wgrads(fn, segs[i - 1][2] if i else None, items if i == len(segs) - 1 else None)
+                    fn = self._with_overlapped_wgrads(fn, segs[i - 1][2:] if i else None, (items, ends) if i == len(segs) - 1 else None)
                 self._segment(name + sfx, key, fn)
         self._dw_conv_clear = False
         if self.fp8 is not None:
             self.fp8.end_of_backward()
 
+    def _ends(self, part: str, plan: str | None = None) -> bool:
+        return part in self.ends_parts and (self._plan if plan is None else plan) in ("all", "enc", "ovl")
+
+    def _ends_tags(self, *tags) -> tuple:
+        if not self.ends_parts or self._plan == "fused":
+            return ()
+        stale = self._ends("b") and not self._loss_cs
+        return tuple("dec:nolcs" if t == "dec" and stale else t for t in tags)
+
+    def _ends_deferred(self, prob, plan: str | None = None) -> bool:
+        if not self._ends("a", plan):
+            return False
+        try:
+            hip.GroupedTN.check(0, prob)
+            return True
+        except hip.HipExtensionError:
+            return False
+
+    def _embed_cs(self) -> bool:
+        return self._ends("b") and self.E <= 1024
+
+    def _ends_buf(self, key, *shape) -> torch.Tensor:
+        buf = self._ends_ws.get(key)
+        if buf is None:
+            if torch.cuda.is_current_stream_capturing():
+                raise hip.HipExtensionError(f"ends workspace {key} first needed inside a hipGraph capture")
+            buf = self._ends_ws[key] = torch.empty(*shape, dtype=F32, device=self.device)
+        return buf
+
+    def _final_layernorm_bwd(self, key, gbuf, dy, dy_L, dy_off, x, x_L, x_off, norm, mean, rstd, dx, dx16, bias_grad, B, n, dim) -> None:
+        if self._ends("b"):
+            ws = self._ends_buf(key, hip.layernorm_bwd_workspace(B * n, dim))
+            hip.layernorm_bwd_partial(dy, dy_L, dy_off, x, x_L, x_off, norm.weight, mean, rstd, None, dx, dx16, ws, B, n, dim)
+        else:
+            g = self.store.g
+            hip.layernorm_bwd(dy, dy_L, dy_off, x, x_L, x_off, norm.weight, mean, rstd, None, dx, dx16, g(norm.weight), g(norm.bias),
+                              bias_grad, gbuf["ln_ws"], B, n, dim)
+
+    def _ends_ln_jobs(self, key, norm, bias_grad, dim) -> list:
+        ws, g = self._ends_ws[key], self.store.g
+        rows = ws.numel() // (3 * dim)
+        jobs = [(ws, g(norm.weight), rows, dim, 3 * dim), (ws[dim:], g(norm.bias), rows, dim, 3 * dim)]
+        if bias_grad is not None:
+            jobs.append((ws[2 * dim:], bias_grad, rows, dim, 3 * dim))
+        return jobs
+
+    def _rec_wgrad(self, s) -> tuple:
+        b, Dd = self.mb[s.name], self.Dd
+        conv = self.model.embed_to_rec[s.embed].pixelify_bands[s.gi].conv
+        return (b["drec"], b["hdec"], self.store.g(conv.weight).view(s.K, Dd), s.K, Dd, s.Beff * s.n_tok, s.K, Dd, Dd)
+
+    def _e2d_wgrad(self, g) -> tuple:
+        gbuf, lin = self.gb[g.name], self.model.enc_to_dec[g.model]
+        return (gbuf["dy_e2d16"], gbuf["henc"], self.store.g(lin.weight), self.Dd, self.E, g.Beff * g.N, self.Dd, self.E, self.E)
+
+    def _ends_table(self, tag: str):
+        m, ps, E, Dd = self.model, self.store, self.E, self.Dd
+        probs, jobs, after, ready = [], [], [], []
+        if tag in ("dec", "dec:nolcs"):
+            for g in self.groups:
+                gbuf, st = self.gb[g.name], self.dec[g.name]
+                for s in g.mods:
+                    b = self.mb[s.name]
+                    conv = m.embed_to_rec[s.embed].pixelify_bands[s.gi].conv
+                    if self._ends_deferred(self._rec_wgrad(s)):
+                        probs.append(self._rec_wgrad(s))
+                    if self._ends("b"):
+                        if tag == "dec" and b.get("drec_cs") is not None:
+                            jobs.append((b["drec_cs"].view(-1), ps.g(conv.bias), b["drec_cs"].shape[0], s.K, s.K))
+                        jobs += self._ends_ln_jobs(("ln_dec", s.name), st.t.norm, st.top_bias_grad(), Dd)
+                    ready.append(m.embed_to_rec[s.embed])
+                ready.append(st.t.norm)
+                if not self.e2d_identity:
+                    if self._ends_deferred(self._e2d_wgrad(g)):
+                        probs.append(self._e2d_wgrad(g))
+                    if self._ends("b") and gbuf["e2d_cs"] is not None:
+                        jobs.append((gbuf["e2d_cs"].view(-1), ps.g(m.enc_to_dec[g.model].bias), gbuf["e2d_cs"].shape[0], Dd, Dd))
+                    ready.append(m.enc_to_dec[g.model])
+                if self.joint is not None and self._ends("b"):
+                    jobs += self._ends_ln_jobs(("ln_joint", g.name), self.joint.t.norm, self.joint.top_bias_grad(), E)
+        elif tag == "enc_first":
+            for g in self.groups:
+                st = self.enc[g.name]
+                if self._ends("b"):
+                    jobs += self._ends_ln_jobs(("ln_enc", g.name), st.t.norm, st.top_bias_grad(), E)
+                ready.append(st.t.norm)
+        elif tag == "enc_last":
+            for g in self.groups:
+                for s in g.mods:
+                    end, b = self.embed[s.name], self.mb[s.name]
+                    if self._ends_deferred(end.wgrad_problem()):
+                        probs.append(end.wgrad_problem())
+                        after.append(lambda b=b, s=s: hip.unpack_rows_add(b["dw_conv"], ps.g(b["pe"].conv.weight), E, s.K, s.Kpad))
+                    if self._embed_cs():
+                        jobs.append((end.cs_buffer().view(-1), ps.g(b["pe"].conv.bias), end.cs_buffer().shape[0], E, E))
+        else:
+            raise ValueError(tag)
+        return probs, jobs, after, ready
+
     def _bwd_decoder_side(self) -> None:
         m, E, Dd, ps = self.model, self.E, self.Dd, self.store
         AT = hip.OUT_F32 | hip.ATOMIC
+        ends = self._ends_tags("dec")
+        loss_cs = ends == ("dec",) and self._ends("b")
 
         def side(g):
             def run():
@@ -1350,19 +1510,26 @@
                                                 b["rstd_f"], dx, dx16, st.top_bias_grad(), s.Beff, s.n_tok, Dd)
                         self._grads_ready(m.embed_to_rec[s.embed])
                         continue
-                    hip.gemm(hip.GEMM_TN, s.K, Dd, T, b["drec"], s.K, b["hdec"], Dd, ps.g(conv.weight).view(s.K, Dd), Dd, AT)
-                    hip.colsum(b["drec"], ps.g(conv.bias), T, s.K, s.K)
-                    hip.layernorm_bwd(b["dh"], s.n_tok, 0, st.x_last, g.L, s.tok_off, nrm.weight, b["mean_f"], b["rstd_f"],
-                                      None, dx, dx16, ps.g(nrm.weight), ps.g(nrm.bias), st.top_bias_grad(), gbuf["ln_ws"],
-                                      s.Beff, s.n_tok, Dd)
-                    self._grads_ready(m.embed_to_rec[s.embed])
+                    if not self._ends_deferred(self._rec_wgrad(s)):
+                        hip.gemm(hip.GEMM_TN, s.K, Dd, T, b["drec"], s.K, b["hdec"], Dd, ps.g(conv.weight).view(s.K, Dd), Dd, AT)
+                    if not (loss_cs and b.get("drec_cs") is not None):
+                        hip.colsum(b["drec"], ps.g(conv.bias), T, s.K, s.K)
+                    self._final_layernorm_bwd(("ln_dec", s.name), gbuf, b["dh"], s.n_tok, 0, st.x_last, g.L, s.tok_off, nrm, b["mean_f"],
+                                              b["rstd_f"], dx, dx16, st.top_bias_grad(), s.Beff, s.n_tok, Dd)
+                    if not ends:
+                        self._grads_ready(m.embed_to_rec[s.embed])
                 dx0, _ = st.backward(dx, defer=self._plan in ("all", "enc", "ovl"))
                 side_post(g, gbuf, st, dx0)
             return run
 
         def side_post(g, gbuf, st, dx0):
-            self._grads_ready(st.t.norm)
-            hip.gather_rows(dx0, gbuf["vis"], gbuf["dy_e2d"], g.Beff, g.L, g.N, Dd, g.N, 0)
+            if not ends:
+                self._grads_ready(st.t.norm)
+            e2d_cs = gbuf["e2d_cs"] if self._ends("b") and not self.e2d_identity else None
+            if e2d_cs is not None:
+                hip.gather_rows_bf16_cs(dx0, gbuf["vis"], gbuf["dy_e2d16"], e2d_cs, g.Beff, g.L, g.N, Dd)
+            else:
+                hip.gather_rows(dx0, gbuf["vis"], gbuf["dy_e2d"], g.Beff, g.L, g.N, Dd, g.N, 0)
             for s in g.mods:
                 if self.deterministic:
                     per_sample = self.tie_order == "torch"
@@ -1388,14 +1555,18 @@
             M = g.Beff * g.N
             lin = m.enc_to_dec[g.model]
             if not self.e2d_identity:
-                hip.cast_bf16(gbuf["dy_e2d"], gbuf["dy_e2d16"], M * Dd)
+                if e2d_cs is None:
+                    hip.cast_bf16(gbuf["dy_e2d"], gbuf["dy_e2d16"], M * Dd)
                 hip.gemm(hip.GEMM_NN, M, E, Dd, gbuf["dy_e2d16"], Dd, ps.h(lin.weight), E, gbuf["dhenc"], E)
                 if self.deterministic:
                     self._det_linear_grads(("e2d", g.name), gbuf["dy_e2d16"], gbuf["henc"], Dd, E, M, ps.g(lin.weight), ps.g(lin.bias))
                 else:
-                    hip.gemm(hip.GEMM_TN, Dd, E, M, gbuf["dy_e2d16"], Dd, gbuf["henc"], E, ps.g(lin.weight), E, AT)
-                    hip.colsum(gbuf["dy_e2d16"], ps.g(lin.bias), M, Dd, Dd)
-                self._grads_ready(lin)
+                    if not self._ends_deferred(self._e2d_wgrad(g)):
+                        hip.gemm(hip.GEMM_TN, Dd, E, M, gbuf["dy_e2d16"], Dd, gbuf["henc"], E, ps.g(lin.weight), E, AT)
+                    if e2d_cs is None:
+                        hip.colsum(gbuf["dy_e2d16"], ps.g(lin.bias), M, Dd, Dd)
+                if not ends:
+                    self._grads_ready(lin)
             if self.joint is not None:
                 jt = self.joint
                 jn = jt.t.norm
@@ -1404,13 +1575,12 @@
                     self._det_layernorm_bwd(("ln_joint", g.name), dy, g.N, 0, jt.x_last, m.joint_N, g.joint_off, jn, gbuf["mean_j"],
                                             gbuf["rstd_j"], jt.dxa, jt.top16, jt.top_bias_grad(), g.Beff, g.N, E)
                 else:
-                    hip.layernorm_bwd(dy, g.N, 0, jt.x_last, m.joint_N, g.joint_off, jn.weight, gbuf["mean_j"],
-                                      gbuf["rstd_j"], None, jt.dxa, jt.top16, ps.g(jn.weight), ps.g(jn.bias),
-                                      jt.top_bias_grad(), gbuf["ln_ws"], g.Beff, g.N, E)
+                    self._final_layernorm_bwd(("ln_joint", g.name), gbuf, dy, g.N, 0, jt.x_last, m.joint_N, g.joint_off, jn, gbuf["mean_j"],
+                                              gbuf["rstd_j"], jt.dxa, jt.top16, jt.top_bias_grad(), g.Beff, g.N, E)
 
         self._run_parallel([side(g) for g in self.groups])
         if self._plan == "enc":
-            self._launch_wgrads([(st, 0, st.depth) for st in self.dec.values()])
+            self._launch_wgrads([(st, 0, st.depth) for st in self.dec.values()], ends)
 
     def _bwd_joint(self) -> None:
         jt = self.joint
@@ -1421,6 +1591,7 @@
 
     def _bwd_encoder_side(self, hi: int, lo: int, first: bool, last: bool) -> None:
         m, E, ps = self.model, self.E, self.store
+        ends = self._ends_tags(*(["enc_first"] if first else []), *(["enc_last"] if last else []))
 
         def side(g):
             def run():
@@ -1435,16 +1606,12 @@
                     self._grads_ready(nrm)
                     self._enc_state[g.name] = (st.dxa, st.top16)
                 elif first:
-                    if self.joint is not None:
-                        hip.layernorm_bwd(self._djoint, m.joint_N, g.joint_off, st.x_last, g.N, 0, nrm.weight, gbuf["mean_e"],
-                                          gbuf["rstd_e"], None, st.dxa, st.top16, ps.g(nrm.weight), ps.g(nrm.bias),
-                                          st.top_bias_grad(), gbuf["ln_ws"], g.Beff, g.N, E)
-                    else:
-                        hip.layernorm_bwd(gbuf["dy_e2d" if self.e2d_identity else "dhenc"], g.N, 0, st.x_last, g.N, 0, nrm.weight,
-                                          gbuf["mean_e"],
-                                          gbuf["rstd_e"], None, st.dxa, st.top16, ps.g(nrm.weight), ps.g(nrm.bias),
-                                          st.top_bias_grad(), gbuf["ln_ws"], g.Beff, g.N, E)
-                    self._grads_ready(nrm)
+                    dy, dy_L, dy_off = ((self._djoint, m.joint_N, g.joint_off) if self.joint is not None else
+                                        (gbuf["dy_e2d" if self.e2d_identity else "dhenc"], g.N, 0))
+                    self._final_layernorm_bwd(("ln_enc", g.name), gbuf, dy, dy_L, dy_off, st.x_last, g.N, 0, nrm, gbuf["mean_e"],
+                                              gbuf["rstd_e"], st.dxa, st.top16, st.top_bias_grad(), g.Beff, g.N, E)
+                    if not ends:
+                        self._grads_ready(nrm)
                     self._enc_state[g.name] = (st.dxa, st.top16)
                 cur, _ = self._enc_state[g.name]
                 self._enc_state[g.name] = st.backward(cur, s_hi, s_lo, defer=self._plan != "fused")
@@ -1454,17 +1621,28 @@
 
         def side_post(g, gbuf, st):
             dx0 = self._enc_state[g.name][0]
+            if self._ends("c") and self._embed_cs():
+                for s in g.mods:
+                    end = self.embed[s.name]
+                    end.backward_ends(dx0, gbuf["inv"], g.N, g.L, self._ends_deferred(end.wgrad_problem()), not self._dw_conv_clear)
+                return
+            if gbuf.get("dxg") is None:
+                gbuf["dxg"] = torch.empty(g.Beff, g.L, E, dtype=F32, device=self.device)
             hip.expand_rows(dx0, gbuf["inv"], gbuf["dxg"], g.Beff, g.L, g.N, E)
             for s in g.mods:
-                self.embed[s.name].backward(gbuf["dxg"], g.L, not self._dw_conv_clear)
+                end = self.embed[s.name]
+                if self._embed_cs():
+                    end.backward_ends(gbuf["dxg"], None, 0, g.L, self._ends_deferred(end.wgrad_problem()), not self._dw_conv_clear)
+                else:
+                    end.backward(gbuf["dxg"], g.L, not self._dw_conv_clear, self._ends_deferred(end.wgrad_problem()))
 
         self._run_parallel([side(g) for g in self.groups])
         if self._plan == "enc":
-            self._launch_wgrads([(st, min(lo, st.depth), min(hi, st.depth)) for st in self.enc.values()])
+            self._launch_wgrads([(st, min(lo, st.depth), min(hi, st.depth)) for st in self.enc.values()], ends)
         elif self.deterministic and last:
             self._det_finish_backward()
         elif self._plan == "all" and last:
-            self._launch_wgrads([(st, 0, st.depth) for st in self._all_stacks()])
+            self._launch_wgrads([(st, 0, st.depth) for st in self._all_stacks()], self._ends_tags("dec", "enc_first", "enc_last"))
         if last:
             for name in m.patch_embed:
                 self._grads_ready(m.patch_embed[name])
diff --git a/maestro_amd/hip.py b/maestro_amd/hip.py
--- a/maestro_amd/hip.py
+++ b/maestro_amd/hip.py
@@ -40,6 +40,8 @@
         _lib.mh_colsum_partial_rows.argtypes = [ci]
         _lib.mh_masked_loss_partial_size.argtypes = _lib.mh_embed_bwd_partial_rows.argtypes = [ci, ci]
         _lib.mh_unmask_token_grad_partial_rows.argtypes = [ctypes.c_long]
+        _lib.mh_masked_loss_cs_rows.argtypes = [ci, ci]
+        _lib.mh_gather_rows_cs_rows.argtypes = _lib.mh_embed_bwd_cs_rows.argtypes = [ctypes.c_long]
     return _lib
 
 
@@ -490,6 +492,38 @@
 def embed_finish_bwd_det(dxg, y, stats, gamma, dyc, param_partial, blk_sums, sums, B, D, L, E, tok_off, Lgroup):
     call("mh_embed_finish_bwd_det", dxg, y, stats, gamma, dyc, param_partial, blk_sums, sums, _I(B), _I(D), _I(L), _I(E),
          _I(tok_off), _I(Lgroup))
+
+
+def masked_loss_cs_rows(B, Lm) -> int:
+    return int(lib().mh_masked_loss_cs_rows(_I(B), _I(Lm)))
+
+
+def masked_loss_cs(rec, target, mask_group, n_masked, weight, acc, drec, cs_partial, B, Lm, Lgroup, tok_off, PPC, p):
+    _hbm_call("masked_loss", float(B) * Lm * (PPC * (_esz(rec) + 4 + _esz(drec)) + 1), "mh_masked_loss_cs", rec, target, mask_group,
+              n_masked, _F(weight), acc, drec, cs_partial, _I(B), _I(Lm), _I(Lgroup), _I(tok_off), _I(PPC), _I(p))
+
+
+def masked_loss_bands_cs(rec, target, mask_group, n_elems, weight, acc, drec, cs_partial, B, Lm, Lgroup, tok_off, PPC, p, tgt_C,
+                         tgt_c0, n_g):
+    call("mh_masked_loss_bands_cs", rec, target, mask_group, n_elems, _F(weight), acc, drec, cs_partial, _I(B), _I(Lm), _I(Lgroup),
+         _I(tok_off), _I(PPC), _I(p), _I(tgt_C), _I(tgt_c0), _I(n_g))
+
+
+def gather_rows_cs_rows(rows) -> int:
+    return int(lib().mh_gather_rows_cs_rows(_L(rows)))
+
+
+def gather_rows_bf16_cs(src, idx, dst16, cs_partial, B, src_L, n_idx, dim):
+    call("mh_gather_rows_bf16_cs", src, idx, dst16, cs_partial, _I(B), _I(src_L), _I(n_idx), _I(dim))
+
+
+def embed_bwd_cs_rows(rows) -> int:
+    return int(lib().mh_embed_bwd_cs_rows(_L(rows)))
+
+
+def embed_finish_bwd_ends(dx, inv, n_vis, y, stats, gamma, dyc, dgamma, dbeta, sums, cs_partial, B, D, L, E, tok_off, Lgroup):
+    call("mh_embed_finish_bwd_ends", dx, inv, _I(n_vis), y, stats, gamma, dyc, dgamma, dbeta, sums, cs_partial, _I(B), _I(D), _I(L),
+         _I(E), _I(tok_off), _I(Lgroup))
 
 
 def det_slices(K: int) -> int:
```

Measured after the change: 1860 (median of 6 runs). 1.7% higher.
